# phaistos-networks/Trinity

Hardware: AMD Instinct MI355X
Metric: queries/sec (higher is better)
Workload: dtype u32

## Files before the change

### trinity_amd/csrc/dev_stream.hpp

```cpp
#pragma once
#include "dev_structs.hpp"
#include <hip/hip_runtime.h>

#ifdef TRI_PROF
__device__ unsigned long long g_prof[32];
struct ProfClock {
        long long t;
        unsigned long long acc[16];
        __device__ __forceinline__ void start() {
                for (int i = 0; i < 16; ++i)
                        acc[i] = 0;
                t = clock64();
        }
        __device__ __forceinline__ void lap(const int phase) {
                const long long n = clock64();
                acc[phase] += (unsigned long long)(n - t);
                t = n;
        }
        __device__ __forceinline__ void flush() {
                if (threadIdx.x == 0)
                        for (int i = 0; i < 16; ++i)
                                if (acc[i])
                                        atomicAdd(&g_prof[i], acc[i]);
        }
};
#define PROF_DECL ProfClock prof_
#define PROF_START() prof_.start()
#define PROF_LAP(p) prof_.lap(p)
#define PROF_FLUSH() prof_.flush()
#define PROF_ARG , ProfClock &prof_
#define PROF_PASS , prof_
#ifdef TRI_PROF_COUNTS
#define PROF_COUNT(slot, n) atomicAdd(&g_prof[slot], (unsigned long long)(n))
#else
#define PROF_COUNT(slot, n)
#endif
#else
#define PROF_DECL
#define PROF_START()
#define PROF_LAP(p)
#define PROF_FLUSH()
#define PROF_ARG
#define PROF_PASS
#define PROF_COUNT(slot, n)
#endif

#ifdef TRI_TASKTIMES
static unsigned long long *g_tt_host = nullptr;
static size_t g_tt_cap = 0;
__device__ unsigned long long *g_tt = nullptr;
#define TASKTIME_(i) do { if (threadIdx.x == 0) g_tt[(i)] = wall_clock64(); } while (0)
#if TRI_TASKTIMES == 2
#define TASKTIME(i)
#define TASKTIME_SCORE(i) TASKTIME_(i)
#define TASKTIME_PLANES(i)
#define TASKTIME_DENSE(i)
#define TASKTIME_PHRASE(i)
#elif TRI_TASKTIMES == 3
#define TASKTIME(i)
#define TASKTIME_SCORE(i)
#define TASKTIME_PLANES(i) TASKTIME_(i)
#define TASKTIME_DENSE(i)
#define TASKTIME_PHRASE(i)
#elif TRI_TASKTIMES == 4
#define TASKTIME(i)
#define TASKTIME_SCORE(i)
#define TASKTIME_PLANES(i)
#define TASKTIME_DENSE(i) TASKTIME_(i)
#define TASKTIME_PHRASE(i)
#elif TRI_TASKTIMES == 5
#define TASKTIME(i)
#define TASKTIME_SCORE(i)
#define TASKTIME_PLANES(i)
#define TASKTIME_DENSE(i)
#define TASKTIME_PHRASE(i) TASKTIME_(i)
#else
#define TASKTIME(i) TASKTIME_(i)
#define TASKTIME_SCORE(i)
#define TASKTIME_PLANES(i)
#define TASKTIME_DENSE(i)
#define TASKTIME_PHRASE(i)
#endif
#else
#define TASKTIME(i)
#define TASKTIME_SCORE(i)
#define TASKTIME_PLANES(i)
#define TASKTIME_DENSE(i)
#define TASKTIME_PHRASE(i)
#endif

#ifdef TRI_TRACE
static uint32_t *g_trace_host = nullptr;
__device__ volatile uint32_t *g_trace = nullptr;
#ifndef TRI_TRACE_MASK
#define TRI_TRACE_MASK 0xffffffffu
#endif
#define TRACE(stage, a, b)                                                      \
        do {                                                                    \
                if (((TRI_TRACE_MASK >> (stage)) & 1u) && threadIdx.x == 0 && g_trace) {                              \
                        volatile uint32_t *t_ = g_trace + (blockIdx.x & 63) * 4; \
                        t_[0] = (stage);                                        \
                        t_[1] = (a);                                            \
                        t_[2] = (b);                                            \
                        t_[3] = t_[3] + 1;                                      \
                        __threadfence_system();                                 \
                }                                                               \
        } while (0)
#else
#define TRACE(stage, a, b) \
        do {               \
        } while (0)
#endif

__device__ __forceinline__ uint32_t vb_decode(uint64_t w, uint32_t &len) {
        const uint32_t lo32 = (uint32_t)w;
        const uint32_t b0 = lo32 & 0xffu;
        const uint32_t ones = __clz(~(lo32 << 24));
        const uint32_t n = ones < 4u ? ones : 4u;
        const uint32_t be = __builtin_bswap32(lo32);
        const uint32_t v1 = b0;
        const uint32_t v2 = (be >> 16) & 0x3fffu;
        const uint32_t v3 = ((b0 & 0x1fu) << 16) | ((lo32 >> 8) & 0xffffu);
        const uint32_t v4 = be & 0x0fffffffu;
        const uint32_t v5 = (uint32_t)(w >> 8);
        len = n + 1;
        uint32_t v = v1;
        v = n == 1 ? v2 : v;
        v = n == 2 ? v3 : v;
        v = n == 3 ? v4 : v;
        v = n == 4 ? v5 : v;
        return v;
}

#ifndef TRI_VB_AHEAD
#define TRI_VB_AHEAD 3
#endif
struct VbStream {
        static constexpr int AHEAD = TRI_VB_AHEAD;
        const uint64_t *q;
        uint64_t lo, hi, n[AHEAD];
        int valid;

        __device__ __forceinline__ void init(const uint8_t *p) {
                const uint32_t sk = (uint32_t)((uintptr_t)p & 7u);
                q = (const uint64_t *)(p - sk);
                const uint64_t w0 = q[0], w1 = q[1];
#pragma unroll
                for (int i = 0; i < AHEAD; ++i)
                        n[i] = q[2 + i];
                q += 2 + AHEAD;
                const uint32_t sh = sk * 8;
                lo = sh ? (w0 >> sh) | (w1 << (64 - sh)) : w0;
                hi = sh ? (w1 >> sh) : w1;
                valid = 16 - (int)sk;
        }
        __device__ __forceinline__ void refill() {
                if (valid <= 8) {
                        const uint64_t w = n[0];
#pragma unroll
                        for (int i = 0; i + 1 < AHEAD; ++i)
                                n[i] = n[i + 1];
                        n[AHEAD - 1] = *q++;
                        const uint32_t sh = (uint32_t)valid * 8;
                        if (valid == 8)
                                hi = w;
                        else if (valid == 0) {
                                lo = w;
                                hi = 0;
                        } else {
                                lo |= w << sh;
                                hi = w >> (64 - sh);
                        }
                        valid += 8;
                }
        }
        __device__ __forceinline__ uint32_t next() {
                refill();
                uint32_t len;
                const uint32_t v = vb_decode(lo, len);
                const uint32_t s = len * 8;
                lo = (lo >> s) | (hi << (64 - s));
                hi >>= s;
                valid -= (int)len;
                return v;
        }
        __device__ __forceinline__ const uint8_t *tell() const { return (const uint8_t *)q - 8 * AHEAD - valid; }
        __device__ __forceinline__ uint32_t byte() {
                refill();
                const uint32_t b = (uint32_t)lo & 0xffu;
                lo = (lo >> 8) | (hi << 56);
                hi >>= 8;
                valid -= 1;
                return b;
        }
        __device__ __forceinline__ void skip(uint32_t n) {
                for (; n; --n)
                        (void)byte();
        }
        __device__ __forceinline__ bool small_run(const uint32_t k) const { return (lo & (0x8080808080808080ull >> (8u * (8u - k)))) == 0; }
        __device__ __forceinline__ uint64_t take(const uint32_t k) {
                const uint64_t w = lo;
                if (k == 8) {
                        lo = hi;
                        hi = 0;
                } else {
                        const uint32_t s = k * 8;
                        lo = (lo >> s) | (hi << (64 - s));
                        hi >>= s;
                }
                valid -= (int)k;
                return w;
        }
};
```

### trinity_amd/csrc/dev_structs.hpp

```cpp
#pragma once
#include <cstdint>
#ifdef __HIPCC__
#define TRI_HD __host__ __device__
#else
#define TRI_HD
#endif

struct DevTerm {
        uint32_t documents;
        uint32_t first_block;
        uint32_t nblocks;
        uint32_t last_n;
        uint32_t win_off;
        uint32_t flags;
        uint32_t npfor;
        uint32_t pad;
};
constexpr uint32_t TERM_FULL_BLOCKS = 1u;
constexpr uint32_t TERM_SPARSE = 2u;

#define TRI_BLOCK_N(t, b, index, off) (((t).flags & TERM_FULL_BLOCKS) ? ((b) + 1 == (t).nblocks ? (t).last_n : 32u) : (uint32_t)(index)[(off)-1])
constexpr uint32_t WIN_MIN_BLOCKS = 128;

constexpr uint32_t QT_GROUP = 0x80000000u;
constexpr uint32_t QT_NOT = 0x40000000u;
constexpr uint32_t QT_TERM = 0x3fffffffu;
constexpr uint32_t MAX_QTERMS = 16;
struct DevQuery {
        uint32_t nterms;
        uint32_t term_base;
        uint64_t out_off;
        uint32_t out_cap;
        uint32_t qid;
        uint32_t first_task, ntasks;
        uint32_t score_base, nscore;
        uint32_t phrase_base, nphrases;
        uint32_t fused_idx, form;
};

constexpr uint32_t RESULT_DOCIDS = 0, RESULT_BITMAP = 1;
constexpr uint32_t MAX_PHRASE_TERMS = 16;
struct DevPhrase {
        uint32_t term_base;
        uint32_t nterms;
        double weight;
};

struct DevTask {
        uint32_t slot;
        uint32_t tile_begin;
        uint32_t tile_end;
        uint32_t kind;
        uint64_t out_off;
};
constexpr uint32_t CAND_QUEUES = 8;
constexpr uint32_t CAND_TICKET_STRIDE = 16;
constexpr uint32_t CAND_HEAVY_TILES = 3;
constexpr uint32_t TASK_CAND = 0;
constexpr uint32_t TASK_DENSE = 1;
constexpr uint32_t TASK_FUSED = 2;
constexpr uint32_t TASK_FUSED16 = 3;

constexpr uint32_t TASK_FUSED_GEN = 4;
constexpr uint32_t TASK_PLANES = 5;
constexpr uint32_t TASK_PLANES8 = 6;
constexpr uint32_t TASK_PSET = 7;
constexpr uint32_t TASK_PROBE = 8;
constexpr uint32_t TASK_TREE = 9;
constexpr uint32_t TASK_KINDS = 10;
constexpr uint32_t PSET_INLINE_TERMS = 4;
#ifndef TRI_PSET_TASK_WINDOWS
#define TRI_PSET_TASK_WINDOWS 4
#endif
constexpr uint32_t PSET_TASK_WINDOWS = TRI_PSET_TASK_WINDOWS;
struct DevPsetUnit {
        uint64_t out_off;
        uint32_t w_begin, w_end;
        uint32_t tix;
        uint32_t nterms;
        uint32_t term_base;
        uint32_t first;
        uint32_t tt[PSET_INLINE_TERMS];
        uint32_t row[PSET_INLINE_TERMS];
};
static_assert(sizeof(DevPsetUnit) == 64, "one cache-line half per unit");
constexpr uint32_t PSET_UNIT_FIRST = 1u, PSET_UNIT_BITMAP = 2u;
constexpr uint32_t PSET_UNIT_ROUND_SHIFT = 4, PSET_UNIT_ROUND_MASK = 15u;
constexpr uint32_t PSET_ROUND_DOCS = 16384, PSET_STAGE_DOCS = 1024;
constexpr uint32_t PSET_UNIT_SCATTER = 4u;
constexpr uint32_t TREE_MAX_NODES = 64;
constexpr uint32_t TREE_HDR_WORDS = 8;
constexpr uint32_t TREE_CHUNK_WORDS = 2048;
constexpr uint32_t TREE_ROW_PHRASE = 0x80000000u;
struct DevTreeNode {
        uint8_t op;
        uint8_t parent;
        uint8_t ord;
        uint8_t thr;
        uint32_t arg;
        uint32_t row;
        uint32_t score;
        uint32_t rmask;
        uint8_t kid0, kid1, pad0, pad1;
        uint64_t kids;
};
static_assert(sizeof(DevTreeNode) == 32, "eight words per node");
TRI_HD constexpr bool task_onepass(const uint32_t kind) { return kind >= TASK_FUSED && kind <= TASK_PLANES8; }

constexpr uint32_t PL_W = 32768;
constexpr uint32_t PL_WORDS = PL_W / 32;
constexpr uint32_t PL_NONE = 0xffffffffu;
constexpr uint32_t PL_NESTED = 6;
constexpr uint32_t PL_LEVEL_WORDS = 3;
constexpr uint32_t PL_STORED = 4;
constexpr uint32_t PL_PLANES = PL_STORED + PL_LEVEL_WORDS;
constexpr uint32_t PL_HI = PL_PLANES - 1;
constexpr uint32_t PL_HI_LEVELS = PL_STORED - 1;
constexpr uint32_t PL_RANK_WORDS = 16;
constexpr uint32_t PL_RANK_DOCS = 256;
constexpr uint32_t BLK_HITS_PLAIN = 0x80000000u;
constexpr int TILE_BLOCKS = 256;
constexpr int TILE_CANDS = TILE_BLOCKS * 32;
constexpr uint32_t SPAN_BITS = 1u << 17;
constexpr uint32_t SPAN_WORDS = SPAN_BITS / 32;
constexpr uint32_t CELL_LOG2 = 10;
constexpr uint32_t CELL_DOCS = 1u << CELL_LOG2;
constexpr uint32_t CELLS_PER_SPAN = SPAN_BITS / CELL_DOCS;
#ifndef TRI_FUS_CELLS
#define TRI_FUS_CELLS 14
#endif
constexpr uint32_t FUS_CELLS = TRI_FUS_CELLS;
constexpr uint32_t FUS_W = FUS_CELLS * CELL_DOCS;
constexpr uint32_t PLK_MAX_SPARSE = 6;
constexpr uint32_t PLK_NS_SMALL = 5;
constexpr uint32_t TOPK_MAX = 256;
constexpr uint32_t FUS_MAX_SLOTS = 8;
constexpr uint32_t FUS_MAX_LEAVES = 16;
struct DevFused {
        uint32_t nslots;
        uint32_t fbits;
        uint32_t cap;
        uint32_t nreq;
        uint32_t term[FUS_MAX_SLOTS];
        uint32_t gmask[FUS_MAX_SLOTS];
        uint32_t gslots[FUS_MAX_SLOTS];
        uint32_t nmask;
        uint32_t hw;
        uint32_t mode;
        uint32_t nleaf;
        uint32_t tt[8];
        uint8_t leaf_slot[FUS_MAX_LEAVES];
        uint32_t ctt[FUS_MAX_LEAVES][8];
        uint32_t plane[FUS_MAX_SLOTS];
        uint32_t negslots;
};
constexpr uint32_t FUS_MODE_TT = 1;
constexpr uint32_t FUS_MODE_EMIT = 2;
```

### trinity_amd/csrc/host/plan_host.cpp

```cpp
#include "../planner.hpp"
#include "../lucene_enc_units.hpp"
#include "lucene_encoder.hpp"

#include <cstdlib>
#include <memory>
#include <mutex>

namespace {
        struct HostPlan {
                BatchPlan P;
                uint8_t *block = nullptr;
                ~HostPlan() { free(block); }
        };
        void put_err(char *err, size_t cap, const std::string &s) {
                if (err && cap) {
                        const size_t n = std::min(cap - 1, s.size());
                        memcpy(err, s.data(), n);
                        err[n] = 0;
                }
        }
}

extern "C" {
void *tri_host_index_build(const uint8_t *index, uint64_t len, const uint8_t *hits, uint64_t hits_len, int codec, const uint32_t *terms3, uint64_t nterms,
                           uint32_t docs_cnt, char *err, uint64_t errcap) {
        auto H = std::make_unique<HostIndex>();
        std::string e;
        static_assert(sizeof(tri_term) == 12, "tri_term is three u32");
        if (build_host_index(index, len, hits, hits_len, codec, reinterpret_cast<const tri_term *>(terms3), nterms, docs_cnt, *H, e) != TRI_OK) {
                put_err(err, errcap, e);
                return nullptr;
        }
        return H.release();
}
void tri_host_index_free(void *h) { delete static_cast<HostIndex *>(h); }

void *tri_host_plan(void *hindex, const uint32_t *prog, uint64_t prog_len, const uint32_t *queries2, uint64_t nq, uint32_t flags, uint32_t topk, int similarity,
                    unsigned threads, const char *const *opt_names, const uint64_t *opt_values, unsigned nopt, uint32_t cus, char *err, uint64_t errcap) {
        const HostIndex &H = *static_cast<HostIndex *>(hindex);
        PlanEnv env;
        env.cus = cus ? cus : 256;
        bool use_frag_cache = false;
        for (unsigned i = 0; i < nopt; ++i) {
                const std::string n = opt_names[i];
                if (n == "frag_cache") {
                        use_frag_cache = opt_values[i] != 0;
                        continue;
                }
                tri_options &o = env.opt;
                uint64_t *slot = n == "dense_min_postings" ? &o.dense_min_postings : n == "dense_task_cost" ? &o.dense_task_cost : n == "fused" ? &o.fused
                                 : n == "fused_task_cost" ? &o.fused_task_cost : n == "fused_freq_cap" ? &o.fused_freq_cap : n == "fused_halfwords" ? &o.fused_halfwords
                                 : n == "account_needed_bytes" ? &o.account_needed_bytes : n == "planes" ? &o.planes : n == "planes_split" ? &o.planes_split
                                 : n == "plane_div" ? &o.plane_div : n == "plane_max_bytes" ? &o.plane_max_bytes : n == "probe_max_blocks" ? &o.probe_max_blocks : n == "tree_max_bytes" ? &o.tree_max_bytes : n == "result_bitmaps" ? &o.result_bitmaps : n == "cand_task_cost" ? &o.cand_task_cost : n == "dense_window_cost" ? &o.dense_window_cost
                                 : n == "cand_xcd" ? &o.cand_xcd : n == "planes_order" ? &o.planes_order : n == "pset_order" ? &o.pset_order : n == "scatter_bitmap_slack" ? &o.scatter_bitmap_slack : n == "phrase_task_div" ? &o.phrase_task_div : n == "plane_amortize" ? &o.plane_amortize : nullptr;
                if (!slot) {
                        put_err(err, errcap, "unknown option " + n);
                        return nullptr;
                }
                *slot = opt_values[i];
        }
        PlanInput in;
        in.prog = prog;
        in.prog_len = prog_len;
        static_assert(sizeof(tri_query) == 8, "tri_query is two u32");
        in.queries = reinterpret_cast<const tri_query *>(queries2);
        in.nq = nq;
        in.flags = flags;
        in.topk = topk;
        in.similarity = similarity;
        auto hp = std::make_unique<HostPlan>();
        std::unique_ptr<HostPool> pool;
        if (threads > 1)
                pool = std::make_unique<HostPool>(threads);
        std::string e;
        static trip::FragCache g_frag_cache;
        static std::mutex g_frag_mu;
        std::unique_lock<std::mutex> frag_lock(g_frag_mu, std::defer_lock);
        if (use_frag_cache)
                frag_lock.lock();
        const int rc = plan_batch(
                H, env, in, pool.get(),
                [&](size_t bytes) {
                        hp->block = static_cast<uint8_t *>(aligned_alloc(64, (bytes + 63) & ~(size_t)63));
                        if (hp->block)
                                memset(hp->block, 0, bytes);
                        return hp->block;
                },
                hp->P, e, use_frag_cache ? &g_frag_cache : nullptr);
        if (rc != TRI_OK) {
                put_err(err, errcap, e);
                return nullptr;
        }
        return hp.release();
}
void tri_host_plan_free(void *p) { delete static_cast<HostPlan *>(p); }

void tri_host_plan_summary(void *p, uint64_t *out , double *ms ) {
        const BatchPlan &P = static_cast<HostPlan *>(p)->P;
        const uint64_t v[] = {P.block_bytes,       P.plan.size(),    P.qterms.size(),      P.tasks.size(),  P.fused.size(),       P.qplane.size(),    P.plane_terms.size(), P.sterms.size(),
                              P.sweights.size(),   P.phrases.size(), P.pterms.size(),      P.ptasks.size(), P.plan.off,           P.qterms.off,       P.tasks.off,          P.sched.off,
                              P.fused.off,         P.qplane.off,     P.plane_terms.off,    P.sterms.off,    P.sweights.off,       P.phrases.off,      P.pterms.off,         P.ptasks.off,
                              P.n_dense,           P.n_cand,         P.n_fused,            P.n_fused16,     P.n_fusedgen,         P.n_planes,         P.n_planes8,          P.plw,
                              P.sparse_cap,        P.out_capacity,   P.term_bytes,         P.term_bytes_dense, P.dense_queries,   P.cand_queries,     P.fused_queries,      P.planes_queries,
                              P.unsupported_queries, P.rich_R,       sizeof(DevQuery),     sizeof(DevTask), sizeof(DevFused),     sizeof(DevPhrase),  P.cand_needed_term_bytes, P.plane_decoded_bytes,
                              P.n_pset,            P.pset_queries,   P.n_probe,            P.probe_queries, P.units.size(),       P.units.off,        P.pset_sched.off,     sizeof(DevPsetUnit),
                              P.n_tree,            P.tree_queries,   P.tree.size(),        P.tree.off,      P.tree_terms.size(),  P.tree_terms.off,   P.tree_hidden.size(), P.tree_hidden.off,
                              P.cand_q.off};
        static_assert(sizeof v / sizeof v[0] == 65, "summary layout");
        memcpy(out, v, sizeof v);
        if (ms)
                memcpy(ms, P.plan_ms, sizeof P.plan_ms);
}
const uint8_t *tri_host_plan_block(void *p) { return static_cast<HostPlan *>(p)->P.block; }
void tri_host_plan_query_maps(void *p, uint32_t *slot_of_query, int32_t *qstatus) {
        const BatchPlan &P = static_cast<HostPlan *>(p)->P;
        memcpy(slot_of_query, P.slot_of_query.data(), P.slot_of_query.size() * 4);
        memcpy(qstatus, P.qstatus.data(), P.qstatus.size() * 4);
}
}

extern "C" {
int tri_host_lucene_encode(const uint32_t *docs, const uint32_t *freqs, const uint16_t *pos, const uint64_t *term_first, uint64_t nterms, uint8_t *index_out, uint64_t icap,
                           uint64_t *ilen, uint8_t *hits_out, uint64_t hcap, uint64_t *hlen, uint32_t *terms3) {
        using namespace trinity_amd::Codecs;
        Lucene::IndexSession sess;
        Lucene::Encoder enc(&sess);
        uint64_t h = 0;
        for (uint64_t t = 0; t < nterms; ++t) {
                enc.begin_term();
                for (uint64_t p = term_first[t]; p < term_first[t + 1]; ++p) {
                        enc.begin_document(docs[p]);
                        for (uint32_t i = 0; i < freqs[p]; ++i)
                                enc.new_hit(pos[h++]);
                        enc.end_document();
                }
                trinity_amd::term_index_ctx tctx;
                enc.end_term(&tctx);
                terms3[3 * t] = tctx.documents, terms3[3 * t + 1] = tctx.offset, terms3[3 * t + 2] = tctx.size;
        }
        *ilen = sess.indexOut.size(), *hlen = sess.positionsOut.size();
        if (*ilen > icap || *hlen > hcap)
                return -1;
        if (*ilen)
                memcpy(index_out, sess.indexOut.data(), *ilen);
        if (*hlen)
                memcpy(hits_out, sess.positionsOut.data(), *hlen);
        return 0;
}
int tri_host_lucene_encode_units(const uint32_t *docs, const uint32_t *freqs, const uint16_t *pos, const uint64_t *term_first, uint64_t nterms, uint8_t *index_out, uint64_t icap,
                                 uint64_t *ilen, uint8_t *hits_out, uint64_t hcap, uint64_t *hlen, uint32_t *terms3) {
        const uint64_t np = term_first[nterms];
        std::vector<uint64_t> hit_off(np + 1, 0), dblk_first(nterms + 1, 0), hblk_first(nterms + 1, 0);
        for (uint64_t p = 0; p < np; ++p)
                hit_off[p + 1] = hit_off[p] + freqs[p];
        for (uint64_t t = 0; t < nterms; ++t) {
                dblk_first[t + 1] = dblk_first[t] + (term_first[t + 1] - term_first[t]) / LENC_BLOCK;
                hblk_first[t + 1] = hblk_first[t] + (hit_off[term_first[t + 1]] - hit_off[term_first[t]]) / LENC_BLOCK;
        }
        std::vector<uint32_t> hdelta(hit_off[np] + 1);
        LencArgs a{docs, freqs, pos, hit_off.data(), term_first, hdelta.data(), dblk_first.data(), hblk_first.data(), nterms};
        for (uint64_t p = 0; p < np; ++p)
                lenc_unit_hdelta(a, p, hdelta.data());
        const uint64_t nd = dblk_first[nterms], nh = hblk_first[nterms];
        std::vector<uint64_t> doff(nd + 1, 0), hoff(nh + 1, 0), term_off(nterms + 1, 0), hterm_off(nterms + 1, 0);
        std::vector<uint32_t> tail_d(nterms + 1), tail_h(nterms + 1);
        for (uint64_t g = 0; g < nd; ++g)
                doff[g + 1] = doff[g] + lenc_unit_dblk_size(a, g);
        for (uint64_t h = 0; h < nh; ++h)
                hoff[h + 1] = hoff[h] + lenc_unit_hblk_size(a, h);
        for (uint64_t t = 0; t < nterms; ++t)
                lenc_unit_tail_size(a, t, &tail_d[t], &tail_h[t]);
        LencPlace pl{doff.data(), hoff.data(), term_off.data(), hterm_off.data(), tail_d.data(), tail_h.data()};
        for (uint64_t t = 0; t < nterms; ++t) {
                term_off[t + 1] = term_off[t] + lenc_term_index_size(a, pl, t);
                hterm_off[t + 1] = hterm_off[t] + lenc_term_hits_size(a, pl, t);
        }
        *ilen = term_off[nterms], *hlen = hterm_off[nterms];
        if (*ilen > icap || *hlen > hcap)
                return -1;
        for (uint64_t g = 0; g < nd; ++g)
                lenc_unit_dblk_write(a, pl, g, index_out);
        for (uint64_t h = 0; h < nh; ++h)
                lenc_unit_hblk_write(a, pl, h, hits_out);
        for (uint64_t t = 0; t < nterms; ++t) {
                lenc_unit_term_write(a, pl, t, index_out, hits_out);
                terms3[3 * t] = (uint32_t)(term_first[t + 1] - term_first[t]), terms3[3 * t + 1] = (uint32_t)term_off[t], terms3[3 * t + 2] = lenc_term_index_size(a, pl, t);
        }
        return 0;
}
}

extern "C" {
void tri_host_pfor128_group(const uint32_t *v, uint8_t *a, uint32_t *alen, uint8_t *b, uint32_t *blen) {
        auto get = [&](uint32_t i) { return v[i]; };
        const Pfor128Plan p = pfor128_plan(get);
        uint8_t *e = pfor128_emit(get, p, a);
        *alen = (uint32_t)(e - a);
        if ((uint32_t)(e - a) != p.bytes)
                *alen = 0xffffffffu;
        std::vector<uint8_t> o;
        trinity_amd::Codecs::Lucene::ints_encode(v, o);
        memcpy(b, o.data(), o.size());
        *blen = (uint32_t)o.size();
}
uint32_t tri_host_fastpfor_encode(const uint32_t *v, uint32_t *out) {
        std::vector<uint32_t> w;
        trif::fastpfor_encode(v, w);
        memcpy(out, w.data(), w.size() * 4);
        return (uint32_t)w.size();
}
int tri_host_fastpfor_decode(const uint32_t *w, uint32_t L, uint32_t *v) { return trif::fastpfor_decode(w, L, v) ? 1 : 0; }
uint32_t tri_host_pool_cpus(uint32_t threads, int32_t *out, uint32_t cap) {
        HostPool pool(threads);
        const std::vector<int> &c = pool.pinned_cpus();
        for (size_t i = 0; i < c.size() && i < cap; ++i)
                out[i] = c[i];
        return (uint32_t)c.size();
}

uint32_t tri_host_cpu_budget() { return host_cpu_budget(); }

void tri_host_index_facts(void *h, uint64_t *info6, uint32_t *per_term3) {
        const HostIndex &H = *static_cast<HostIndex *>(h);
        info6[0] = H.info.postings, info6[1] = H.info.blocks, info6[2] = H.info.doc_bytes, info6[3] = H.info.hit_bytes, info6[4] = H.transcoded_groups, info6[5] = H.dev_index.size();
        for (size_t t = 0; t < H.terms.size(); ++t) {
                per_term3[3 * t] = H.terms[t].documents;
                per_term3[3 * t + 1] = H.terms[t].nblocks;
                per_term3[3 * t + 2] = H.terms[t].nblocks ? H.blk_last[H.terms[t].first_block + H.terms[t].nblocks - 1] : 0;
        }
}
}
```

### trinity_amd/csrc/k_match.hpp

```cpp
#pragma once
#include "codec_streams.hpp"

constexpr int AND_WG = 256;
constexpr int DENSE_WG = 512;
static_assert(TILE_BLOCKS == AND_WG, "the candidate kernel maps one 32-candidate row to each of its 256 lanes");

__device__ __forceinline__ uint32_t uni(uint32_t v) { return (uint32_t)__builtin_amdgcn_readfirstlane((int)v); }

__device__ __forceinline__ uint32_t phys(uint32_t j) { return (j & ~31u) | ((j + (j >> 5)) & 31u); }

__device__ __forceinline__ uint32_t wave_excl_scan(uint32_t v, uint32_t &total) {
        uint32_t x = v;
        asm volatile("s_nop 1\n\t"
                     "v_add_u32_dpp %0, %0, %0 row_shr:1 row_mask:0xf bank_mask:0xf bound_ctrl:1\n\t"
                     "s_nop 1\n\t"
                     "v_add_u32_dpp %0, %0, %0 row_shr:2 row_mask:0xf bank_mask:0xf bound_ctrl:1\n\t"
                     "s_nop 1\n\t"
                     "v_add_u32_dpp %0, %0, %0 row_shr:4 row_mask:0xf bank_mask:0xf bound_ctrl:1\n\t"
                     "s_nop 1\n\t"
                     "v_add_u32_dpp %0, %0, %0 row_shr:8 row_mask:0xf bank_mask:0xf bound_ctrl:1\n\t"
                     "s_nop 1\n\t"
                     "v_add_u32_dpp %0, %0, %0 row_bcast:15 row_mask:0xa bank_mask:0xf\n\t"
                     "s_nop 1\n\t"
                     "v_add_u32_dpp %0, %0, %0 row_bcast:31 row_mask:0xc bank_mask:0xf\n\t"
                     "s_nop 1"
                     : "+v"(x));
        total = (uint32_t)__builtin_amdgcn_readlane((int)x, 63);
        return x - v;
}

constexpr uint32_t BM_B_WORDS = SPAN_WORDS + 32;
constexpr uint32_t BM_STRIDE = BM_B_WORDS + BM_B_WORDS / 32;
__device__ __forceinline__ uint32_t bm_pad(const uint32_t w) { return w + (w >> 5); }

__device__ __forceinline__ float sim_score(const int sim, const double weight, const uint32_t freq32) {
        const float f = (float)(uint16_t)freq32;
        if (sim == TRI_SIM_TFIDF)
                return (float)((double)sqrtf(f) * weight);
        if (sim == TRI_SIM_TRIVIAL)
                return f;
        return (float)(weight * (double)f / (double)(f + 1.2f));
}

struct AndShared {
        uint32_t cand[TILE_CANDS];
        uint32_t hit[TILE_BLOCKS];
        uint32_t scan[8];
        uint32_t bcast[4];
        uint32_t lcur[16];
};

struct DenseShared {
        uint32_t bm[2 * BM_STRIDE];
        uint32_t tbase[DENSE_WG];
        uint32_t scan[8];
        uint32_t bcast[4];
        uint32_t lcur[16];
        uint32_t seg_lo[MAX_QTERMS];
        uint32_t seg_cnt[MAX_QTERMS + 1];
        DevTerm seg_term[MAX_QTERMS];
        uint32_t seg_tt[MAX_QTERMS];
        uint32_t seg_wlo[MAX_QTERMS];
        uint32_t seg_whi[MAX_QTERMS];
        uint32_t seg_plane[MAX_QTERMS];
        uint32_t nslow;
};
constexpr uint32_t DENSE_SLOW_CAP = DENSE_WG / 4;

template <int WG = AND_WG>
__device__ uint32_t wg_lower_bound(uint32_t *scan, const uint32_t *__restrict__ a, const uint32_t n, const uint32_t key) {
        const uint32_t tid = threadIdx.x;
        uint32_t lo = 0, hi = n;
        while (hi > lo) {
                const uint32_t len = hi - lo;
                const uint32_t step = (len + WG - 1) / WG;
                const uint32_t pos = lo + (tid + 1) * step - 1;
                const bool ge = pos >= hi ? true : a[pos] >= key;
                const uint64_t m = __ballot(ge);
                scan[tid >> 6] = m ? (tid & ~63u) + (uint32_t)__builtin_ctzll(m) : 0xffffffffu;
                __syncthreads();
                uint32_t first = 0xffffffffu;
#pragma unroll
                for (int wv = 0; wv < WG / 64; ++wv)
                        first = min(first, scan[wv]);
                first = uni(first);
                __syncthreads();
                if (first == 0xffffffffu)
                        return hi;
                const uint32_t nlo = lo + first * step;
                const uint32_t nhi = min(hi, lo + (first + 1) * step - 1);
                lo = nlo;
                hi = step == 1 ? nlo : nhi;
        }
        return lo;
}

typedef uint32_t u32x4_a4 __attribute__((ext_vector_type(4), aligned(4)));
__device__ __forceinline__ void block_bytes32_issue(const uint8_t *__restrict__ p, uint32_t (&r)[9]) {
        const uint8_t *q = p - ((uintptr_t)p & 3u);
        const u32x4_a4 A = *(const u32x4_a4 *)q, B = *(const u32x4_a4 *)(q + 16);
        r[0] = A.x, r[1] = A.y, r[2] = A.z, r[3] = A.w, r[4] = B.x, r[5] = B.y, r[6] = B.z, r[7] = B.w;
        r[8] = *(const uint32_t *)(q + 32);
}
__device__ __forceinline__ bool block_bytes32_finish(const uint8_t *__restrict__ p, const uint32_t (&r)[9], uint32_t (&v)[8]) {
        const uint32_t sk = (uint32_t)((uintptr_t)p & 3u);
#pragma unroll
        for (int i = 0; i < 8; ++i)
                v[i] = __builtin_amdgcn_alignbyte(r[i + 1], r[i], sk);
        return ((v[0] | v[1] | v[2] | v[3] | v[4] | v[5] | v[6] | (v[7] & 0x00ffffffu)) & 0x80808080u) == 0;
}
__device__ __forceinline__ bool load_block_bytes32(const uint8_t *__restrict__ p, uint32_t (&v)[8]) {
        uint32_t r[9];
        block_bytes32_issue(p, r);
        return block_bytes32_finish(p, r, v);
}

__device__ __forceinline__ uint32_t cand_gallop(const AndShared &sh, uint32_t ptr, const uint32_t C, const uint32_t doc) {
        uint32_t step = 1, lo = ptr;
        while (lo + step <= C && sh.cand[phys(lo + step - 1)] < doc) {
                lo += step;
                step <<= 1;
        }
        uint32_t hi = min(lo + step - 1, C);
        while (lo < hi) {
                const uint32_t mid = (lo + hi) >> 1;
                if (sh.cand[phys(mid)] < doc)
                        lo = mid + 1;
                else
                        hi = mid;
        }
        return lo;
}

template <int CODEC, bool PRE>
__device__ __forceinline__ void merge_block(AndShared &sh, const uint8_t *__restrict__ index, const DevTerm &t, const uint32_t b, const uint32_t off,
                                            const uint32_t n, const uint32_t prev, const uint32_t last, uint32_t ptr, uint32_t cv, const uint32_t C,
                                            const uint32_t (&raw)[9]) {
        uint32_t doc = prev;
        uint32_t v[8];
        if (CODEC == CODEC_GOOGLE && n == 32 && (PRE ? block_bytes32_finish(index + off, raw, v) : load_block_bytes32(index + off, v))) {
                uint32_t c[8];
#pragma unroll
                for (int i = 0; i < 8; ++i)
                        c[i] = ptr + i < C ? sh.cand[phys(ptr + i)] : 0xffffffffu;
                if (c[7] > last) {
                        uint32_t at = ptr;
#pragma unroll
                        for (int j = 0; j < 32; ++j) {
                                doc = j < 31 ? doc + ((v[j >> 2] >> ((j & 3) * 8)) & 0xffu) : last;
                                while (c[0] <= doc) {
                                        if (c[0] == doc)
                                                atomicOr(&sh.hit[at >> 5], 1u << (at & 31));
                                        ++at;
#pragma unroll
                                        for (int i = 0; i < 7; ++i)
                                                c[i] = c[i + 1];
                                        c[7] = 0xffffffffu;
                                }
                                if (c[0] > last)
                                        return;
                        }
                        return;
                }
#pragma unroll
                for (int j = 0; j < 32; ++j) {
                        doc = j < 31 ? doc + ((v[j >> 2] >> ((j & 3) * 8)) & 0xffu) : last;
                        if (cv <= doc) {
                                if (cv == doc)
                                        atomicOr(&sh.hit[ptr >> 5], 1u << (ptr & 31));
                                ptr = cand_gallop(sh, ptr + 1, C, doc);
                                cv = ptr < C ? sh.cand[phys(ptr)] : 0xffffffffu;
                                if (cv == doc)
                                        atomicOr(&sh.hit[ptr >> 5], 1u << (ptr & 31));
                                if (cv > last)
                                        return;
                        }
                }
                return;
        }
        DeltaStream<CODEC> s;
        s.init(index, t, b, off);
        for (uint32_t i = 0; i < n; ++i) {
                doc = (i + 1 < n) ? doc + s.next() : last;
                if (cv < doc) {
                        ptr = cand_gallop(sh, ptr + 1, C, doc);
                        cv = ptr < C ? sh.cand[phys(ptr)] : 0xffffffffu;
                }
                if (cv == doc)
                        atomicOr(&sh.hit[ptr >> 5], 1u << (ptr & 31));
                if (cv > last)
                        break;
        }
}

__device__ __forceinline__ uint32_t wave_lower_bound(const uint32_t *__restrict__ a, uint32_t lo, uint32_t hi, const uint32_t key) {
        const uint32_t lane = threadIdx.x & 63u;
        while (hi > lo) {
                const uint32_t len = hi - lo;
                const uint32_t step = (len + 63u) / 64u;
                const uint32_t pos = lo + (lane + 1) * step - 1;
                const bool ge = pos >= hi ? true : a[pos] >= key;
                const uint64_t m = __ballot(ge);
                if (m == 0)
                        return hi;
                const uint32_t first = (uint32_t)__builtin_ctzll(m);
                const uint32_t nlo = lo + first * step;
                const uint32_t nhi = min(hi, lo + (first + 1) * step - 1);
                lo = nlo;
                hi = step == 1 ? nlo : nhi;
        }
        return lo;
}

template <int CODEC>
__device__ void and_filter_tile(AndShared &sh, const uint8_t *__restrict__ index, const uint32_t *__restrict__ blk_last,
                                const uint32_t *__restrict__ blk_off, const uint32_t *__restrict__ win, const DevTerm t, const uint32_t C,
                                const uint32_t lcur_slot, const bool block_driven PROF_ARG) {
        const uint32_t tid = threadIdx.x;
        const uint32_t *bl = blk_last + t.first_block;
        const uint32_t *bo = blk_off + t.first_block;
        const uint32_t cmin = sh.cand[phys(0)], cmax = sh.cand[phys(C - 1)];

        if (block_driven) {
                uint32_t lcur = uni(sh.lcur[lcur_slot]);
                if (lcur == 0xffffffffu)
                        lcur = wg_lower_bound(sh.scan, bl, t.nblocks, cmin);
                for (;;) {
                        const uint32_t b = lcur + tid;
                        const bool below = b < t.nblocks && bl[b] < cmin;
                        const uint64_t m = __ballot(below);
                        const uint32_t lead = m == ~0ull ? 64u : (uint32_t)__builtin_ctzll(~m);
                        sh.scan[tid >> 6] = lead;
                        __syncthreads();
                        uint32_t adv = 0;
                        for (int w = 0; w < AND_WG / 64; ++w) {
                                adv += sh.scan[w];
                                if (sh.scan[w] != 64)
                                        break;
                        }
                        adv = uni(adv);
                        __syncthreads();
                        lcur += adv;
                        if (adv != AND_WG || lcur >= t.nblocks)
                                break;
                }
                sh.lcur[lcur_slot] = lcur;
                PROF_LAP(5);
                TRACE(10, lcur, t.nblocks);
                uint32_t nprev = 0, nlast = 0, noff = 0;
                {
                        const uint32_t b = lcur + tid;
                        if (b < t.nblocks) {
                                nprev = b ? bl[b - 1] : 0;
                                nlast = bl[b];
                                noff = bo[b];
                        }
                }
                for (uint32_t cb = lcur; cb < t.nblocks; cb += AND_WG) {
                        TRACE(11, cb, t.nblocks);
                        const uint32_t b = cb + tid;
                        bool beyond = true;
                        const uint32_t prev = nprev, last = nlast, off = noff;
                        uint32_t raw[9];
                        const bool full = CODEC == CODEC_GOOGLE && b < t.nblocks && prev < cmax && TRI_BLOCK_N(t, b, index, off) == 32;
                        if (full)
                                block_bytes32_issue(index + off, raw);
                        {
                                const uint32_t b2 = b + AND_WG;
                                if (b2 < t.nblocks) {
                                        nprev = bl[b2 - 1];
                                        nlast = bl[b2];
                                        noff = bo[b2];
                                }
                        }
                        if (b < t.nblocks) {
                                beyond = last >= cmax;
                                if (prev < cmax) {
                                        uint32_t lo = 0, hi = C;
                                        while (lo < hi) {
                                                const uint32_t mid = (lo + hi) >> 1;
                                                if (sh.cand[phys(mid)] <= prev)
                                                        lo = mid + 1;
                                                else
                                                        hi = mid;
                                        }
                                        uint32_t ptr = lo;
                                        uint32_t cv = ptr < C ? sh.cand[phys(ptr)] : 0xffffffffu;
                                        PROF_LAP(6);
                                        if (cv <= last) {
                                                if (full)
                                                        merge_block<CODEC, true>(sh, index, t, b, off, 32, prev, last, ptr, cv, C, raw);
                                                else
                                                        merge_block<CODEC, false>(sh, index, t, b, off, TRI_BLOCK_N(t, b, index, off), prev, last, ptr, cv, C, raw);
                                        }
                                        PROF_LAP(7);
                                }
                        }
                        sh.scan[4 + (tid >> 6)] = __ballot(beyond) != 0ull;
                        __syncthreads();
                        const uint32_t any_beyond = uni(sh.scan[4] | sh.scan[5] | sh.scan[6] | sh.scan[7]);
                        __syncthreads();
                        PROF_LAP(8);
                        if (any_beyond)
                                break;
                }
        } else {
                uint32_t carry = 0xffffffffu;
                uint32_t wcur = 0;
                for (uint32_t base = 0; base < C; base += AND_WG) {
                        TRACE(20, base, C);
                        const uint32_t j = base + tid;
                        uint32_t bj = 0xffffffffu;
                        uint32_t cv = 0;
                        const uint32_t wbase = base + (tid & ~63u);
                        uint32_t rlo = 0, rhi = 0;
                        if (t.win_off != 0xffffffffu) {
                                if (j < C) {
                                        const uint32_t c = sh.cand[phys(j)] >> CELL_LOG2;
                                        rlo = win[t.win_off + c];
                                        rhi = win[t.win_off + c + 1];
                                }
                        } else if (wbase < C) {
                                const uint32_t nval = min(64u, C - wbase);
                                const uint32_t klo = sh.cand[phys(wbase)], khi = sh.cand[phys(wbase + nval - 1)];
                                rlo = wave_lower_bound(bl, wcur, t.nblocks, klo);
                                rhi = wave_lower_bound(bl, rlo, t.nblocks, khi);
                                wcur = rlo;
                        }
                        if (j < C) {
                                cv = sh.cand[phys(j)];
                                uint32_t lo = rlo, hi = rhi;
                                while (lo < hi) {
                                        const uint32_t mid = (lo + hi) >> 1;
                                        if (bl[mid] < cv)
                                                lo = mid + 1;
                                        else
                                                hi = mid;
                                }
                                bj = lo;
                        }
                        uint32_t prevb = __shfl_up(bj, 1, 64);
                        if ((tid & 63u) == 0)
                                prevb = carry;
                        carry = __shfl(bj, 63, 64);
                        if (j < C && bj < t.nblocks && bj != prevb) {
                                const uint32_t prev = bj ? bl[bj - 1] : 0;
                                const uint32_t none[9] = {};
                                merge_block<CODEC, false>(sh, index, t, bj, bo[bj], TRI_BLOCK_N(t, bj, index, bo[bj]), prev, bl[bj], j, cv, C, none);
                        }
                }
        }
}

__device__ __forceinline__ void dense_visit(uint32_t *bm, const uint32_t rel) {
        uint32_t w, r, a;
        asm("v_lshrrev_b32 %0, 5, %1" : "=v"(w) : "v"(rel));
        asm("v_lshrrev_b32 %0, 10, %1" : "=v"(r) : "v"(rel));
        asm("v_add_lshl_u32 %0, %1, %2, 2" : "=v"(a) : "v"(w), "v"(r));
        atomicOr((uint32_t *)((uint8_t *)bm + a), 1u << (rel & 31u));
}
__device__ __forceinline__ void dense_visit_clamped(uint32_t *bm, const uint32_t rel, const uint32_t wbase) {
        atomicOr(&bm[bm_pad(min(rel >> 5, SPAN_WORDS) + wbase)], 1u << (rel & 31u));
}

template <int CODEC>
__device__ __forceinline__ void dense_block_stream(const uint8_t *__restrict__ index, const DevTerm &t, const uint32_t b, const uint32_t off,
                                                   const uint32_t n, const uint32_t prev, const uint32_t last, const uint32_t w0, uint32_t *bm,
                                                   const uint32_t wbase) {
        uint32_t rel = prev - w0;
        const uint32_t nd = n - 1;
        if (CODEC != CODEC_GOOGLE) {
                DeltaStream<CODEC> ls;
                ls.init(index, t, b, off);
                for (uint32_t i = 0; i < nd; ++i) {
                        rel += ls.next();
                        dense_visit_clamped(bm, rel, wbase);
                }
                dense_visit_clamped(bm, last - w0, wbase);
                return;
        }
        VbStream s;
        s.init(index + off);
        uint32_t i = 0;
        while (i < nd) {
                s.refill();
                const uint32_t k = min(8u, nd - i);
                if (s.small_run(k)) {
                        uint64_t w = s.take(k);
#pragma unroll
                        for (uint32_t j = 0; j < 8; ++j) {
                                if (j < k) {
                                        rel += (uint32_t)(w & 0xffu);
                                        w >>= 8;
                                        dense_visit_clamped(bm, rel, wbase);
                                }
                        }
                        i += k;
                } else {
                        rel += s.next();
                        dense_visit_clamped(bm, rel, wbase);
                        ++i;
                }
        }
        dense_visit_clamped(bm, last - w0, wbase);
}

__device__ __forceinline__ void dense_block_regs(const uint8_t *__restrict__ index, const uint32_t off, const uint32_t n, const uint32_t prev,
                                                 const uint32_t last, const uint32_t w0, uint32_t *bm, const uint32_t wbase) {
        const uint8_t *p = index + off;
        const uint32_t sk = (uint32_t)((uintptr_t)p & 3u);
        const uint8_t *q = p - sk;
        const u32x4_a4 A = *(const u32x4_a4 *)q, B = *(const u32x4_a4 *)(q + 16), C = *(const u32x4_a4 *)(q + 32), D = *(const u32x4_a4 *)(q + 48);
        const uint32_t raw[16] = {A.x, A.y, A.z, A.w, B.x, B.y, B.z, B.w, C.x, C.y, C.z, C.w, D.x, D.y, D.z, D.w};
        uint64_t win = 0;
        uint32_t have = 0, done = 0, rel = prev - w0;
        const uint32_t nd = n - 1;
#pragma unroll
        for (int d = 0; d < 15; ++d) {
                win |= (uint64_t)__builtin_amdgcn_alignbyte(raw[d + 1], raw[d], sk) << (have * 8);
                have += 4;
                while (done < nd) {
                        uint32_t len;
                        const uint32_t v = vb_decode(win, len);
                        if (len > have)
                                break;
                        win >>= 8 * len;
                        have -= len;
                        rel += v;
                        dense_visit_clamped(bm, rel, wbase);
                        ++done;
                }
        }
        if (done < nd) {
                VbStream st;
                st.init(p + (60 - have));
                for (; done < nd; ++done) {
                        rel += st.next();
                        dense_visit_clamped(bm, rel, wbase);
                }
        }
        dense_visit_clamped(bm, last - w0, wbase);
}

__device__ __forceinline__ void dense_block_coop(const uint8_t *__restrict__ index, const uint32_t off, const uint32_t n, const uint32_t prev,
                                                 const uint32_t last, const uint32_t w0, uint32_t *bm, const uint32_t wbase) {
        const uint32_t lane = threadIdx.x & 63u;
        const uint8_t *p = index + off + lane;
        const uint32_t sk = (uint32_t)((uintptr_t)p & 3u);
        const uint32_t *q = (const uint32_t *)(p - sk);
        const uint32_t d0 = q[0], d1 = q[1], d2 = q[2];
        const uint64_t w = (uint64_t)__builtin_amdgcn_alignbyte(d1, d0, sk) | ((uint64_t)__builtin_amdgcn_alignbyte(d2, d1, sk) << 32);
        uint32_t len;
        const uint32_t v = vb_decode(w, len);
        const uint32_t nd = n - 1;
        uint64_t starts = 0;
        uint32_t s = 0, found = 0;
        for (; found < nd && s < 64; ++found) {
                starts |= 1ull << s;
                s += (uint32_t)__builtin_amdgcn_readlane((int)len, (int)s);
        }
        if (found < nd) {
                if (lane == 0)
                        dense_block_regs(index, off, n, prev, last, w0, bm, wbase);
                return;
        }
        const bool is_start = (starts >> lane) & 1ull;
        uint32_t x = is_start ? v : 0u, wtot;
        x += wave_excl_scan(x, wtot);
        if (is_start)
                dense_visit_clamped(bm, prev - w0 + x, wbase);
        if (lane == 0)
                dense_visit_clamped(bm, last - w0, wbase);
}

template <int WG, int CODEC>
__device__ __forceinline__ void dense_pass(DenseShared &sh, const uint8_t *__restrict__ index, const uint32_t *__restrict__ blk_last,
                                           const uint32_t *__restrict__ blk_off, const uint32_t kbeg, const uint32_t kend, const uint32_t ksplit,
                                           const uint32_t w0, const uint32_t *__restrict__ planes, const uint32_t plw PROF_ARG) {
        const uint32_t tid = threadIdx.x;
        uint32_t total = 0;
        for (uint32_t k = kbeg; k < kend; ++k) {
                total += uni(sh.seg_cnt[k]);
                const uint32_t prow = uni(sh.seg_plane[k]);
                if (prow != PL_NONE) {
                        const uint32_t *pa = planes + (size_t)prow * plw + (w0 >> 5);
                        const uint32_t wbase = k < ksplit ? 0u : BM_B_WORDS;
#pragma unroll
                        for (uint32_t j = 0; j < SPAN_WORDS / WG; ++j) {
                                const uint32_t i = j * WG + tid;
                                const uint32_t v = pa[i];
                                if (v)
                                        atomicOr(&sh.bm[bm_pad(i + wbase)], v);
                        }
                }
        }
        for (uint32_t v0 = 0; v0 < total; v0 += WG) {
                const uint32_t v = v0 + tid;
                if (v < total) {
                        uint32_t k = kbeg, r = v;
                        for (uint32_t c = sh.seg_cnt[k]; r >= c; c = sh.seg_cnt[k]) {
                                r -= c;
                                ++k;
                        }
// ... 263 lines not shown
                                bool here = false;
                                if (uni(sh.seg_plane[k]) != PL_NONE) {
                                        cur = 0;
                                        here = true;
                                } else if (uni(t.win_off) != 0xffffffffu) {
                                        cur = uni(sh.seg_wlo[k]);
                                        here = cur != uni(sh.seg_whi[k]);
                                } else {
                                        cur = uni(sh.lcur[k]);
                                        if (cur < uni(t.nblocks) && bl[cur] < w * SPAN_BITS)
                                                cur = uni(wave_lower_bound(bl, cur, t.nblocks, w * SPAN_BITS));
                                        sh.lcur[k] = cur;
                                }
                                if (here)
                                        wnext = w;
                                else if (cur < uni(t.nblocks)) {
                                        const uint32_t first_possible = cur ? bl[cur - 1] + 1 : 1;
                                        wnext = min(wnext, max(w, first_possible / SPAN_BITS));
                                }
                        }
                        wnext = uni(wnext);
                        __syncthreads();
                        if (wnext == w || wnext >= task.tile_end) {
                                w = wnext;
                                break;
                        }
                        w = wnext;
                }
                if (w >= task.tile_end)
                        break;
                const uint32_t w0 = w * SPAN_BITS;
                const uint32_t wlast = w0 + (SPAN_BITS - 1);
                uint32_t ngroups = 0, g1 = q.nterms, g2 = q.nterms;
                bool galive = false, neg = false;
                for (uint32_t k = 0; k < q.nterms; ++k) {
                        const uint32_t tt = uni(sh.seg_tt[k]);
                        const DevTerm t = sh.seg_term[k];
                        const uint32_t nblocks = uni(t.nblocks);
                        const uint32_t *bl = blk_last + t.first_block;
                        if (tt & QT_GROUP) {
                                if (k && !galive)
                                        done = true;
                                if (ngroups == 1)
                                        g1 = k;
                                else if (ngroups == 2)
                                        g2 = k;
                                ++ngroups;
                                galive = false;
                                neg = tt & QT_NOT;
                        }
                        uint32_t b_lo, b_hi;
                        if (uni(sh.seg_plane[k]) != PL_NONE) {
                                galive = true;
                                sh.seg_lo[k] = 0;
                                sh.seg_cnt[k] = 0;
                                continue;
                        }
                        if (uni(t.win_off) != 0xffffffffu) {
                                b_lo = uni(sh.seg_wlo[k]);
                                b_hi = min(uni(sh.seg_whi[k]), nblocks - 1);
                        } else {
                                b_lo = uni(sh.lcur[k]);
                                if (b_lo < nblocks && bl[b_lo] < w0)
                                        b_lo = uni(wave_lower_bound(bl, b_lo, nblocks, w0));
                                b_hi = b_lo;
                                if (b_lo < nblocks) {
                                        b_hi = uni(wave_lower_bound(bl, b_lo, nblocks, wlast));
                                        if (b_hi >= nblocks)
                                                b_hi = nblocks - 1;
                                }
                        }
                        if (b_lo < nblocks)
                                galive = true;
                        sh.seg_lo[k] = b_lo;
                        sh.seg_cnt[k] = b_lo < nblocks ? b_hi - b_lo + 1 : 0;
                }
                sh.seg_cnt[q.nterms] = 0xffffffffu;
                if (!galive && !neg)
                        done = true;
                if (done)
                        break;
                PROF_LAP(1);
                __syncthreads();
                PROF_LAP(2);
                dense_pass<WG, CODEC>(sh, index, blk_last, blk_off, 0, g2, g1, w0, planes, plw PROF_PASS);
                for (uint32_t kb = g2; kb < q.nterms;) {
                        uint32_t ke = kb + 1;
                        while (ke < q.nterms && !(qterms[q.term_base + ke] & QT_GROUP))
                                ++ke;
                        for (uint32_t i = tid; i < BM_STRIDE; i += WG) {
                                sh.bm[i] &= sh.bm[BM_STRIDE + i];
                                sh.bm[BM_STRIDE + i] = 0;
                        }
                        __syncthreads();
                        dense_pass<WG, CODEC>(sh, index, blk_last, blk_off, kb, ke, kb, w0, planes, plw PROF_PASS);
                        kb = ke;
                }
                if (as_bitmap) {
                        for (; wdone < w; ++wdone)
                                dense_store_zero<WG>(qout + (size_t)(wdone - task.tile_begin) * SPAN_WORDS);
                        produced += dense_store<WG>(sh, w0, ngroups > 1, neg, masked, qout + (size_t)(w - task.tile_begin) * SPAN_WORDS);
                        wdone = w + 1;
                } else
                        produced += dense_expand<WG>(sh, w0, ngroups > 1, neg, masked, qout, produced PROF_PASS);
                ++w;
        }
        if (as_bitmap)
                for (; wdone < task.tile_end; ++wdone)
                        dense_store_zero<WG>(qout + (size_t)(wdone - task.tile_begin) * SPAN_WORDS);
        __syncthreads();
        if (uni(tid >> 6) == 0)
                *count_out = produced;
        PROF_LAP(8);
}

#ifndef TRI_DENSE_WAVES
#define TRI_DENSE_WAVES 8
#endif
template <int CODEC>
__global__ __launch_bounds__(DENSE_WG, TRI_DENSE_WAVES) void k_and_dense(const uint8_t *__restrict__ index, const uint32_t *__restrict__ blk_last,
                                                        const uint32_t *__restrict__ blk_off, const uint32_t *__restrict__ win,
                                                        const DevTerm *__restrict__ terms, const DevQuery *__restrict__ plan,
                                                        const DevTask *__restrict__ tasks, const uint32_t *__restrict__ sched,
                                                        const uint32_t *__restrict__ qterms, const uint32_t ntasks, uint32_t *__restrict__ ticket,
                                                        uint32_t *__restrict__ out, uint32_t *__restrict__ counts,
                                                        const uint32_t *__restrict__ masked, const uint32_t *__restrict__ qplane,
                                                        const uint32_t *__restrict__ planes, const uint32_t plw) {
        __shared__ DenseShared sh;
        const uint32_t wave = uni(threadIdx.x >> 6);
        PROF_DECL;
        PROF_START();
        for (;;) {
                if (wave == 0) {
                        const uint32_t old = atomicAdd(ticket, 1u);
                        sh.bcast[0] = uni(old) >> 6;
                }
                __syncthreads();
                const uint32_t ticket_no = uni(sh.bcast[0]);
                __syncthreads();
                if (ticket_no >= ntasks)
                        break;
                const uint32_t tix = sched[ticket_no];
                const DevTask task = tasks[tix];
                const DevQuery q = plan[task.slot];
                PROF_LAP(0);
                TASKTIME_DENSE(8 * ticket_no);
                dense_task<DENSE_WG, CODEC>(sh, index, blk_last, blk_off, win, terms, qterms, q, task, out, counts + tix, masked, qplane, planes, plw PROF_PASS);
                TASKTIME_DENSE(8 * ticket_no + 1);
        }
        PROF_LAP(9);
        PROF_FLUSH();
}

#ifndef TRI_AND_PROBES
#define TRI_AND_PROBES 8
#endif
constexpr int AND_PROBES = TRI_AND_PROBES;
template <int CODEC>
#ifndef TRI_AND_WAVES
#define TRI_AND_WAVES 4
#endif
__global__ __launch_bounds__(AND_WG, TRI_AND_WAVES) void k_and(const uint8_t *__restrict__ index, const uint32_t *__restrict__ blk_last,
                                                const uint32_t *__restrict__ blk_off, const uint32_t *__restrict__ win,
                                                const DevTerm *__restrict__ terms,
                                                const DevQuery *__restrict__ plan, const DevTask *__restrict__ tasks,
                                                const uint32_t *__restrict__ sched, const uint32_t *__restrict__ qterms,
                                                const uint32_t *__restrict__ cand_q, uint32_t *__restrict__ ticket,
                                                uint32_t *__restrict__ out, uint32_t *__restrict__ counts,
                                                const uint32_t *__restrict__ masked, const uint32_t *__restrict__ qplane,
                                                const uint32_t *__restrict__ planes, const uint32_t plw) {
        __shared__ AndShared sh;
        const uint32_t tid = threadIdx.x;
        const uint32_t wave = uni(tid >> 6);
        const uint32_t home = uni(__builtin_amdgcn_s_getreg(20 | (0 << 6) | (3 << 11))) % CAND_QUEUES;
        uint32_t qdone = 0;
        PROF_DECL;
        PROF_START();
        for (;;) {
                if (wave == 0) {
                        uint32_t got = 0xffffffffu;
                        for (uint32_t t = 0; t < CAND_QUEUES && got == 0xffffffffu; ++t) {
                                const uint32_t x = (home + t) % CAND_QUEUES;
                                if ((qdone >> x) & 1u)
                                        continue;
                                const uint32_t q0 = cand_q[x], qn = cand_q[x + 1] - q0;
                                const uint32_t old = uni(atomicAdd(ticket + x * CAND_TICKET_STRIDE, 1u)) >> 6;
                                if (old < qn)
                                        got = q0 + old;
                                else
                                        qdone |= 1u << x;
                        }
                        sh.bcast[0] = got;
                }
                __syncthreads();
                const uint32_t ticket_no = uni(sh.bcast[0]);
                __syncthreads();
                if (ticket_no == 0xffffffffu)
                        break;
                const uint32_t tix = sched[ticket_no];
                TASKTIME(8 * ticket_no);
                const DevTask task = tasks[tix];
                const uint32_t slot = task.slot;
                const DevQuery q = plan[slot];
                const DevTerm lead = terms[qterms[q.term_base] & QT_TERM];
                TRACE(1, slot, q.nterms);
                uint32_t *qout = out + task.out_off;
                uint32_t produced = 0;
                sh.lcur[tid & 15] = 0xffffffffu;
                const uint32_t tb_end = min(lead.nblocks, task.tile_end * TILE_BLOCKS);
                PROF_LAP(10);

                for (uint32_t tb = task.tile_begin * TILE_BLOCKS; tb < tb_end; tb += TILE_BLOCKS) {
                        const uint32_t nb = min((uint32_t)TILE_BLOCKS, lead.nblocks - tb);
                        uint32_t C = (tb + nb == lead.nblocks) ? (nb - 1) * 32 + lead.last_n : nb * 32;
                        if (tid < nb) {
                                const uint32_t b = tb + tid, gb = lead.first_block + b;
                                const uint32_t off = blk_off[gb];
                                const uint32_t n = TRI_BLOCK_N(lead, b, index, off);
                                const uint32_t last = blk_last[gb];
                                uint32_t doc = b ? blk_last[gb - 1] : 0;
#if defined(TRI_AND_EXP) && TRI_AND_EXP == 2
                                const uint32_t row = tid * 32, step = (last - doc) / 32u + 1u;
                                for (uint32_t i = 0; i + 1 < n; ++i) {
                                        doc += step;
                                        sh.cand[row | ((i + tid) & 31u)] = min(doc, last);
                                }
                                sh.cand[row | ((n - 1 + tid) & 31u)] = last;
                                (void)off;
#else
                                DeltaStream<CODEC> s;
                                s.init(index, lead, b, off);
                                const uint32_t row = tid * 32;
                                for (uint32_t i = 0; i + 1 < n; ++i) {
                                        doc += s.next();
                                        sh.cand[row | ((i + tid) & 31u)] = doc;
                                }
                                sh.cand[row | ((n - 1 + tid) & 31u)] = last;
#endif
                        }
                        __syncthreads();
                        PROF_LAP(11);
                        TASKTIME(8 * ticket_no + 2);
                        TRACE(2, slot, tb);

                        bool gneg = false;
                        for (uint32_t k = 1; k < q.nterms && C; ++k) {
                                const uint32_t tt = qterms[q.term_base + k];
                                const DevTerm t = terms[tt & QT_TERM];
                                if (tt & QT_GROUP) {
                                        sh.hit[tid] = 0;
                                        gneg = tt & QT_NOT;
                                }
                                __syncthreads();
#if defined(TRI_FORCE_CAND)
                                const bool bd = false;
#elif defined(TRI_FORCE_BLOCK)
                                const bool bd = true;
#else
                                const bool bd = t.nblocks <= lead.documents;
#endif
                                TRACE(3, slot, (k << 16) | (bd ? 1 : 0));
                                const uint32_t prow = qplane ? qplane[q.term_base + k] : PL_NONE;
                                if (prow != PL_NONE) {
                                        const uint32_t *pa = planes + (size_t)prow * plw;
                                        for (uint32_t j0 = tid; j0 < C; j0 += AND_WG * AND_PROBES) {
                                                uint32_t doc[AND_PROBES], w[AND_PROBES];
#pragma unroll
                                                for (int u = 0; u < AND_PROBES; ++u) {
                                                        const uint32_t j = j0 + u * AND_WG;
                                                        doc[u] = j < C ? sh.cand[phys(j)] : 0u;
                                                }
#pragma unroll
                                                for (int u = 0; u < AND_PROBES; ++u)
#if defined(TRI_AND_EXP) && TRI_AND_EXP == 1
                                                        w[u] = pa[(doc[u] >> 5) & 0x3ffu];
#else
                                                        w[u] = pa[doc[u] >> 5];
#endif
#pragma unroll
                                                for (int u = 0; u < AND_PROBES; ++u) {
                                                        const uint32_t j = j0 + u * AND_WG;
                                                        if (j < C && ((w[u] >> (doc[u] & 31u)) & 1u))
                                                                atomicOr(&sh.hit[j >> 5], 1u << (j & 31u));
                                                }
                                        }
                                } else
                                and_filter_tile<CODEC>(sh, index, blk_last, blk_off, win, t, C, k - 1, bd PROF_PASS);
                                TRACE(4, slot, C);
                                __syncthreads();
                                TASKTIME(8 * ticket_no + 2 + min(k, 5u));
                                PROF_LAP(bd ? 12 : 13);
                                const bool lastterm = k + 1 == q.nterms;
                                if (!lastterm && !(qterms[q.term_base + k + 1] & QT_GROUP))
                                        continue;
                                uint32_t bits = sh.hit[tid];
                                if (gneg) {
                                        const uint32_t left = C > tid * 32 ? C - tid * 32 : 0u;
                                        bits = ~bits & (left >= 32 ? 0xffffffffu : ((1u << left) - 1u));
                                }
                                if (masked && lastterm)
                                        for (uint32_t m = bits; m;) {
                                                const uint32_t kbit = __builtin_ctz(m);
                                                m &= m - 1;
                                                const uint32_t doc = sh.cand[phys(tid * 32 + kbit)];
                                                if ((masked[doc >> 5] >> (doc & 31u)) & 1u)
                                                        bits &= ~(1u << kbit);
                                        }
                                const uint32_t cnt = __popc(bits);
                                uint32_t wtot;
                                uint32_t ex = wave_excl_scan(cnt, wtot);
                                sh.scan[tid >> 6] = wtot;
                                __syncthreads();
                                uint32_t wbase = 0, total = 0;
                                for (int w = 0; w < AND_WG / 64; ++w) {
                                        if (w < (int)(tid >> 6))
                                                wbase += sh.scan[w];
                                        total += sh.scan[w];
                                }
                                ex += wbase;
                                if (lastterm) {
                                        uint32_t m = bits, o = produced + ex;
                                        while (m) {
                                                const uint32_t kbit = __builtin_ctz(m);
                                                m &= m - 1;
                                                qout[o++] = sh.cand[phys(tid * 32 + kbit)];
                                        }
                                } else {
                                        uint32_t vals[32];
#pragma unroll
                                        for (int kk = 0; kk < 32; ++kk)
                                                vals[kk] = sh.cand[(tid * 32) | ((kk + tid) & 31u)];
                                        __syncthreads();
                                        uint32_t o = ex;
#pragma unroll
                                        for (int kk = 0; kk < 32; ++kk)
                                                if ((bits >> kk) & 1u) {
                                                        sh.cand[phys(o)] = vals[kk];
                                                        ++o;
                                                }
                                }
                                C = uni(total);
                                __syncthreads();
                        }
                        if (q.nterms == 1) {
                                if (!masked) {
                                        for (uint32_t j = tid; j < C; j += AND_WG)
                                                qout[produced + j] = sh.cand[phys(j)];
                                } else {
                                        const uint32_t left = C > tid * 32 ? C - tid * 32 : 0u;
                                        uint32_t bits = left >= 32 ? 0xffffffffu : ((1u << left) - 1u);
                                        for (uint32_t m = bits; m;) {
                                                const uint32_t kbit = __builtin_ctz(m);
                                                m &= m - 1;
                                                const uint32_t doc = sh.cand[phys(tid * 32 + kbit)];
                                                if ((masked[doc >> 5] >> (doc & 31u)) & 1u)
                                                        bits &= ~(1u << kbit);
                                        }
                                        uint32_t wtot;
                                        uint32_t ex = wave_excl_scan(__popc(bits), wtot);
                                        sh.scan[tid >> 6] = wtot;
                                        __syncthreads();
                                        uint32_t wbase = 0, total = 0;
                                        for (int w = 0; w < AND_WG / 64; ++w) {
                                                if (w < (int)(tid >> 6))
                                                        wbase += sh.scan[w];
                                                total += sh.scan[w];
                                        }
                                        uint32_t o = produced + ex + wbase;
                                        for (uint32_t m = bits; m;) {
                                                const uint32_t kbit = __builtin_ctz(m);
                                                m &= m - 1;
                                                qout[o++] = sh.cand[phys(tid * 32 + kbit)];
                                        }
                                        C = uni(total);
                                }
                        }
                        produced += C;
                        __syncthreads();
                        PROF_LAP(14);
                }
                if (wave == 0)
                        counts[tix] = produced;
                TASKTIME(8 * ticket_no + 1);
                TRACE(5, slot, produced);
        }
        PROF_LAP(15);
        PROF_FLUSH();
        TRACE(6, 0, 0);
}
```

### trinity_amd/csrc/planner.hpp

```cpp
#pragma once
#include "planner_lower.hpp"
#include "planner_tasks.hpp"

namespace trip {
        struct RowQ {
                uint8_t n = 0, q[CAND_QUEUES] = {}, sub[CAND_QUEUES] = {};
        };
        struct LapTimer {
                const bool on;
                std::chrono::steady_clock::time_point t0 = std::chrono::steady_clock::now();
                std::string line;
                void lap(const char *what) {
                        if (!on)
                                return;
                        char buf[64];
                        snprintf(buf, sizeof buf, " %s %.3f", what, ms_since(t0));
                        line += buf;
                }
        };

        struct PlanState {
                const HostIndex &ix;
                const PlanEnv &env;
                const tri_options &opt;
                HostPool *pool;
                BatchPlan &P;
                std::string &err;
                Ctx C;
                LapTimer dbg;
                FragCache *cache = nullptr;
                std::vector<Frag> frags;
                SectionCounts n;
                uint64_t cand_queries_all = 0;
                std::vector<uint64_t> benefit, cand_row;
                std::vector<uint32_t> tree_terms;
                std::vector<uint32_t> chosen;
                std::vector<uint32_t> row_of_rank;
                bool cand_rows = false;
                std::vector<RowQ> rowq;
                uint32_t pset_ranges = 0;
                uint32_t cand_first = 0, cand_qat[CAND_QUEUES] = {};
                std::vector<uint32_t> unit_of_task;
                ~PlanState() {
                        if (!cache)
                                return;
                        if (cache->frags.size() < frags.size())
                                cache->frags.resize(frags.size());
                        for (size_t k = 0; k < frags.size(); ++k)
                                cache->frags[k] = std::move(frags[k]);
                }
                template <class Fn>
                void run(Fn &&fn) {
                        if (pool && frags.size() > 1)
                                pool->run((unsigned)frags.size(), fn);
                        else
                                for (unsigned k = 0; k < frags.size(); ++k)
                                        fn(k);
                }
                int first_error() {
                        for (Frag &f : frags)
                                if (f.rc != TRI_OK) {
                                        err = f.err;
                                        return f.rc;
                                }
                        return TRI_OK;
                }
                template <class Fn>
                int run_pass(const char *name, const char *doing, Fn &&fn) {
                        run([&](unsigned k) {
                                Frag &f = frags[k];
                                try {
                                        f.rc = fn(f);
                                } catch (const std::bad_alloc &) {
                                        f.rc = herr(f.err, TRI_ERR_NOMEM, "tri_batch_create: out of host memory while %s", doing);
                                } catch (...) {
                                        f.rc = herr(f.err, TRI_ERR_INVALID, "tri_batch_create: unexpected exception while %s", doing);
                                }
                        });
                        dbg.lap(name);
                        return first_error();
                }
        };

        inline void eligible_planes(PlanState &S) {
                const HostIndex &ix = S.ix;
                const tri_options &opt = S.opt;
                S.P.plw = ((ix.max_doc >> 17) + 2u) * (SPAN_BITS / 32u);
                S.C.plw = S.P.plw;
                if (opt.planes && opt.plane_div && !ix.df_sorted.empty()) {
                        const uint64_t min_df = std::max<uint64_t>(1, ix.info.docs_cnt / opt.plane_div);
                        const size_t n = (size_t)(std::partition_point(ix.df_sorted.begin(), ix.df_sorted.end(), [&](uint32_t d) { return d && d >= min_df; }) - ix.df_sorted.begin());
                        const uint64_t row_bytes = (uint64_t)PL_PLANES * S.P.plw * 4;
                        S.C.n_ok = (uint32_t)std::min<uint64_t>(n, std::max<uint64_t>(1, opt.plane_max_bytes / std::max<uint64_t>(1, row_bytes)));
                }
        }

        inline void take_fragments(PlanState &S, FragCache *cache) {
                const size_t nq = S.C.in.nq;
                const unsigned nthreads = S.pool ? std::min<unsigned>(S.pool->size(), (unsigned)std::max<size_t>(1, nq / 512)) : 1u;
                const size_t nfrag = nthreads <= 1 ? 1 : std::min<size_t>(2 * nthreads, std::max<size_t>(1, nq / 256));
                S.frags.resize(nfrag);
                S.cache = cache;
                for (size_t k = 0; k < nfrag; ++k) {
                        if (cache && k < cache->frags.size()) {
                                S.frags[k] = std::move(cache->frags[k]);
                                S.frags[k].recycle();
                        }
                        S.frags[k].q_lo = nq * k / nfrag;
                        S.frags[k].q_hi = nq * (k + 1) / nfrag;
                }
        }

        inline void settle_batch_knobs(PlanState &S) {
                const tri_options &opt = S.opt;
                const PlanEnv &env = S.env;
                Ctx &C = S.C;
                uint64_t onepass_queries = 0, fused_postings = 0, phrase_queries = 0;
                for (const Frag &f : S.frags) {
                        onepass_queries += f.onepass_queries;
                        fused_postings += f.fused_postings;
                        phrase_queries += f.phrase_queries;
                }
                C.phrase_task_div = opt.phrase_task_div ? opt.phrase_task_div : !phrase_queries ? 1 : phrase_queries <= 8ull * env.cus ? 4 : phrase_queries <= 16ull * env.cus ? 2 : 1;
                C.planes_split = opt.planes_split ? opt.planes_split : (2 * onepass_queries >= 4ull * (uint64_t)env.cus * env.plk_wgs_per_cu ? 2 : 3) ;
                C.fused_task_cost = opt.fused_task_cost;
                if (!C.fused_task_cost) {
                        const uint64_t want_tasks = 2ull * (uint64_t)env.cus * env.fus_wgs_per_cu;
                        C.fused_task_cost = std::min<uint64_t>(8u << 20, std::max<uint64_t>(256u << 10, fused_postings / std::max<uint64_t>(1, want_tasks)));
                }
        }

        inline int place_fragments(PlanState &S) {
                BatchPlan &P = S.P;
                SectionCounts &n = S.n;
                const uint32_t n_ok = S.C.n_ok;
                uint64_t off = 0;
                S.benefit.assign(n_ok, 0), S.cand_row.assign(n_ok, 0);
                for (Frag &f : S.frags) {
                        f.b_plan = n.plan, f.b_qterms = n.qterms, f.b_sterms = n.sterms, f.b_phrases = n.phrases, f.b_pterms = n.pterms, f.b_tasks = n.tasks, f.b_fused = n.fused,
                        f.b_ptasks = n.ptasks, f.b_off = off, f.b_units = n.units, f.b_tree = n.tree, f.b_hidden = n.tree_hidden;
                        n.plan += f.tmp.size(), n.qterms += f.qterms.size(), n.sterms += f.sterms.size(), n.phrases += f.phrases.size(), n.pterms += f.pterms.size(),
                                n.tasks += f.tasks.size(), n.fused += f.fused.size(), n.ptasks += f.ptasks.size(), n.units += f.units.size(), n.tree += f.treepool.size(),
                                n.tree_hidden += f.n_hidden, off += f.off;
                        S.tree_terms.insert(S.tree_terms.end(), f.tree_terms.begin(), f.tree_terms.end());
                        P.merge(f);
                        for (uint32_t r = 0; r < n_ok; ++r)
                                S.benefit[r] += f.benefit[r], S.cand_row[r] += f.cand_row[r];
                        for (const size_t qi : f.left_out) {
                                P.qstatus[qi] = TRI_ERR_UNSUPPORTED;
                                ++P.unsupported_queries;
                        }
                        if (!f.left_out.empty())
                                P.last_unsupported = f.err;
                }
                S.cand_queries_all = P.cand_queries + P.probe_queries;
                if (n.qterms > 0xfffffff0ull || n.sterms > 0xfffffff0ull || n.tasks > 0xfffffff0ull || n.pterms > 0xfffffff0ull)
                        return herr(S.err, TRI_ERR_UNSUPPORTED, "tri_batch_create: the batch exceeds 2^32 terms or tasks: split it");
                P.out_capacity = off;
                std::sort(S.tree_terms.begin(), S.tree_terms.end());
                S.tree_terms.erase(std::unique(S.tree_terms.begin(), S.tree_terms.end()), S.tree_terms.end());
                n.tree_terms = S.tree_terms.size();
                P.tree_scratch_bytes = ((uint64_t)n.tree_terms * PL_PLANES + n.tree_hidden + P.tree_queries) * P.plw * 4;
                if (P.tree_scratch_bytes > S.opt.tree_max_bytes)
                        return herr(S.err, TRI_ERR_NOMEM, "tri_batch_create: the batch's %llu tree queries need %llu bytes of bitmap scratch (%zu distinct term leaves, %zu phrase leaves; option tree_max_bytes = %llu): split the batch",
                                    (unsigned long long)P.tree_queries, (unsigned long long)P.tree_scratch_bytes, n.tree_terms, n.tree_hidden, (unsigned long long)S.opt.tree_max_bytes);
                return TRI_OK;
        }

        inline void choose_planes(PlanState &S) {
                const HostIndex &ix = S.ix;
                const uint32_t n_ok = S.C.n_ok;
                std::vector<uint32_t> rank_term(n_ok, UINT32_MAX);
                std::vector<uint8_t> forced(n_ok, 0);
                for (const Frag &f : S.frags) {
                        for (const QUse &u : f.quses)
                                rank_term[ix.df_rank[u.term]] = u.term;
                        for (const QUse &u : f.suses)
                                rank_term[ix.df_rank[u.term]] = u.term;
                        for (const FUse &u : f.fuses)
                                rank_term[ix.df_rank[u.term]] = u.term, forced[ix.df_rank[u.term]] = 1;
                }
                for (uint32_t r = 0; r < n_ok; ++r)
                        if (rank_term[r] != UINT32_MAX && (forced[r] || S.benefit[r] * std::max<uint64_t>(1, S.opt.plane_amortize) >= ix.terms[rank_term[r]].documents))
                                S.chosen.push_back(rank_term[r]);
                std::sort(S.chosen.begin(), S.chosen.end());
                S.row_of_rank.assign(n_ok, PL_NONE);
                for (const uint32_t term : S.chosen) {
                        S.row_of_rank[ix.df_rank[term]] = ix.df_rank[term];
                        S.P.plane_decoded_bytes += ix.docbytes[term];
                }
                S.P.plane_rows = n_ok;
                S.n.plane_terms = S.chosen.size();
                S.n.qplane = S.chosen.empty() ? 0 : S.n.qterms;
                S.n.splane = (S.chosen.empty() || !S.C.scored) ? 0 : S.n.sterms;
                S.n.sweights = S.C.scored ? S.n.sterms : 0;
        }

        inline void assign_cand_rows(PlanState &S) {
                const BatchPlan &P = S.P;
                const uint32_t n_ok = S.C.n_ok;
                const std::vector<uint64_t> &cand_row = S.cand_row;
                S.pset_ranges = ((S.ix.max_doc >> 17) + 1u + PSET_TASK_WINDOWS - 1) / PSET_TASK_WINDOWS;
                S.cand_rows = S.opt.cand_xcd && !S.chosen.empty() && S.cand_queries_all && P.cand_lead_docs >= CAND_ROWS_MIN_LEAD * S.cand_queries_all && P.cand_terms <= 3 * S.cand_queries_all;
                S.rowq.assign(S.cand_rows ? n_ok : 0, RowQ{});
                if (S.cand_rows) {
                        uint64_t total = 0, load[CAND_QUEUES] = {};
                        uint32_t placed[CAND_QUEUES] = {};
                        std::vector<uint32_t> rows;
                        for (uint32_t r = 0; r < n_ok; ++r)
                                if (cand_row[r] && S.row_of_rank[r] != PL_NONE)
                                        rows.push_back(r), total += cand_row[r];
                        std::sort(rows.begin(), rows.end(), [&](uint32_t a, uint32_t b) { return cand_row[a] != cand_row[b] ? cand_row[a] > cand_row[b] : a < b; });
                        const uint64_t cap = std::max<uint64_t>(1, total / (2 * CAND_QUEUES));
                        for (const uint32_t r : rows) {
                                RowQ &z = S.rowq[r];
                                z.n = (uint8_t)std::min<uint64_t>(CAND_QUEUES, (cand_row[r] + cap - 1) / cap);
                                for (uint32_t k = 0; k < z.n; ++k) {
                                        const uint32_t x = (uint32_t)(std::min_element(load, load + CAND_QUEUES) - load);
                                        load[x] += cand_row[r] / z.n;
                                        z.q[k] = (uint8_t)x;
                                        z.sub[k] = (uint8_t)(CAND_COST_SUBS + placed[x]++ % (CAND_SUBS - CAND_COST_SUBS - 1));
                                }
                        }
                }
                if (S.dbg.on) {
                        char buf[96];
                        snprintf(buf, sizeof buf, " [cand queries %llu lead docs %llu terms %llu rows %d]", (unsigned long long)S.cand_queries_all, (unsigned long long)P.cand_lead_docs, (unsigned long long)P.cand_terms, (int)S.cand_rows);
                        S.dbg.line += buf;
                }
        }

        inline int layout_block(PlanState &S, const std::function<uint8_t *(size_t)> &alloc_block) {
                BatchPlan &P = S.P;
                P.block_bytes = layout_sections(P, S.n);
                S.dbg.lap("sums+planes+layout");
                P.block = alloc_block(P.block_bytes);
                S.dbg.lap("alloc_block");
                if (!P.block)
                        return herr(S.err, TRI_ERR_NOMEM, "tri_batch_create: no host memory for the plan (%zu bytes)", P.block_bytes);
                point_sections(P, S.n);
                std::copy(S.tree_terms.begin(), S.tree_terms.end(), P.tree_terms.p);
                S.unit_of_task.assign(S.n.units ? S.n.tasks : 0, 0u);
                std::copy(S.chosen.begin(), S.chosen.end(), P.plane_terms.p);
                S.dbg.lap("spans");
                return TRI_OK;
        }

        inline int fill_fragment(PlanState &S, Frag &f) {
                const HostIndex &ix = S.ix;
                BatchPlan &P = S.P;
                const std::vector<uint32_t> &row_of_rank = S.row_of_rank;
                for (size_t i = 0; i < f.tmp.size(); ++i) {
                        DevQuery q = f.tmp[i].q;
                        q.term_base += (uint32_t)f.b_qterms;
                        q.score_base += (uint32_t)f.b_sterms;
                        q.phrase_base += (uint32_t)f.b_phrases;
                        q.first_task += (uint32_t)f.b_tasks;
                        q.out_off += f.b_off;
                        if (f.tmp[i].fuse)
                                q.fused_idx += (uint32_t)f.b_fused;
                        if (f.tmp[i].tree)
                                q.fused_idx += (uint32_t)f.b_tree;
                        if (f.tmp[i].hidden) {
                                q.qid = 0xffffffffu;
                                P.tree_hidden[f.b_hidden + f.tmp[i].hidden_ord] = (uint32_t)(f.b_plan + i);
                        } else
                                P.slot_of_query[q.qid] = (uint32_t)(f.b_plan + i);
                        P.plan[f.b_plan + i] = q;
                }
                if (!f.treepool.empty()) {
                        memcpy(&P.tree[f.b_tree], f.treepool.data(), f.treepool.size() * 4);
                        for (size_t i = 0; i < f.tmp.size(); ++i) {
                                if (!f.tmp[i].tree)
                                        continue;
                                uint32_t *rec = &P.tree[f.b_tree + f.tmp[i].q.fused_idx];
                                DevTreeNode *tn = reinterpret_cast<DevTreeNode *>(rec + TREE_HDR_WORDS);
                                for (uint32_t k = 0; k < rec[0]; ++k)
                                        if (tn[k].op == TRI_OP_TERM)
                                                tn[k].row = (uint32_t)(std::lower_bound(P.tree_terms.begin(), P.tree_terms.end(), tn[k].arg) - P.tree_terms.begin());
                                        else if (tn[k].op == TRI_OP_PHRASE) {
                                                tn[k].arg += (uint32_t)f.b_plan;
                                                tn[k].row += (uint32_t)f.b_hidden;
                                        }
                        }
                }
                for (size_t i = 0; i < f.tasks.size(); ++i) {
                        DevTask t = f.tasks[i];
                        t.slot += (uint32_t)f.b_plan;
                        t.out_off += f.b_off;
                        P.tasks[f.b_tasks + i] = t;
                }
                if (!f.qterms.empty())
                        memcpy(&P.qterms[f.b_qterms], f.qterms.data(), f.qterms.size() * 4);
                if (!f.sterms.empty())
                        memcpy(&P.sterms[f.b_sterms], f.sterms.data(), f.sterms.size() * 4);
                if (S.C.scored && !f.sweights.empty())
                        memcpy(&P.sweights[f.b_sterms], f.sweights.data(), f.sweights.size() * 8);
                for (size_t i = 0; i < f.phrases.size(); ++i) {
                        DevPhrase ph = f.phrases[i];
                        ph.term_base += (uint32_t)f.b_pterms;
                        P.phrases[f.b_phrases + i] = ph;
                }
                if (!f.pterms.empty())
                        memcpy(&P.pterms[f.b_pterms], f.pterms.data(), f.pterms.size() * 4);
                for (size_t i = 0; i < f.ptasks.size(); ++i)
                        P.ptasks[f.b_ptasks + i] = f.ptasks[i] + (uint32_t)f.b_tasks;
                for (size_t i = 0; i < f.fused.size(); ++i)
                        P.fused[f.b_fused + i] = f.fused[i];
                for (const FUse &u : f.fuses)
                        P.fused[f.b_fused + u.fidx].plane[u.slot] = row_of_rank[ix.df_rank[u.term]];
                for (size_t i = 0; i < f.units.size(); ++i) {
                        DevPsetUnit u = f.units[i];
                        u.out_off += f.b_off;
                        u.tix += (uint32_t)f.b_tasks;
                        u.term_base += (uint32_t)f.b_qterms;
                        const bool is_probe = f.tasks[f.units[i].tix].kind == TASK_PROBE;
                        bool rows = true;
                        for (uint32_t k = is_probe ? 1u : 0u; k < u.nterms; ++k) {
                                const uint32_t term = (k < PSET_INLINE_TERMS ? u.tt[k] : f.qterms[f.units[i].term_base + k]) & QT_TERM;
                                const uint32_t rank = ix.df_rank[term];
                                const uint32_t row = rank < row_of_rank.size() ? row_of_rank[rank] : PL_NONE;
                                rows &= row != PL_NONE;
                                if (k < PSET_INLINE_TERMS)
                                        u.row[k] = row;
                                if (row == PL_NONE && (u.first & PSET_UNIT_SCATTER) && u.w_begin == 0)
                                        f.pscatter_docs += ix.terms[term].documents;
                        }
                        if (is_probe && !rows) {
                                P.tasks[u.tix].kind = TASK_CAND;
                                if (u.first & PSET_UNIT_FIRST) {
                                        ++f.probe_demoted;
                                        f.probe_demoted_bytes += distinct_docbytes(ix, &f.qterms[f.units[i].term_base], u.nterms, f.S.seen);
                                }
                        }
                        P.units[f.b_units + i] = u;
                        S.unit_of_task[u.tix] = (uint32_t)(f.b_units + i);
                }
                if (S.n.splane) {
                        std::fill(&P.splane.p[f.b_sterms], &P.splane.p[f.b_sterms] + f.sterms.size(), PL_NONE);
                        for (const QUse &u : f.suses)
                                P.splane[f.b_sterms + u.qpos] = row_of_rank[ix.df_rank[u.term]];
                }
                if (S.n.qplane) {
                        std::fill(&P.qplane.p[f.b_qterms], &P.qplane.p[f.b_qterms] + f.qterms.size(), PL_NONE);
                        for (const QUse &u : f.quses)
                                P.qplane[f.b_qterms + u.qpos] = row_of_rank[ix.df_rank[u.term]];
                }
                return TRI_OK;
        }

        inline uint32_t key_planes_order(const PlanState &S, const Frag &f, const size_t i, const DevTask &tk) {
                const DevQuery &q = S.P.plan[tk.slot];
                const DevFused &z = S.P.fused[q.fused_idx];
                uint32_t minrow = PL_NONE;
                for (uint32_t sidx = 0; sidx < z.nslots; ++sidx)
                        minrow = std::min(minrow, z.plane[sidx]);
                const uint32_t ord = (uint32_t)(f.b_tasks + i) - q.first_task, per = SCHED_NB / 4;
                return SCHED_RANK[tk.kind] * SCHED_NB + (S.opt.planes_order == 2 ? std::min(minrow, per - 1) * 4 + std::min(ord, 3u) : std::min(ord, 3u) * per + std::min(minrow, per - 1));
        }
        inline uint32_t key_pset_order(const PlanState &S, const Frag &f, const size_t i) {
                const uint32_t range = (uint32_t)(f.tcost[i] & 0xffffffffull) / PSET_TASK_WINDOWS;
                const uint32_t rb = S.pset_ranges <= PSET_RANGE_BKS ? std::min(range, PSET_RANGE_BKS - 1) : (uint32_t)std::min<uint64_t>((uint64_t)range * PSET_RANGE_BKS / S.pset_ranges, PSET_RANGE_BKS - 1);
                return PSET_KEY0 + rb * PSET_SUBS + pset_sub((uint32_t)(f.tcost[i] >> 32));
        }
        inline uint32_t key_cand_rows(const PlanState &S, const Frag &f, const size_t i, const DevTask &tk) {
                const DevQuery &q = S.P.plan[tk.slot];
                uint32_t row = PL_NONE;
                for (uint32_t k = 1; k < q.nterms && row == PL_NONE; ++k)
                        row = S.P.qplane[q.term_base + k];
                uint32_t queue, sub;
                if (tk.tile_end - tk.tile_begin > CAND_HEAVY_TILES || row == PL_NONE)
                        queue = (uint32_t)(f.b_tasks + i) % CAND_QUEUES, sub = (sched_key(TASK_CAND, f.tcost[i]) % SCHED_NB) / (SCHED_NB / CAND_COST_SUBS);
                else if (row < S.rowq.size() && S.rowq[row].n) {
                        const RowQ &z = S.rowq[row];
                        const uint32_t piece = (uint32_t)(f.b_tasks + i) % z.n;
                        queue = z.q[piece], sub = z.sub[piece];
                } else
                        queue = row % CAND_QUEUES, sub = CAND_SUBS - 1;
                return CAND_KEY0 + queue * CAND_SUBS + sub;
        }
        inline uint32_t schedule_key(const PlanState &S, const Frag &f, const size_t i) {
                const DevTask &tk = S.P.tasks[f.b_tasks + i];
                switch (tk.kind) {
                        case TASK_PLANES:
                        case TASK_PLANES8:
                                if (S.opt.planes_order)
                                        return key_planes_order(S, f, i, tk);
                                break;
                        case TASK_PSET:
                                if (S.opt.pset_order)
                                        return key_pset_order(S, f, i);
                                break;
                        case TASK_CAND:
                                if (S.cand_rows)
                                        return key_cand_rows(S, f, i, tk);
                                break;
                }
                return sched_key(tk.kind, f.tcost[i]);
        }
        inline int key_fragment(const PlanState &S, Frag &f) {
                f.keys.resize(f.tasks.size());
                f.hist.assign(SCHED_KEYS, 0u);
                for (size_t i = 0; i < f.tasks.size(); ++i)
                        ++f.hist[f.keys[i] = schedule_key(S, f, i)];
                return TRI_OK;
        }

        inline void place_schedule(PlanState &S) {
                BatchPlan &P = S.P;
                uint32_t at = 0;
                for (uint32_t r = 0; r < TASK_KINDS; ++r) {
                        const uint32_t before = at;
                        if (r == SCHED_RANK[TASK_CAND])
                                S.cand_first = at;
                        auto place = [&](const uint32_t bk) {
                                for (Frag &f : S.frags) {
                                        const uint32_t c = f.hist[bk];
                                        f.hist[bk] = at;
                                        at += c;
                                }
                        };
                        for (uint32_t bk = r * SCHED_NB; bk < (r + 1) * SCHED_NB; ++bk)
                                place(bk);
                        if (r == SCHED_RANK[TASK_PSET] && S.opt.pset_order)
                                for (uint32_t bk = PSET_KEY0; bk < PSET_KEY0 + std::min(S.pset_ranges, PSET_RANGE_BKS) * PSET_SUBS; ++bk)
                                        place(bk);
                        if (r == SCHED_RANK[TASK_CAND])
                                for (uint32_t bk = CAND_KEY0; bk < PSET_KEY0; ++bk) {
                                        if ((bk - CAND_KEY0) % CAND_SUBS == 0)
                                                S.cand_qat[(bk - CAND_KEY0) / CAND_SUBS] = at;
                                        place(bk);
                                }
                        for (uint32_t k = 0; k < TASK_KINDS; ++k)
                                if (SCHED_RANK[k] == r)
                                        P.*SCHED_COUNT[k] = at - before;
                }
                const uint32_t units_first = sched_first(P, TASK_PSET), n_units_run = P.n_pset + P.n_probe;
                S.run([&](unsigned k) {
                        Frag &f = S.frags[k];
                        for (size_t i = 0; i < f.tasks.size(); ++i) {
                                const uint32_t pos = f.hist[f.keys[i]]++, ti = (uint32_t)(f.b_tasks + i);
                                P.sched[pos] = ti;
                                if (pos >= units_first && pos - units_first < n_units_run)
                                        P.pset_sched[pos - units_first] = S.unit_of_task[ti];
                        }
                });
        }

        inline void deal_cand_queues(PlanState &S) {
                BatchPlan &P = S.P;
                const uint32_t nc = P.n_cand;
                uint32_t *const sc = P.sched.p + S.cand_first;
                if (S.cand_rows) {
                        for (uint32_t x = 0; x <= CAND_QUEUES; ++x)
                                P.cand_q[x] = x < CAND_QUEUES ? S.cand_qat[x] - S.cand_first : nc;
                } else {
                        const std::vector<uint32_t> was(sc, sc + nc);
                        uint32_t pos = 0;
                        for (uint32_t x = 0; x < CAND_QUEUES; ++x) {
                                P.cand_q[x] = pos;
                                for (uint32_t i = x; i < nc; i += CAND_QUEUES)
                                        sc[pos++] = was[i];
                        }
                        P.cand_q[CAND_QUEUES] = pos;
                }
        }

        inline void order_phrase_tasks(BatchPlan &P) {
                if (P.ptasks.size() <= 1)
                        return;
                const size_t np = P.ptasks.size();
                std::vector<uint32_t> key(np), sorted(np);
                uint32_t hist[SCHED_NB + 1] = {};
                for (size_t i = 0; i < np; ++i) {
                        const uint32_t ti = P.ptasks[i];
                        const DevTask &tk = P.tasks[ti];
                        const DevQuery &q = P.plan[tk.slot];
                        const uint64_t end = ti + 1 < q.first_task + q.ntasks ? P.tasks[ti + 1].out_off : q.out_off + q.out_cap;
                        key[i] = SCHED_NB - 1 - cost_bucket(end - tk.out_off);
                        ++hist[key[i] + 1];
                }
                for (uint32_t bk = 0; bk < SCHED_NB; ++bk)
                        hist[bk + 1] += hist[bk];
                for (size_t i = 0; i < np; ++i)
                        sorted[hist[key[i]]++] = P.ptasks[i];
                std::copy(sorted.begin(), sorted.end(), P.ptasks.p);
        }

        inline void account_distinct_bytes(const HostIndex &ix, const Ctx &C, BatchPlan &P) {
                std::vector<uint8_t> seen(ix.terms.size(), 0);
                std::vector<uint8_t> seen_hits(ix.terms.size(), 0);
                for (size_t sidx = 0; sidx < P.plan.size(); ++sidx) {
                        const DevQuery &q = P.plan[sidx];
                        const uint32_t kind = P.tasks[q.first_task].kind;
                        auto touch = [&](uint32_t term) {
                                if (!(seen[term] & 0x80u))
                                        P.distinct_bytes += ix.docbytes[term];
                                if (!(seen[term] & (1u << kind)))
                                        P.distinct_bytes_kind[kind] += ix.docbytes[term];
                                seen[term] |= (uint8_t)(0x80u | (1u << kind));
                        };
                        if (kind == TASK_TREE) {
                                const uint32_t *rec = &P.tree[q.fused_idx];
                                const DevTreeNode *tn = reinterpret_cast<const DevTreeNode *>(rec + TREE_HDR_WORDS);
                                for (uint32_t k = 0; k < rec[0]; ++k)
                                        if (tn[k].op == TRI_OP_TERM)
                                                touch(tn[k].arg);
                        } else if (task_onepass(kind)) {
                                const DevFused &z = P.fused[q.fused_idx];
                                for (uint32_t k = 0; k < z.nslots; ++k)
                                        touch(z.term[k]);
                        } else {
                                for (uint32_t k = 0; k < q.nterms; ++k)
                                        touch(P.qterms[q.term_base + k] & QT_TERM);
                                if (C.mode != TRI_FLAG_DOCUMENTS_ONLY)
                                        for (uint32_t k = 0; k < q.nscore; ++k)
                                                touch(P.sterms[q.score_base + k]);
                        }
                        auto touch_hits = [&](uint32_t term, bool phrase) {
                                if (!(seen_hits[term] & 1u))
                                        P.distinct_bytes += ix.hitbytes[term];
                                if (phrase && !(seen_hits[term] & 2u))
                                        P.distinct_bytes_kind[TASK_KINDS] += ix.hitbytes[term];
                                seen_hits[term] |= (uint8_t)(1u | (phrase ? 2u : 0u));
                        };
                        for (uint32_t ph = 0; ph < q.nphrases; ++ph)
                                for (uint32_t k = 0; k < P.phrases[q.phrase_base + ph].nterms; ++k)
                                        touch_hits(P.pterms[P.phrases[q.phrase_base + ph].term_base + k], true);
                        if (C.rich)
                                for (uint32_t k = 0; k < q.nscore; ++k)
                                        touch_hits(P.sterms[q.score_base + k], false);
                }
        }
}

inline int plan_batch(const HostIndex &ix, const PlanEnv &env, const PlanInput &in, HostPool *pool, const std::function<uint8_t *(size_t)> &alloc_block,
                      BatchPlan &P, std::string &err, trip::FragCache *frag_cache = nullptr) {
        using namespace trip;
        auto t0 = std::chrono::steady_clock::now();
        static const bool dbg_plan = getenv("TRINITY_DEBUG_PLAN") != nullptr;
        const uint32_t mode = in.flags & (TRI_FLAG_DOCUMENTS_ONLY | TRI_FLAG_ACCUMULATED_SCORE | TRI_FLAG_MATCHED_TERMS);
        PlanState S{ix, env, env.opt, pool, P, err, Ctx{ix, env, in, mode == TRI_FLAG_ACCUMULATED_SCORE, mode == TRI_FLAG_MATCHED_TERMS, mode}, LapTimer{dbg_plan}};
        P.slot_of_query.assign(in.nq, UINT32_MAX);
        P.qstatus.assign(in.nq, TRI_OK);
        eligible_planes(S);
        take_fragments(S, frag_cache);
        S.dbg.lap("setup");
        if (const int rc = S.run_pass("LOWER", "lowering the batch", [&](Frag &f) { return lower_range(S.C, f); }))
                return rc;
        settle_batch_knobs(S);
        S.dbg.lap("glue0");
        P.plan_ms[0] = ms_since(t0);
        if (const int rc = S.run_pass("TASKS", "cutting the batch into tasks", [&](Frag &f) { return task_range(S.C, f); }))
                return rc;
        P.plan_ms[1] = ms_since(t0);
        if (const int rc = place_fragments(S))
                return rc;
        choose_planes(S);
        assign_cand_rows(S);
        if (const int rc = layout_block(S, alloc_block))
                return rc;
        if (const int rc = S.run_pass("FILL", "filling the plan", [&](Frag &f) {
                    fill_fragment(S, f);
                    return key_fragment(S, f);
            }))
                return rc;
        for (const Frag &f : S.frags) {
                P.pscatter_docs += f.pscatter_docs;
                P.probe_queries -= f.probe_demoted, P.cand_queries += f.probe_demoted;
                P.term_bytes_probe -= f.probe_demoted_bytes;
        }
        P.plan_ms[2] = ms_since(t0);
        place_schedule(S);
        deal_cand_queues(S);
        order_phrase_tasks(P);
        P.sparse_cap = (P.sparse_cap + 63u) & ~63u;
        S.dbg.lap("sched+rest");
        if (dbg_plan)
                fprintf(stderr, "[tri plan] nq %zu frags %zu:%s\n", in.nq, S.frags.size(), S.dbg.line.c_str());
        P.plan_ms[3] = ms_since(t0);
        if (env.opt.account_needed_bytes && !ix.terms.empty())
                account_distinct_bytes(ix, S.C, P);
        return TRI_OK;
}
```

### trinity_amd/csrc/planner_types.hpp

```cpp
#pragma once
#include "host_pool.hpp"
#include "index_host.hpp"

#include <array>
#include <chrono>
#include <cmath>
#include <memory>
#include <numeric>

struct tri_options {
        uint64_t dense_min_postings = 512 * 1024;
        uint64_t dense_task_cost = 192 * 1024;
        uint64_t dense_window_cost = 16 * 1024;
        uint64_t cand_task_cost = 32 * 1024;
        uint64_t fused = 1;
        uint64_t fused_task_cost = 0;
        uint64_t fused_freq_cap = 0;
        uint64_t account_needed_bytes = 0;
        uint64_t fused_halfwords = 1;
        uint64_t overlap_dense_wgs = 0, overlap_cand_wgs = 0;
        uint64_t overlap = 0;
        uint64_t planes = 7;
        uint64_t planes_split = 0;
        uint64_t plane_div = 1024;
        uint64_t plane_amortize = 1;
        uint64_t plane_max_bytes = 8ull << 30;
        uint64_t planes_rebuild = 0;
        uint64_t phrase_task_div = 0;
        uint64_t planes_order = 1;
        uint64_t scatter_bitmap_slack = 4;
        uint64_t pset_order = 1;
        uint64_t cand_xcd = 1;
        uint64_t plan_threads = 0;
        uint64_t plan_hot_us = 300;
        uint64_t plan_pin = 2;
        uint64_t result_bitmaps = 1;
        uint64_t tree_max_bytes = 16ull << 30;
        uint64_t probe_max_blocks = 0;
};

struct PlanEnv {
        tri_options opt;
        uint32_t cus = 256;
        uint32_t fus_wgs_per_cu = 2;
        uint32_t plk_wgs_per_cu = 2;
};

template <class T>
struct Span {
        T *p = nullptr;
        size_t n = 0;
        size_t off = 0;
        size_t size() const { return n; }
        bool empty() const { return !n; }
        T *data() { return p; }
        const T *data() const { return p; }
        T &operator[](size_t i) { return p[i]; }
        const T &operator[](size_t i) const { return p[i]; }
        T *begin() { return p; }
        T *end() { return p + n; }
        const T *begin() const { return p; }
        const T *end() const { return p + n; }
};

struct PlanInput {
        const uint32_t *prog = nullptr;
        size_t prog_len = 0;
        const tri_query *queries = nullptr;
        size_t nq = 0;
        const double *weights = nullptr;
        uint32_t flags = 0, topk = 0;
        int similarity = TRI_SIM_BM25;
};

namespace trip {
        struct PlanCounters {
                uint64_t term_bytes = 0, term_bytes_dense = 0, term_bytes_fused = 0, term_bytes_planes = 0, term_bytes_phrase_hits = 0, term_bytes_pset = 0, term_bytes_probe = 0,
                         cand_needed_term_bytes = 0;
                uint64_t dense_queries = 0, pset_queries = 0, probe_queries = 0, cand_queries = 0, fused_queries = 0, planes_queries = 0, tree_queries = 0;
                uint64_t bitmap_queries = 0;
                uint64_t pscatter_queries = 0, pscatter_docs = 0;
                uint64_t cand_lead_docs = 0, cand_terms = 0;
                uint64_t probe_demoted = 0, probe_demoted_bytes = 0;
                uint32_t sparse_cap = 0;
                uint32_t rich_R = 0;
                bool rich_allow = false;
                void merge(const PlanCounters &o) {
                        term_bytes += o.term_bytes, term_bytes_dense += o.term_bytes_dense, term_bytes_fused += o.term_bytes_fused, term_bytes_planes += o.term_bytes_planes;
                        term_bytes_phrase_hits += o.term_bytes_phrase_hits, term_bytes_pset += o.term_bytes_pset, term_bytes_probe += o.term_bytes_probe;
                        cand_needed_term_bytes += o.cand_needed_term_bytes;
                        dense_queries += o.dense_queries, pset_queries += o.pset_queries, probe_queries += o.probe_queries, cand_queries += o.cand_queries;
                        fused_queries += o.fused_queries, planes_queries += o.planes_queries, tree_queries += o.tree_queries;
                        bitmap_queries += o.bitmap_queries, pscatter_queries += o.pscatter_queries, pscatter_docs += o.pscatter_docs;
                        cand_lead_docs += o.cand_lead_docs, cand_terms += o.cand_terms;
                        probe_demoted += o.probe_demoted, probe_demoted_bytes += o.probe_demoted_bytes;
                        sparse_cap = std::max(sparse_cap, o.sparse_cap);
                        rich_R = std::max(rich_R, o.rich_R);
                        rich_allow |= o.rich_allow;
                }
        };
}

struct BatchPlan : trip::PlanCounters {
        uint8_t *block = nullptr;
        size_t block_bytes = 0;
        Span<DevQuery> plan;
        Span<uint32_t> qterms;
        Span<DevTask> tasks;
        Span<uint32_t> sched;
        Span<DevFused> fused;
        Span<uint32_t> qplane;
        Span<uint32_t> plane_terms;
        Span<uint32_t> splane;
        Span<uint32_t> sterms;
        Span<double> sweights;
        Span<DevPhrase> phrases;
        Span<uint32_t> pterms, ptasks;
        Span<DevPsetUnit> units;
        Span<uint32_t> pset_sched;
        Span<uint32_t> cand_q;
        Span<uint32_t> tree;
        Span<uint32_t> tree_terms;
        Span<uint32_t> tree_hidden;
        uint32_t n_tree = 0;
        uint64_t tree_scratch_bytes = 0;
        std::vector<uint32_t> slot_of_query;
        std::vector<int32_t> qstatus;
        uint32_t n_dense = 0, n_pset = 0, n_probe = 0, n_cand = 0, n_fused = 0, n_fused16 = 0, n_fusedgen = 0, n_planes = 0, n_planes8 = 0;
        uint32_t plw = 0;
        uint32_t plane_rows = 0;
        uint64_t out_capacity = 0;
        uint64_t plane_decoded_bytes = 0, unsupported_queries = 0;
        uint64_t distinct_bytes = 0, distinct_bytes_kind[TASK_KINDS + 1] = {};
        std::string last_unsupported;
        double plan_ms[4] = {0, 0, 0, 0};
};

namespace trip {
        constexpr size_t SECTION_ALIGN = 64;
        struct SectionCounts {
                size_t plan = 0, qterms = 0, tasks = 0, fused = 0, qplane = 0, plane_terms = 0, splane = 0, sterms = 0, sweights = 0, phrases = 0, pterms = 0, ptasks = 0, units = 0,
                       tree = 0, tree_terms = 0, tree_hidden = 0;
        };
        template <class Plan, class Fn>
        inline void for_each_section(Plan &P, const SectionCounts &n, Fn &&fn) {
                fn(P.plan, n.plan);
                fn(P.qterms, n.qterms);
                fn(P.tasks, n.tasks);
                fn(P.sched, n.tasks);
                fn(P.fused, n.fused);
                fn(P.qplane, n.qplane);
                fn(P.plane_terms, n.plane_terms);
                fn(P.splane, n.splane);
                fn(P.sterms, n.sterms);
                fn(P.sweights, n.sweights);
                fn(P.phrases, n.phrases);
                fn(P.pterms, n.pterms);
                fn(P.ptasks, n.ptasks);
                fn(P.units, n.units);
                fn(P.pset_sched, n.units);
                fn(P.cand_q, (size_t)CAND_QUEUES + 1);
                fn(P.tree, n.tree);
                fn(P.tree_terms, n.tree_terms);
                fn(P.tree_hidden, n.tree_hidden);
        }
        inline size_t layout_sections(BatchPlan &P, const SectionCounts &n) {
                size_t bytes = 0;
                for_each_section(P, n, [&](auto &s, const size_t count) {
                        s.off = bytes;
                        s.n = count;
                        bytes += (count * sizeof(*s.p) + SECTION_ALIGN + SECTION_ALIGN - 1) & ~(SECTION_ALIGN - 1);
                });
                return bytes;
        }
        inline void point_sections(BatchPlan &P, const SectionCounts &n) {
                for_each_section(P, n, [&](auto &s, size_t) { s.p = reinterpret_cast<std::remove_reference_t<decltype(*s.p)> *>(P.block + s.off); });
        }

        constexpr uint32_t SCHED_NB = 64 * 4;
        constexpr uint32_t CAND_SUBS = 128, CAND_COST_SUBS = 16;
        constexpr uint32_t PSET_RANGE_BKS = 64, PSET_SUBS = 64;
        constexpr uint32_t CAND_KEY0 = TASK_KINDS * SCHED_NB, PSET_KEY0 = CAND_KEY0 + CAND_QUEUES * CAND_SUBS, SCHED_KEYS = PSET_KEY0 + PSET_RANGE_BKS * PSET_SUBS;
        inline uint32_t pset_sub(const uint32_t rank) { return rank < PSET_SUBS / 2 ? rank : std::min(PSET_SUBS / 2 + (rank - PSET_SUBS / 2) / 8, PSET_SUBS - 1); }
        constexpr uint64_t CAND_ROWS_MIN_LEAD = 1024;
        constexpr uint32_t SCHED_RANK[TASK_KINDS] = {3, 0, 4, 5, 6, 7, 8, 1, 2, 9};
        constexpr uint32_t BatchPlan::*const SCHED_COUNT[TASK_KINDS] = {&BatchPlan::n_cand, &BatchPlan::n_dense, &BatchPlan::n_fused, &BatchPlan::n_fused16, &BatchPlan::n_fusedgen,
                                                                        &BatchPlan::n_planes, &BatchPlan::n_planes8, &BatchPlan::n_pset, &BatchPlan::n_probe, &BatchPlan::n_tree};
        inline uint32_t sched_first(const BatchPlan &P, const uint32_t kind) {
                uint32_t at = 0;
                for (uint32_t k = 0; k < TASK_KINDS; ++k)
                        if (SCHED_RANK[k] < SCHED_RANK[kind])
                                at += P.*SCHED_COUNT[k];
                return at;
        }
        inline uint32_t cost_bucket(const uint64_t cost) {
                const uint64_t c = std::max<uint64_t>(1, cost);
                const uint32_t lg = 63u - (uint32_t)__builtin_clzll(c);
                const uint32_t frac = lg >= 2 ? (uint32_t)((c >> (lg - 2)) & 3u) : (uint32_t)((c << (2 - lg)) & 3u);
                return lg * 4 + frac;
        }
        inline uint32_t sched_key(const uint32_t kind, const uint64_t cost) {
                if (kind == TASK_PSET)
                        return SCHED_RANK[TASK_PSET] * SCHED_NB + (uint32_t)std::min<uint64_t>((cost & 0xffffffffull) / PSET_TASK_WINDOWS, SCHED_NB - 1);
                return SCHED_RANK[kind] * SCHED_NB + (SCHED_NB - 1 - cost_bucket(cost));
        }

        struct PNode {
                uint32_t op = 0, term = 0;
                uint32_t tok = 0;
                uint32_t kid_off = 0, kid_n = 0;
                uint64_t cost = 0;
                bool empty = false;
        };

        struct Scratch {
                std::vector<PNode> nodes;
                std::vector<int> kidpool, st, tmpk;
                std::vector<uint64_t> cs;
                std::vector<uint32_t> gt, gs;
                std::vector<uint32_t> gorder, leaves, leaf_tok, negs, opts, opt_tok, ts, ts_tok, u, uniq, rt, seen, phterms, slots;
                struct PhraseTmp {
                        uint32_t t0, n;
                        double weight;
                };
                std::vector<PhraseTmp> qphrases;
                std::vector<std::pair<uint32_t, double>> sc;
                const int *kids(const PNode &x) const { return kidpool.data() + x.kid_off; }
        };

        struct Tmp {
                DevQuery q;
                uint64_t cost;
                uint32_t nlead;
                int32_t fz;
                bool truth;
                bool tree;
                bool hidden;
                uint64_t tree_ub;
                uint32_t hidden_ord;
                uint64_t sumdf, lead_docs;
                uint32_t last_doc;
                bool dense, fuse;
        };

        struct QUse {
                uint32_t qpos, term;
        };
        struct FUse {
                uint32_t fidx, slot, term;
        };

        struct Frag : PlanCounters {
                size_t q_lo = 0, q_hi = 0;
                Scratch S;
                std::vector<Tmp> tmp;
                std::vector<uint32_t> qterms, pterms, sterms;
                std::vector<double> sweights;
                std::vector<DevPhrase> phrases;
                std::vector<DevFused> fz;
                std::vector<size_t> left_out;
                uint64_t onepass_queries = 0, fused_postings = 0, phrase_queries = 0;
                std::vector<DevTask> tasks;
                std::vector<uint64_t> tcost;
                std::vector<DevFused> fused;
                std::vector<uint32_t> ptasks;
                std::vector<DevPsetUnit> units;
                std::vector<QUse> quses, suses;
                std::vector<FUse> fuses;
                std::vector<uint64_t> benefit;
                std::vector<uint64_t> cand_row;
                std::vector<uint32_t> keys, hist;
                std::vector<uint32_t> treepool;
                std::vector<uint32_t> tree_terms;
                uint32_t n_hidden = 0;
                uint64_t off = 0;
                size_t b_plan = 0, b_qterms = 0, b_sterms = 0, b_phrases = 0, b_pterms = 0, b_tasks = 0, b_fused = 0, b_ptasks = 0, b_units = 0, b_tree = 0, b_hidden = 0;
                uint64_t b_off = 0;
                int rc = TRI_OK;
                std::string err;
                void recycle() {
                        Frag fresh;
                        auto keep = [](auto &dst, auto &src) {
                                src.clear();
                                dst = std::move(src);
                        };
                        keep(fresh.S.nodes, S.nodes), keep(fresh.S.kidpool, S.kidpool), keep(fresh.S.st, S.st), keep(fresh.S.tmpk, S.tmpk), keep(fresh.S.cs, S.cs);
                        keep(fresh.S.gt, S.gt), keep(fresh.S.gs, S.gs), keep(fresh.S.gorder, S.gorder), keep(fresh.S.leaves, S.leaves), keep(fresh.S.leaf_tok, S.leaf_tok);
                        keep(fresh.S.negs, S.negs), keep(fresh.S.opts, S.opts), keep(fresh.S.opt_tok, S.opt_tok), keep(fresh.S.ts, S.ts), keep(fresh.S.ts_tok, S.ts_tok);
                        keep(fresh.S.u, S.u), keep(fresh.S.uniq, S.uniq), keep(fresh.S.rt, S.rt), keep(fresh.S.seen, S.seen), keep(fresh.S.phterms, S.phterms);
                        keep(fresh.S.slots, S.slots), keep(fresh.S.qphrases, S.qphrases), keep(fresh.S.sc, S.sc);
                        keep(fresh.tmp, tmp), keep(fresh.qterms, qterms), keep(fresh.pterms, pterms), keep(fresh.sterms, sterms), keep(fresh.sweights, sweights);
                        keep(fresh.phrases, phrases), keep(fresh.fz, fz), keep(fresh.left_out, left_out), keep(fresh.tasks, tasks), keep(fresh.tcost, tcost);
                        keep(fresh.fused, fused), keep(fresh.ptasks, ptasks), keep(fresh.units, units), keep(fresh.quses, quses), keep(fresh.suses, suses);
                        keep(fresh.fuses, fuses), keep(fresh.benefit, benefit), keep(fresh.cand_row, cand_row), keep(fresh.keys, keys), keep(fresh.hist, hist), keep(fresh.treepool, treepool);
                        keep(fresh.tree_terms, tree_terms);
                        *this = std::move(fresh);
                }
        };
        struct FragCache {
                std::vector<Frag> frags;
        };

        struct Ctx {
                const HostIndex &ix;
                const PlanEnv &env;
                const PlanInput &in;
                bool scored, rich;
                uint32_t mode;
                uint32_t n_ok = 0;
                bool plane_ok(uint32_t term) const { return ix.df_rank[term] < n_ok; }
                uint64_t planes_split = 2, fused_task_cost = 0, phrase_task_div = 1;
                uint32_t plw = 0;
                double term_weight(const uint32_t df) const {
                        if (in.similarity == TRI_SIM_TFIDF)
                                return std::log((double)((uint64_t)ix.info.docs_cnt + 1) / (double)(df + 1)) + 1.0;
                        if (in.similarity == TRI_SIM_TRIVIAL)
                                return 0.0;
                        const float num = (float)((uint64_t)ix.info.docs_cnt - (uint64_t)df) + 0.5f;
                        const float den = (float)df + 0.5f;
                        return (double)std::log(1 + num / den);
                }
                uint32_t first_block_ge(const DevTerm &t, const uint64_t key) const {
                        if (t.win_off != 0xffffffffu && !ix.win.empty() && !(key & (CELL_DOCS - 1)) && (key >> CELL_LOG2) < ix.nwin)
                                return ix.win[t.win_off + (key >> CELL_LOG2)];
                        const uint32_t *lb = &ix.blk_last[t.first_block];
                        return (uint32_t)(std::lower_bound(lb, lb + t.nblocks, (uint32_t)std::min<uint64_t>(key, 0xffffffffull)) - lb);
                }
        };

        inline uint64_t distinct_docbytes(const HostIndex &ix, const uint32_t *terms, const size_t n, std::vector<uint32_t> &seen) {
                uint64_t bytes = 0;
                seen.clear();
                for (size_t k = 0; k < n; ++k) {
// ... 46 lines not shown
```

### trinity_amd/csrc/trinity_hip.hip

```cpp
#include "../../include/trinity_hip.h"
#include <chrono>
#include <hip/hip_runtime.h>

#include <algorithm>
#include <array>
#include <cmath>
#include <cstdarg>
#include <cstdio>
#include <cstring>
#include <ctime>
#include <unistd.h>
#include <dlfcn.h>
#include <memory>
#include <mutex>
#include <numeric>
#include <string>
#include <thread>
#include <unordered_map>
#include <functional>
#include <vector>

static thread_local char g_err[512] = "";
static int fail(int code, const char *fmt, ...) {
        va_list ap;
// ... 934 lines not shown
                HIP_TRY(pool_alloc(dev, (void **)&b->d_part_docs, (nt * topk + 1) * 4));
                HIP_TRY(pool_alloc(dev, (void **)&b->d_part_scores, (nt * topk + 1) * 8));
        }
        if (b->n_tree) {
                const size_t plw = b->plw, nterms = b->tree_terms.size(), nhid = b->tree_hidden.size(), nchunks = (plw + TREE_CHUNK_WORDS - 1) / TREE_CHUNK_WORDS;
                const size_t w_rows = nterms * PL_PLANES * plw, w_prows = nhid * plw, w_qbits = (size_t)b->n_tree * plw, w_cc = (size_t)b->n_tree * nchunks + 64;
                HIP_TRY(pool_alloc(dev, (void **)&b->d_tree_scratch, (w_rows + w_prows + w_qbits + w_cc + 2 * nterms + 64) * 4));
                b->d_tree_rows = b->d_tree_scratch;
                b->d_tree_prows = b->d_tree_rows + w_rows;
                b->d_tree_qbits = b->d_tree_prows + w_prows;
                b->d_tree_cc = b->d_tree_qbits + w_qbits;
                b->d_tree_build = b->d_tree_cc + w_cc;
                std::vector<uint32_t> build(2 * nterms);
                for (size_t i = 0; i < nterms; ++i)
                        build[2 * i] = b->tree_terms[i], build[2 * i + 1] = (uint32_t)i;
                if (nterms)
                        HIP_TRY(hipMemcpyAsync(b->d_tree_build, build.data(), build.size() * 4, hipMemcpyHostToDevice, dev->stream_up));
                if (scored && topk)
                        HIP_TRY(pool_alloc(dev, (void **)&b->d_tree_scores, (off + 64) * 8));
        }
        HIP_TRY(hipEventRecord(b->ev[EV_UP], dev->stream_up));
        b->info.nqueries = nq;
        b->info.tree_queries = b->tree_queries;
        b->info.bitmap_queries = b->bitmap_queries;
        b->info.tree_scratch_bytes = b->tree_scratch_bytes;
        b->info.out_capacity = off;
        b->info.dense_queries = b->dense_queries;
        b->info.cand_queries = b->cand_queries;
        b->info.fused_queries = b->fused_queries;
        b->info.planes_queries = b->planes_queries;
        b->info.unsupported_queries = b->unsupported_queries;
        b->info.plane_terms = b->plane_terms.size();
        b->info.plane_bytes = (uint64_t)b->plane_terms.size() * (b->planes_hi ? PL_PLANES : 1u) * b->plw * 4;
        b->info.launches = (!b->plane_terms.empty()) + (!b->ptasks.empty()) + (rich ? 2 : 0) + ((scored && trip::sched_first(*b, TASK_FUSED)) ? 1 : 0) + ((scored && topk) ? 1 : 0);
        for (uint32_t kind = 0; kind < TASK_KINDS; ++kind)
                b->info.launches += kind != TASK_TREE && b.get()->*trip::SCHED_COUNT[kind];
        b->info.create_plan_ms = (float)(b->plan_ms[0] + b->plan_ms[1] + b->plan_ms[2] + b->plan_ms[3]);
        b->info.create_ms = (float)std::chrono::duration<double, std::milli>(std::chrono::steady_clock::now() - t_create).count();
        if (dbg_create)
                fprintf(stderr, "[tri create] nq %zu: plan %.3f  arena+copy %.3f  planes/sparse %.3f  out(%.1f MB) %.3f  rest %.3f  total %.3f ms\n", nq, dbg_t[0], dbg_t[1] - dbg_t[0],
                        dbg_t[2] - dbg_t[1], (double)off * 4 / 1e6, dbg_t[3] - dbg_t[2], b->info.create_ms - dbg_t[3], b->info.create_ms);
        *out = b.release();
        return TRI_OK;
}

extern "C" void tri_batch_destroy(tri_batch *b) {
        delete b;
}


static int run_plane_rows(tri_batch *b) {
        tri_dev *dev = b->dev;
        tri_index *ix = b->ix;
        b->info.term_planes_decoded_bytes = 0;
        if (!b->plane_terms.empty()) {
                std::vector<uint32_t> build;
                const uint8_t needs = b->planes_hi ? 3u : 1u;
                for (const uint32_t term : b->plane_terms) {
                        const uint32_t row = ix->df_rank[term];
                        if (row < ix->pc_cap && ((ix->pc_built[row] & needs) != needs || dev->opt.planes_rebuild)) {
                                build.push_back(term);
                                build.push_back(row);
                                b->info.term_planes_decoded_bytes += ix->docbytes[term];
                        }
                }
                if (!build.empty()) {
                        HIP_TRY(hipMemcpyAsync(b->d_build, build.data(), build.size() * 4, hipMemcpyHostToDevice, dev->stream));
                        const uint32_t nrows = (uint32_t)(build.size() / 2), nwin = b->plw / PL_WORDS;
                        for (uint32_t y0 = 0; y0 < nrows; y0 += 65535u) {
                                const uint32_t ny = std::min(65535u, nrows - y0);
                                if (b->planes_hi)
                                        TRI_LAUNCH(k_term_planes, ix->codec, dim3(nwin, ny), dim3(AND_WG), dev->stream, ix->d_index, ix->d_blk_last, ix->d_blk_off, ix->d_blk_rec,
                                                   ix->d_blk_doff, ix->d_win, ix->d_terms, (const uint32_t *)b->d_build + 2 * (size_t)y0, ix->d_pcache, (size_t)b->plw, ix->d_pcache_hi,
                                                   (size_t)PL_HI * b->plw, b->plw, (uint32_t *)nullptr);
                                else
                                        TRI_LAUNCH(k_term_plane0, ix->codec, dim3((nwin + P0_GROUP - 1) / P0_GROUP, ny), dim3(AND_WG), dev->stream, ix->d_index, ix->d_blk_last, ix->d_blk_off,
                                                   ix->d_blk_rec, ix->d_blk_doff, ix->d_win, ix->d_terms, (const uint32_t *)b->d_build + 2 * (size_t)y0, ix->d_pcache, b->plw, (uint32_t *)nullptr);
                                HIP_TRY(hipGetLastError());
                        }
                        for (size_t i = 1; i < build.size(); i += 2)
                                ix->pc_built[build[i]] |= needs;
                }
        }
        HIP_TRY(hipEventRecord(b->ev[EV_PLANE_ROWS], dev->stream));
        return TRI_OK;
}

static int run_matching(tri_batch *b) {
        tri_dev *dev = b->dev;
        tri_index *ix = b->ix;
        const uint8_t *match_bytes = ix->codec == TRI_CODEC_GOOGLE ? ix->d_dstream : ix->d_index;
        const uint32_t *match_off = ix->codec == TRI_CODEC_GOOGLE ? ix->d_blk_doff : ix->d_blk_off;
        uint32_t dense_wgs = TRI_DENSE_WAVES * 256 / DENSE_WG, cand_wgs = 4;
        bool overlap = false;
        if (dev->opt.overlap_dense_wgs && dev->opt.overlap_cand_wgs && (b->n_dense || b->n_pset) && b->n_cand) {
                overlap = true;
                dense_wgs = (uint32_t)dev->opt.overlap_dense_wgs;
                cand_wgs = (uint32_t)dev->opt.overlap_cand_wgs;
        } else if (dev->opt.overlap && b->n_cand && trip::sched_first(*b, TASK_CAND))
                overlap = true;
        hipStream_t cand_stream = dev->stream;
        if (overlap) {
                HIP_TRY(hipEventRecord(dev->ev_fork, dev->stream));
                HIP_TRY(hipStreamWaitEvent(dev->stream2, dev->ev_fork, 0));
                cand_stream = dev->stream2;
        }
        const DevPsetUnit *units = b->dev_at(b->units);
        const uint32_t *pset_sched = b->dev_at(b->pset_sched);
        const bool prep = b->n_pset && b->pscatter_queries, prep_forked = prep && !overlap && b->n_dense;
        if (prep) {
                if (prep_forked) {
                        HIP_TRY(hipEventRecord(dev->ev_fork, dev->stream));
                        HIP_TRY(hipStreamWaitEvent(dev->stream2, dev->ev_fork, 0));
                }
                hipStream_t prep_stream = prep_forked ? dev->stream2 : dev->stream;
                const uint32_t nunits = b->n_pset + b->n_probe, nscat = (uint32_t)b->pscatter_queries;
                hipLaunchKernelGGL(k_psets_prep_list, dim3((nunits + 255) / 256), dim3(256), 0, prep_stream, units, nunits, b->d_ticket + TICKET_SCAT_WORD + 1, b->d_scat_list, nscat);
                HIP_TRY(hipGetLastError());
                TRI_LAUNCH(k_psets_prep, ix->codec, dim3(nscat), dim3(PSCAT_WG), prep_stream, units, (const uint32_t *)b->d_scat_list, (const uint32_t *)(b->d_ticket + TICKET_SCAT_WORD + 1),
                           b->dev_at(b->plan), b->dev_at(b->tasks), (const uint32_t *)b->dev_at(b->qterms), (const uint32_t *)b->dev_opt(b->qplane), ix->d_masked, ix->d_index, ix->d_blk_last, ix->d_blk_off, ix->d_blk_rec,
                           ix->d_blk_doff, ix->d_terms, b->d_ticket + TICKET_SCAT_WORD, b->d_scat_off, b->d_scat_cnt, b->d_scat_docs, b->scat_cap);
                HIP_TRY(hipGetLastError());
                if (prep_forked)
                        HIP_TRY(hipEventRecord(dev->ev_join, dev->stream2));
        }
        if (b->n_dense) {
                TRI_LAUNCH(k_and_dense, ix->codec, dim3(std::min<uint32_t>(b->n_dense, (uint32_t)dev->cus * dense_wgs)), dim3(DENSE_WG), dev->stream, match_bytes, ix->d_blk_last,
                           match_off, ix->d_win, ix->d_terms, b->dev_at(b->plan), b->dev_at(b->tasks), b->dev_at(b->sched) + trip::sched_first(*b, TASK_DENSE), b->dev_at(b->qterms), b->n_dense,
                           b->d_ticket + TICKET_DENSE_WORD, b->d_out, b->d_counts, ix->d_masked, (const uint32_t *)b->dev_opt(b->qplane), (const uint32_t *)ix->d_pcache, b->plw);
                HIP_TRY(hipGetLastError());
        }
        HIP_TRY(hipEventRecord(b->ev[EV_DENSE], dev->stream));
        if (prep_forked)
                HIP_TRY(hipStreamWaitEvent(dev->stream, dev->ev_join, 0));
        if (b->n_pset) {
                const uint32_t pset_wgs = TRI_PSET_WAVES * 256 / PSET_WG;
                TRI_LAUNCH(k_psets, ix->codec, dim3(std::min<uint32_t>(b->n_pset, (uint32_t)dev->cus * (overlap && dev->opt.overlap_dense_wgs ? std::min<uint32_t>(dense_wgs, pset_wgs) : pset_wgs))),
                           dim3(PSET_WG), dev->stream, units, pset_sched, b->n_pset, b->d_ticket + TICKET_PSET_WORD, (const uint32_t *)b->dev_at(b->qterms), (const uint32_t *)b->dev_opt(b->qplane), b->d_out,
                           b->d_counts, ix->d_masked, (const uint32_t *)ix->d_pcache, b->plw, (const uint32_t *)b->d_scat_off, (const uint32_t *)b->d_scat_cnt,
                           (const uint32_t *)b->d_scat_docs);
                HIP_TRY(hipGetLastError());
        }
        HIP_TRY(hipEventRecord(b->ev[EV_PSET], dev->stream));
        if (b->n_probe) {
                TRI_LAUNCH(k_probe, ix->codec, dim3(std::min<uint32_t>((b->n_probe + PROBE_WG / 64 - 1) / (PROBE_WG / 64), (uint32_t)dev->cus * (TRI_PROBE_WAVES * 256 / PROBE_WG))),
                           dim3(PROBE_WG), dev->stream, match_bytes, ix->d_blk_last, match_off, ix->d_terms, units, pset_sched + b->n_pset, b->n_probe, b->d_ticket + TICKET_PROBE_WORD,
                           (const uint32_t *)b->dev_at(b->qterms), (const uint32_t *)b->dev_opt(b->qplane), b->d_out, b->d_counts, ix->d_masked, (const uint32_t *)ix->d_pcache, b->plw);
                HIP_TRY(hipGetLastError());
        }
        HIP_TRY(hipEventRecord(b->ev[EV_PROBE], dev->stream));
        if (b->n_cand)
                TRI_LAUNCH(k_and, ix->codec, dim3(std::min<uint32_t>(b->n_cand, (uint32_t)dev->cus * cand_wgs)), dim3(AND_WG), cand_stream, match_bytes, ix->d_blk_last, match_off,
                           ix->d_win, ix->d_terms, b->dev_at(b->plan), b->dev_at(b->tasks), b->dev_at(b->sched) + trip::sched_first(*b, TASK_CAND), b->dev_at(b->qterms), b->dev_at(b->cand_q),
                           b->d_ticket + TICKET_CAND_WORD, b->d_out, b->d_counts, ix->d_masked, (const uint32_t *)b->dev_opt(b->qplane), (const uint32_t *)ix->d_pcache, b->plw);
        HIP_TRY(hipGetLastError());
        if (overlap) {
                HIP_TRY(hipEventRecord(dev->ev_join, dev->stream2));
                HIP_TRY(hipStreamWaitEvent(dev->stream, dev->ev_join, 0));
        }
        HIP_TRY(hipEventRecord(b->ev[EV_CAND], dev->stream));
        return TRI_OK;
}

static int run_fused(tri_batch *b) {
        tri_dev *dev = b->dev;
        tri_index *ix = b->ix;
        for (uint32_t kind = TASK_FUSED; kind <= TASK_FUSED_GEN; ++kind) {
                const uint32_t nf = b->*trip::SCHED_COUNT[kind], variant = kind - TASK_FUSED;
                if (!nf)
                        continue;
                tri_launch(ix->codec, [&](auto c) { return std::array{k_fused<c.value, 0, 0>, k_fused<c.value, 1, 0>, k_fused<c.value, 0, 1>}[variant]; },
                           dim3(std::min<uint32_t>(nf, (uint32_t)dev->cus * FUS_WGS_PER_CU)), dim3(FUS_WG), dev->stream, ix->d_index, ix->d_blk_last, ix->d_blk_off, ix->d_blk_rec,
                           ix->d_blk_doff, ix->d_win, ix->d_terms, b->dev_at(b->plan), b->dev_at(b->fused), b->dev_at(b->tasks), (const uint32_t *)b->dev_at(b->sched) + trip::sched_first(*b, kind), b->dev_at(b->sterms),
                           b->dev_at(b->sweights), nf, b->d_ticket + TICKET_FUSED_WORD + 2 * variant, b->d_counts, b->topk, b->d_part_docs, b->d_part_scores, b->d_part_counts, ix->d_masked,
                           b->similarity, b->d_out, b->d_all_scores, b->d_rich_allow);
                HIP_TRY(hipGetLastError());
        }
        HIP_TRY(hipEventRecord(b->ev[EV_FUSED], dev->stream));
        return TRI_OK;
}

static int run_planes(tri_batch *b) {
        tri_dev *dev = b->dev;
        tri_index *ix = b->ix;
        if (b->d_qthr)
                HIP_TRY(hipMemsetAsync(b->d_qthr, 0, (b->plan.size() + 1) * 8, dev->stream));
        for (uint32_t kind = TASK_PLANES; kind <= TASK_PLANES8; ++kind) {
                const uint32_t np = b->*trip::SCHED_COUNT[kind], wide = kind - TASK_PLANES;
                if (!np)
                        continue;
                tri_launch(ix->codec, [&](auto c) { return wide ? k_planes<c.value, FUS_MAX_SLOTS> : k_planes<c.value, PLK_NS_SMALL>; },
                           dim3(std::min<uint32_t>(np, (uint32_t)dev->cus * PLK_WGS_PER_CU)), dim3(PLK_WG), dev->stream, ix->d_index, ix->d_blk_last, ix->d_blk_off, ix->d_blk_rec,
                           ix->d_blk_doff, ix->d_win, ix->d_terms, b->dev_at(b->plan), b->dev_at(b->fused), b->dev_at(b->tasks), (const uint32_t *)b->dev_at(b->sched) + trip::sched_first(*b, kind), b->dev_at(b->sterms),
                           b->dev_at(b->sweights), np, b->d_ticket + TICKET_PLANES_WORD + 2 * wide, b->d_counts, b->topk, b->d_part_docs, b->d_part_scores, b->d_part_counts, ix->d_masked,
                           b->similarity, (const uint32_t *)ix->d_pcache, (const uint32_t *)ix->d_pcache_hi, b->plw, ix->pc_cap, b->d_sparse, b->sparse_cap, b->d_qthr);
                HIP_TRY(hipGetLastError());
        }
        HIP_TRY(hipEventRecord(b->ev[EV_PLANES], dev->stream));
        return TRI_OK;
}

static int run_phrases(tri_batch *b) {
        tri_dev *dev = b->dev;
        tri_index *ix = b->ix;
        if (!b->ptasks.empty() && ix->codec == TRI_CODEC_GOOGLE && ix->d_prank && ix->pc_cap) {
                std::vector<uint32_t> hits_build, hits_only;
                uint32_t max_blocks = 0;
                for (size_t i = 0; i < b->pterms.size(); ++i) {
                        const uint32_t term = b->pterms[i], r = ix->df_rank[term];
                        if (r >= ix->pc_cap || ix->ph_built[r])
                                continue;
                        const DevTerm &t = ix->terms[term];
                        if (!(t.flags & TERM_FULL_BLOCKS) || !t.documents)
                                continue;
                        ix->ph_built[r] = 1;
                        max_blocks = std::max(max_blocks, t.nblocks);
                        std::vector<uint32_t> &dst = (ix->pc_built[r] & 4u) ? hits_only : hits_build;
                        ix->pc_built[r] |= 5u;
                        dst.push_back(term);
                        dst.push_back(r);
                }
                const uint32_t nrows_build = (uint32_t)(hits_build.size() / 2);
                hits_build.insert(hits_build.end(), hits_only.begin(), hits_only.end());
                if (!hits_build.empty()) {
                        uint32_t *d_pairs = ix->d_ph_pairs + 2 * ix->ph_pairs_n;
                        HIP_TRY(hipMemcpyAsync(d_pairs, hits_build.data(), hits_build.size() * 4, hipMemcpyHostToDevice, dev->stream));
                        ix->ph_pairs_n += hits_build.size() / 2;
                        for (uint32_t y0 = 0; y0 < nrows_build; y0 += 65535u) {
                                const dim3 grid((b->plw / PL_WORDS + P0_GROUP - 1) / P0_GROUP, std::min(65535u, nrows_build - y0));
                                TRI_LAUNCH(k_term_plane0, ix->codec, grid, dim3(AND_WG), dev->stream, ix->d_index, ix->d_blk_last, ix->d_blk_off, ix->d_blk_rec, ix->d_blk_doff, ix->d_win,
                                           ix->d_terms, (const uint32_t *)d_pairs + 2 * (size_t)y0, ix->d_pcache, b->plw, ix->d_prank);
                                HIP_TRY(hipGetLastError());
                        }
                        const uint32_t npairs = (uint32_t)(hits_build.size() / 2);
                        for (uint32_t y0 = 0; y0 < npairs; y0 += 65535u) {
                                hipLaunchKernelGGL(k_term_hits, dim3((max_blocks + 255) / 256, std::min(65535u, npairs - y0)), dim3(256), 0, dev->stream, ix->d_index, ix->d_blk_off,
                                                   ix->d_blk_hits, ix->d_terms, (const uint32_t *)d_pairs + 2 * (size_t)y0, (const uint64_t *)ix->d_hs_off, ix->d_phs, ix->d_term_row);
                                HIP_TRY(hipGetLastError());
                        }
                }
        }
        if (!b->ptasks.empty()) {
                const uint32_t np = (uint32_t)b->ptasks.size();
                TRI_LAUNCH(k_phrase, ix->codec, dim3(std::min<uint32_t>(np, (uint32_t)dev->cus * PHRASE_WGS_PER_CU)), dim3(AND_WG), dev->stream, ix->d_index, ix->d_hits,
                           ix->d_blk_hits, ix->d_hdir, ix->d_blk_last, ix->d_blk_off, ix->d_win, ix->d_terms, b->dev_at(b->plan), b->dev_at(b->tasks), b->dev_at(b->ptasks), np, b->dev_at(b->phrases), b->dev_at(b->pterms),
                           b->d_ticket + TICKET_PHRASE_WORD, b->d_out, b->d_counts, b->d_pscore,
                           (b->flags & TRI_FLAG_ACCUMULATED_SCORE) ? 65535u : 1u,
                           b->similarity, (const uint32_t *)ix->d_pcache, ix->pc_plw, (const uint32_t *)ix->d_prank, (const unsigned long long *)ix->d_phs,
                           (const uint64_t *)ix->d_hs_off, (const uint32_t *)(ix->codec == TRI_CODEC_GOOGLE ? ix->d_term_row : nullptr));
                HIP_TRY(hipGetLastError());
        }
        HIP_TRY(hipEventRecord(b->ev[EV_PHRASE], dev->stream));
        return TRI_OK;
}

static int run_trees(tri_batch *b) {
        tri_dev *dev = b->dev;
        tri_index *ix = b->ix;
        if (b->n_tree) {
                const uint32_t plw = b->plw, nterms = (uint32_t)b->tree_terms.size(), nhid = (uint32_t)b->tree_hidden.size();
                const uint32_t nchunks = (plw + TREE_CHUNK_WORDS - 1) / TREE_CHUNK_WORDS;
                const uint32_t *tsched = b->dev_at(b->sched) + trip::sched_first(*b, TASK_TREE);
                const uint32_t *d_tree = b->dev_at(b->tree);
                for (uint32_t y0 = 0; y0 < nterms; y0 += 65535u) {
                        const dim3 grid(plw / PL_WORDS, std::min(65535u, nterms - y0));
                        TRI_LAUNCH(k_term_planes, ix->codec, grid, dim3(AND_WG), dev->stream, ix->d_index, ix->d_blk_last, ix->d_blk_off, ix->d_blk_rec, ix->d_blk_doff, ix->d_win,
                                   ix->d_terms, (const uint32_t *)b->d_tree_build + 2 * (size_t)y0, b->d_tree_rows, (size_t)PL_PLANES * plw, b->d_tree_rows + plw,
                                   (size_t)PL_PLANES * plw, plw, (uint32_t *)nullptr);
                        HIP_TRY(hipGetLastError());
                }
                if (nhid) {
                        HIP_TRY(hipMemsetAsync(b->d_tree_prows, 0, (size_t)nhid * plw * 4, dev->stream));
                        hipLaunchKernelGGL(k_tree_gather, dim3(nhid), dim3(TREE_WG), 0, dev->stream, b->dev_at(b->plan), b->dev_at(b->tasks), b->dev_at(b->tree_hidden), b->d_out,
                                           b->d_counts, b->d_pscore, b->d_tree_prows, plw);
                        HIP_TRY(hipGetLastError());
                }
                const bool scored_run = b->flags & TRI_FLAG_ACCUMULATED_SCORE, rich_run = b->flags & TRI_FLAG_MATCHED_TERMS;
                double *tscores = scored_run ? (b->topk ? b->d_tree_scores : b->d_all_scores) : nullptr;
                for (uint32_t y0 = 0; y0 < b->n_tree; y0 += 65535u) {
                        const dim3 grid(nchunks, std::min(65535u, b->n_tree - y0));
                        uint32_t *qbits = b->d_tree_qbits + (size_t)y0 * plw, *cc = b->d_tree_cc + (size_t)y0 * nchunks;
                        hipLaunchKernelGGL(k_tree_eval, grid, dim3(TREE_WG), 0, dev->stream, b->dev_at(b->plan), b->dev_at(b->tasks), tsched + y0, d_tree, (const uint32_t *)b->d_tree_rows,
                                           (const uint32_t *)b->d_tree_prows, (const uint32_t *)ix->d_masked, qbits, cc, plw);
                        hipLaunchKernelGGL(k_tree_expand, grid, dim3(TREE_WG), 0, dev->stream, b->dev_at(b->plan), b->dev_at(b->tasks), tsched + y0, (const uint32_t *)qbits, (const uint32_t *)cc,
                                           b->d_out, b->d_counts, plw);
                        if (scored_run || rich_run)
                                TRI_LAUNCH(k_tree_leaves, ix->codec, grid, dim3(TREE_WG), dev->stream, ix->d_index, ix->d_blk_last, ix->d_blk_off, ix->d_terms, b->dev_at(b->plan), b->dev_at(b->tasks),
                                           tsched + y0, d_tree, (const uint32_t *)b->d_tree_rows, (const uint32_t *)b->d_tree_prows, (const uint32_t *)cc, (const uint32_t *)b->d_out,
                                           (const uint32_t *)b->d_counts, (const double *)b->dev_at(b->sweights), (const double *)b->d_pscore, tscores, rich_run ? b->d_rich_allow : nullptr,
                                           plw, b->similarity);
                        HIP_TRY(hipGetLastError());
                }
                if (scored_run && b->topk) {
                        hipLaunchKernelGGL(k_tree_topk, dim3(b->n_tree), dim3(AND_WG), 0, dev->stream, tsched, b->dev_at(b->tasks), (const uint32_t *)b->d_out, (const uint32_t *)b->d_counts,
                                           (const double *)tscores, b->topk, b->d_part_docs, b->d_part_scores, b->d_part_counts);
                        HIP_TRY(hipGetLastError());
                }
        }
        HIP_TRY(hipEventRecord(b->ev[EV_TREE], dev->stream));
        return TRI_OK;
}

template <bool WRITE>
static int launch_rich(tri_batch *b) {
        tri_dev *dev = b->dev;
        tri_index *ix = b->ix;
        const uint32_t n = (uint32_t)b->tasks.size();
// ... 64 lines not shown
                HIP_TRY(hipMemcpyToSymbol(HIP_SYMBOL(g_trace), &dptr, sizeof dptr));
        }
        memset(g_trace_host, 0, 64 * 16);
#endif
        b->ran = true;
#ifdef TRI_TASKTIMES
        if (b->tasks.size()) {
                if (g_tt_cap < 8 * (size_t)b->tasks.size()) {
                        if (g_tt_host)
                                hipHostFree(g_tt_host);
                        g_tt_cap = 8 * (size_t)b->tasks.size() + 1024;
                        HIP_TRY(hipHostMalloc((void **)&g_tt_host, g_tt_cap * 8, hipHostMallocMapped | hipHostMallocCoherent));
                        unsigned long long *dptr = nullptr;
                        HIP_TRY(hipHostGetDevicePointer((void **)&dptr, g_tt_host, 0));
                        HIP_TRY(hipMemcpyToSymbol(HIP_SYMBOL(g_tt), &dptr, sizeof dptr));
                }
                memset(g_tt_host, 0, g_tt_cap * 8);
        }
#endif
        HIP_TRY(hipStreamWaitEvent(dev->stream, b->ev[EV_UP], 0));
        if (b->ix->ev_pc_ready)
                HIP_TRY(hipStreamWaitEvent(dev->stream, b->ix->ev_pc_ready, 0));
        HIP_TRY(hipEventRecord(b->ev[EV_START], dev->stream));
        if (b->tasks.empty()) {
                for (int e = EV_PLANE_ROWS; e <= EV_TREE; ++e)
                        HIP_TRY(hipEventRecord(b->ev[e], dev->stream));
        } else {
                HIP_TRY(hipMemsetAsync(b->d_ticket, 0, TICKET_BYTES, dev->stream));
                for (int (*stage)(tri_batch *) : {run_plane_rows, run_matching, run_fused, run_planes, run_phrases, run_trees, run_rich_count, run_scores})
                        if (const int rc = stage(b))
                                return rc;
        }
        if (const int rc = run_query_counts(b))
                return rc;
        HIP_TRY(hipEventRecord(b->ev[EV_END], dev->stream));
        return TRI_OK;
}

#ifdef TRI_TASKTIMES
static void report_tasktimes(tri_batch *b) {
        const tri_dev *dev = b->dev;
        if (!b->tasks.size() || !getenv("TRINITY_TASKTIMES"))
                return;
#if TRI_TASKTIMES == 2
        const uint32_t nc = trip::sched_first(*b, TASK_FUSED), first = 0;
#elif TRI_TASKTIMES == 5
        const uint32_t nc = (uint32_t)b->ptasks.size(), first = 0;
#elif TRI_TASKTIMES == 4
        const uint32_t nc = b->n_dense, first = trip::sched_first(*b, TASK_DENSE);
#elif TRI_TASKTIMES == 3
        const uint32_t nc = b->n_planes, first = trip::sched_first(*b, TASK_PLANES);
#else
        const uint32_t nc = b->n_cand, first = trip::sched_first(*b, TASK_CAND);
#endif
        unsigned long long t0 = ~0ull, t1 = 0, busy = 0;
        std::vector<std::pair<unsigned long long, uint32_t>> by;
        for (uint32_t i = 0; i < nc; ++i) {
                const unsigned long long s = g_tt_host[8 * i], e = g_tt_host[8 * i + 1];
                if (!s || !e)
                        continue;
                t0 = std::min(t0, s), t1 = std::max(t1, e);
                busy += e - s;
                by.emplace_back(e - s, i);
        }
        std::sort(by.rbegin(), by.rend());
        const double span_us = (double)(t1 - t0) / 100.0;
        const unsigned wgs = std::min<uint32_t>(nc, (uint32_t)dev->cus * (TRI_TASKTIMES == 3 ? PLK_WGS_PER_CU : TRI_TASKTIMES == 2 ? SCORE_WGS_PER_CU : TRI_TASKTIMES == 5 ? PHRASE_WGS_PER_CU : 4));
        fprintf(stderr, "[tri tasktimes] k_and: %u tasks, span %.1f us, busy %.1f %% of %u workgroups; mean task %.2f us\n", nc, span_us,
                100.0 * (double)busy / ((double)(t1 - t0) * wgs), wgs, (double)busy / 100.0 / std::max<size_t>(1, by.size()));
        if (!by.empty()) {
                auto at = [&](double f) { return (double)by[std::min(by.size() - 1, (size_t)(f * by.size()))].first / 100.0; };
                unsigned long long top1 = 0, top5 = 0, top20 = 0;
                for (size_t i = 0; i < by.size(); ++i) {
                        if (i < by.size() / 100)
                                top1 += by[i].first;
                        if (i < by.size() / 20)
                                top5 += by[i].first;
                        if (i < by.size() / 5)
                                top20 += by[i].first;
                }
                fprintf(stderr, "   task us: max %.1f  p99 %.1f  p90 %.1f  p50 %.1f  p10 %.1f; the longest 1 %% / 5 %% / 20 %% of the tasks take %.1f / %.1f / %.1f %% of the time\n", at(0), at(0.01), at(0.1),
                        at(0.5), at(0.9), 100.0 * top1 / busy, 100.0 * top5 / busy, 100.0 * top20 / busy);
        }
        for (const double f : {0.25, 0.5, 0.75, 0.9}) {
                const unsigned long long at = t0 + (unsigned long long)((double)(t1 - t0) * f);
                unsigned running = 0;
                for (uint32_t i = 0; i < nc; ++i)
                        running += g_tt_host[8 * i] <= at && g_tt_host[8 * i + 1] > at;
                fprintf(stderr, "   at %2.0f %% of the span: %u tasks running\n", f * 100, running);
        }
#if TRI_TASKTIMES == 3
        {
                const char *nm[8] = {"", "", "setup+lists", "phase A", "prune+tables", "sweep", "drain", "end"};
                double sum[8] = {0};
                std::vector<double> span[8];
                for (uint32_t i = 0; i < nc; ++i) {
                        unsigned long long prev = g_tt_host[8 * i];
                        for (int j = 2; j <= 7; ++j) {
                                const unsigned long long at = j == 7 ? g_tt_host[8 * i + 1] : g_tt_host[8 * i + j];
                                if (!at || !prev)
                                        continue;
                                const double d = (double)(at - prev) / 100.0;
                                sum[j] += d;
                                span[j].push_back(d);
                                prev = at;
                        }
                }
                fprintf(stderr, "   phases (us per task: mean / median / p90):");
                for (int j = 2; j <= 7; ++j)
                        if (!span[j].empty()) {
                                std::sort(span[j].begin(), span[j].end());
                                fprintf(stderr, "  %s %.1f / %.1f / %.1f", nm[j], sum[j] / span[j].size(), span[j][span[j].size() / 2], span[j][span[j].size() * 9 / 10]);
                        }
                fprintf(stderr, "\n");
                double tsum[9][2] = {}, ssum[9][2] = {}, asum[9][2] = {};
                unsigned tcnt[9][2] = {};
                for (uint32_t i = 0; i < nc; ++i) {
                        const unsigned long long s0 = g_tt_host[8 * i], e0 = g_tt_host[8 * i + 1];
                        if (!s0 || !e0)
                                continue;
                        const DevTask &tk = b->tasks[b->sched[first + i]];
                        const DevFused &z = b->fused[b->plan[tk.slot].fused_idx];
                        uint32_t nd = 0;
                        for (uint32_t k = 0; k < z.nslots; ++k)
                                nd += z.plane[k] != PL_NONE;
                        const int sp = nd < z.nslots;
                        nd = std::min(nd, 8u);
                        tsum[nd][sp] += (double)(e0 - s0) / 100.0;
                        if (g_tt_host[8 * i + 5] > g_tt_host[8 * i + 4] && g_tt_host[8 * i + 4])
                                ssum[nd][sp] += (double)(g_tt_host[8 * i + 5] - g_tt_host[8 * i + 4]) / 100.0;
                        if (g_tt_host[8 * i + 3] > g_tt_host[8 * i + 2] && g_tt_host[8 * i + 2])
                                asum[nd][sp] += (double)(g_tt_host[8 * i + 3] - g_tt_host[8 * i + 2]) / 100.0;
                        ++tcnt[nd][sp];
                }
                for (uint32_t nd = 0; nd <= 8; ++nd)
                        for (int sp = 0; sp < 2; ++sp)
                                if (tcnt[nd][sp])
                                        fprintf(stderr, "   %u dense slots%s: %u tasks, %.1f %% of the time; per task %.1f us (sweep %.1f, phase A %.1f)\n", nd, sp ? " + sparse" : "          ",
                                                tcnt[nd][sp], 100.0 * tsum[nd][sp] * 100.0 / (double)busy, tsum[nd][sp] / tcnt[nd][sp], ssum[nd][sp] / tcnt[nd][sp], asum[nd][sp] / tcnt[nd][sp]);
        }
#endif
#if TRI_TASKTIMES == 1
        {
                double sum[8] = {0}, cnt[8] = {0};
                for (uint32_t i = 0; i < nc; ++i)
                        for (int j = 1; j < 8; ++j)
                                if (g_tt_host[8 * i + j] && g_tt_host[8 * i])
                                        sum[j] += (double)(g_tt_host[8 * i + j] - g_tt_host[8 * i]) / 100.0, cnt[j] += 1;
                fprintf(stderr, "   means over the tasks (us after the task's start): end %.1f  last tile's lead decoded %.1f", sum[1] / std::max(1.0, cnt[1]), sum[2] / std::max(1.0, cnt[2]));
                for (int j = 3; j < 8; ++j)
                        if (cnt[j])
                                fprintf(stderr, "  term %d %.1f (%.0f tasks)", j - 2, sum[j] / cnt[j], cnt[j]);
                fprintf(stderr, "\n");
        }
#endif
        for (size_t k = 0; k < std::min<size_t>(12, by.size()); ++k) {
#if TRI_TASKTIMES == 5
                const uint32_t ti = b->ptasks[by[k].second];
#else
                const uint32_t ti = b->sched[first + by[k].second];
#endif
                const DevTask &tk = b->tasks[ti];
                const DevQuery &q = b->plan[tk.slot];
                std::string tt;
                char buf[96];
                if (task_onepass(tk.kind)) {
                        const DevFused &z = b->fused[q.fused_idx];
                        for (uint32_t j = 0; j < z.nslots; ++j) {
                                snprintf(buf, sizeof buf, " %u(df %u%s)", z.term[j], b->ix->terms[z.term[j]].documents, z.plane[j] != PL_NONE ? " plane" : "");
                                tt += buf;
                        }
                        snprintf(buf, sizeof buf, " nreq %u", z.nreq);
                        tt += buf;
                } else
                for (uint32_t j = 0; j < q.nterms; ++j) {
                        const uint32_t term = b->qterms[q.term_base + j] & QT_TERM;
                        snprintf(buf, sizeof buf, " %s%u(df %u%s)", (b->qterms[q.term_base + j] & QT_GROUP) ? "|" : "", term, b->ix->terms[term].documents,
                                 (!b->qplane.empty() && b->qplane[q.term_base + j] != PL_NONE) ? " plane" : "");
                        tt += buf;
                }
                snprintf(buf, sizeof buf, "  matches %u phrases %u", b->h_counts.empty() ? 0u : b->h_counts[ti], q.nphrases);
                tt += buf;
                fprintf(stderr, "   %.1f us (started %.1f us in)  ticket %u  tiles [%u, %u)  query %u:%s\n", (double)by[k].first / 100.0,
                        (double)(g_tt_host[8 * by[k].second] - t0) / 100.0, by[k].second, tk.tile_begin, tk.tile_end, q.qid, tt.c_str());
                fprintf(stderr, "        last tile: lead decoded +%.1f us", ((double)g_tt_host[8 * by[k].second + 2] - (double)g_tt_host[8 * by[k].second]) / 100.0);
                for (int j = 3; j < 8; ++j)
                        if (g_tt_host[8 * by[k].second + j])
                                fprintf(stderr, "  term %d +%.1f", j - 2, ((double)g_tt_host[8 * by[k].second + j] - (double)g_tt_host[8 * by[k].second]) / 100.0);
                fprintf(stderr, "\n");
        }
}
#endif

static void read_stage_times(tri_batch *b) {
        static const struct { BatchEvent from; float tri_batch_info::*ms; } STAGES[] = {
                {EV_START, &tri_batch_info::term_planes_ms}, {EV_PLANE_ROWS, &tri_batch_info::dense_ms}, {EV_DENSE, &tri_batch_info::pset_ms}, {EV_PSET, &tri_batch_info::probe_ms},
                {EV_PROBE, &tri_batch_info::cand_ms}, {EV_CAND, &tri_batch_info::fused_ms}, {EV_FUSED, &tri_batch_info::planes_ms}, {EV_PLANES, &tri_batch_info::phrase_ms},
                {EV_PHRASE, &tri_batch_info::tree_ms}, {EV_TREE, &tri_batch_info::rest_ms}};
        float ms = 0;
        if (hipEventElapsedTime(&ms, b->ev[EV_START], b->ev[EV_END]) == hipSuccess)
                b->info.last_run_ms = ms;
        for (const auto &s : STAGES) {
                b->info.*s.ms = 0;
                if (!b->tasks.empty() && hipEventElapsedTime(&ms, b->ev[s.from], b->ev[s.from + 1]) == hipSuccess)
                        b->info.*s.ms = ms;
        }
}

static int account_matches(tri_batch *b) {
        b->h_counts.resize(b->tasks.size());
        if (!b->tasks.empty())
                HIP_TRY(hipMemcpy(b->h_counts.data(), b->d_counts, b->tasks.size() * 4, hipMemcpyDeviceToHost));
        const bool sc = b->flags & TRI_FLAG_ACCUMULATED_SCORE;
        uint64_t m = 0, m_kind[TASK_KINDS] = {}, out_kind[TASK_KINDS] = {};
        b->h_query_counts.assign(b->plan.size(), 0);
        for (size_t sidx = 0; sidx < b->plan.size(); ++sidx) {
                const DevQuery &q = b->plan[sidx];
                for (uint32_t t = 0; t < q.ntasks; ++t)
                        b->h_query_counts[sidx] += b->h_counts[q.first_task + t];
                if (q.qid == 0xffffffffu)
                        continue;
                const uint64_t c = b->h_query_counts[sidx];
                m += c;
                if (!q.ntasks)
                        continue;
                const uint32_t kind = b->tasks[q.first_task].kind;
                m_kind[kind] += c;
                if (task_onepass(kind))
                        out_kind[kind] += q.out_cap ? 4 * c : 8 * std::min<uint64_t>(c, b->topk);
                else if (kind != TASK_TREE)
                        out_kind[kind] += sc && b->topk ? 8 * std::min<uint64_t>(c, b->topk) : (kind == TASK_DENSE || kind == TASK_PSET) && q.form == RESULT_BITMAP ? 4ull * q.out_cap : 4 * c;
        }
        const uint64_t out_fused = out_kind[TASK_FUSED] + out_kind[TASK_FUSED16] + out_kind[TASK_FUSED_GEN], out_planes = out_kind[TASK_PLANES] + out_kind[TASK_PLANES8];
        b->info.dense_algorithmic_bytes = b->term_bytes_dense + 4 * m_kind[TASK_DENSE];
        b->info.pset_algorithmic_bytes = b->term_bytes_pset + 4 * m_kind[TASK_PSET];
        b->info.pset_queries = b->pset_queries;
        b->info.probe_algorithmic_bytes = b->term_bytes_probe + 4 * m_kind[TASK_PROBE];
        b->info.probe_queries = b->probe_queries;
        b->info.cand_algorithmic_bytes = (b->term_bytes - b->term_bytes_dense - b->term_bytes_pset - b->term_bytes_probe - b->term_bytes_fused - b->term_bytes_planes - b->term_bytes_phrase_hits) + 4 * m_kind[TASK_CAND];
        b->info.planes_algorithmic_bytes = b->term_bytes_planes + out_planes;
        b->info.phrase_algorithmic_bytes = b->term_bytes_phrase_hits;
        b->info.phrase_queries = 0;
        for (const DevQuery &q : b->plan)
                b->info.phrase_queries += q.nphrases != 0;
        b->info.cand_needed_bytes = b->cand_needed_term_bytes ? b->cand_needed_term_bytes + 4 * (m_kind[TASK_CAND] + m_kind[TASK_PROBE]) : 0;
        b->info.fused_algorithmic_bytes = b->term_bytes_fused + out_fused;
        b->info.matches = m;
        if (b->distinct_bytes) {
                b->info.pset_bound_bytes = b->distinct_bytes_kind[TASK_PSET] + out_kind[TASK_PSET];
                b->info.probe_bound_bytes = b->distinct_bytes_kind[TASK_PROBE] + out_kind[TASK_PROBE];
                b->info.dense_bound_bytes = b->distinct_bytes_kind[TASK_DENSE] + out_kind[TASK_DENSE];
                b->info.cand_bound_bytes = b->distinct_bytes_kind[TASK_CAND] + out_kind[TASK_CAND];
                b->info.fused_bound_bytes = b->distinct_bytes_kind[TASK_FUSED] + b->distinct_bytes_kind[TASK_FUSED16] + b->distinct_bytes_kind[TASK_FUSED_GEN] + out_fused;
                b->info.planes_bound_bytes = b->distinct_bytes_kind[TASK_PLANES] + b->distinct_bytes_kind[TASK_PLANES8] + out_planes;
                b->info.phrase_bound_bytes = b->distinct_bytes_kind[TASK_KINDS];
                b->info.bound_bytes = b->distinct_bytes;
                for (const uint64_t o : out_kind)
                        b->info.bound_bytes += o;
        }
        if (sc) {
                uint64_t outb = 0;
                for (uint64_t c : b->h_query_counts)
                        outb += 8 * std::min<uint64_t>(c, b->topk);
                b->info.algorithmic_bytes = b->term_bytes + outb;
        } else
                b->info.algorithmic_bytes = b->term_bytes + 4 * m;
        return TRI_OK;
}

static int rich_write_pass(tri_batch *b) {
        if (!(b->flags & TRI_FLAG_MATCHED_TERMS) || b->tasks.empty())
                return TRI_OK;
        tri_dev *dev = b->dev;
        const size_t nt = b->tasks.size();
        std::vector<uint32_t> th(nt);
        HIP_TRY(hipMemcpy(th.data(), b->d_task_hits, nt * 4, hipMemcpyDeviceToHost));
        b->h_task_pos_base.assign(nt + 1, 0);
        for (size_t i = 0; i < nt; ++i)
                b->h_task_pos_base[i + 1] = b->h_task_pos_base[i] + th[i];
        const size_t total = b->h_task_pos_base[nt];
        if (total + 64 > b->rich_pool_cap) {
                hipFree(b->d_rich_pool);
                b->d_rich_pool = nullptr;
                b->rich_pool_cap = total + total / 8 + 64;
                HIP_TRY(hipMalloc((void **)&b->d_rich_pool, b->rich_pool_cap * 2));
                if (b->flags & TRI_FLAG_HIT_PAYLOADS) {
                        hipFree(b->d_rich_plen);
                        hipFree(b->d_rich_payload);
                        b->d_rich_plen = nullptr;
                        b->d_rich_payload = nullptr;
                        HIP_TRY(hipMalloc((void **)&b->d_rich_plen, b->rich_pool_cap));
                        HIP_TRY(hipMalloc((void **)&b->d_rich_payload, b->rich_pool_cap * 8));
                }
        }
        HIP_TRY(hipMemcpy(b->d_task_pos_base, b->h_task_pos_base.data(), (nt + 1) * 8, hipMemcpyHostToDevice));
        HIP_TRY(hipMemsetAsync(b->d_ticket + TICKET_RICH_WRITE_WORD, 0, 4, dev->stream));
        if (const int rc = launch_rich<true>(b))
                return rc;
        HIP_TRY(hipStreamSynchronize(dev->stream));
        b->info.algorithmic_bytes += 2 * total + 4 * b->info.matches;
        return TRI_OK;
}

extern "C" int tri_batch_sync(tri_batch *b) {
        if (!b)
                return fail(TRI_ERR_INVALID, "null batch");
// ... 684 lines not shown
```

### trinity_amd/hostplan.py

```python
import ctypes as C

import numpy as np

from .engine import TrinityError, flatten, host_lib

_SUMMARY = ["block_bytes", "n_plan", "n_qterms", "n_tasks", "n_fused_maps", "n_qplane", "n_plane_terms", "n_sterms", "n_sweights", "n_phrases", "n_pterms", "n_ptasks",
            "off_plan", "off_qterms", "off_tasks", "off_sched", "off_fused", "off_qplane", "off_plane_terms", "off_sterms", "off_sweights", "off_phrases", "off_pterms", "off_ptasks",
            "n_dense", "n_cand", "n_fused", "n_fused16", "n_fusedgen", "n_planes", "n_planes8", "plw", "sparse_cap", "out_capacity", "term_bytes", "term_bytes_dense",
            "dense_queries", "cand_queries", "fused_queries", "planes_queries", "unsupported_queries", "rich_R", "sizeof_query", "sizeof_task", "sizeof_fused", "sizeof_phrase",
            "cand_needed_term_bytes", "plane_decoded_bytes", "n_pset", "pset_queries", "n_probe", "probe_queries", "n_units", "off_units", "off_unit_sched", "sizeof_unit",
            "n_tree", "tree_queries", "n_tree_words", "off_tree", "n_tree_terms", "off_tree_terms", "n_tree_hidden", "off_tree_hidden", "off_cand_q"]

DEV_QUERY = np.dtype([("nterms", "<u4"), ("term_base", "<u4"), ("out_off", "<u8"), ("out_cap", "<u4"), ("qid", "<u4"), ("first_task", "<u4"), ("ntasks", "<u4"),
                      ("score_base", "<u4"), ("nscore", "<u4"), ("phrase_base", "<u4"), ("nphrases", "<u4"), ("fused_idx", "<u4"), ("form", "<u4")])
DEV_TASK = np.dtype([("slot", "<u4"), ("begin", "<u4"), ("end", "<u4"), ("kind", "<u4"), ("out_off", "<u8")])
TASK_CAND, TASK_DENSE, TASK_FUSED, TASK_FUSED16, TASK_FUSED_GEN, TASK_PLANES, TASK_PLANES8, TASK_PSET, TASK_PROBE, TASK_TREE = range(10)
DEV_TREE_NODE = np.dtype([("op", "u1"), ("parent", "u1"), ("ord", "u1"), ("thr", "u1"), ("arg", "<u4"), ("row", "<u4"), ("score", "<u4"), ("rmask", "<u4"),
                          ("kid0", "u1"), ("kid1", "u1"), ("pad", "u1", 2), ("kids", "<u8")])
TREE_HDR_WORDS = 8
DEV_UNIT = np.dtype([("out_off", "<u8"), ("begin", "<u4"), ("end", "<u4"), ("tix", "<u4"), ("nterms", "<u4"), ("term_base", "<u4"), ("first", "<u4"), ("tt", "<u4", 4), ("row", "<u4", 4)])
SCHED_ORDER = [TASK_DENSE, TASK_PSET, TASK_PROBE, TASK_CAND, TASK_FUSED, TASK_FUSED16, TASK_FUSED_GEN, TASK_PLANES, TASK_PLANES8, TASK_TREE]


def _lib():
    L = host_lib()
    if not hasattr(L, "_plan_ready"):
        vp = C.c_void_p
        L.tri_host_index_build.restype = vp
        L.tri_host_index_build.argtypes = [vp, C.c_uint64, vp, C.c_uint64, C.c_int, vp, C.c_uint64, C.c_uint32, C.c_char_p, C.c_uint64]
        L.tri_host_index_free.argtypes = [vp]
        L.tri_host_plan.restype = vp
        L.tri_host_plan.argtypes = [vp, vp, C.c_uint64, vp, C.c_uint64, C.c_uint32, C.c_uint32, C.c_int, C.c_uint, vp, vp, C.c_uint, C.c_uint32, C.c_char_p, C.c_uint64]
        L.tri_host_plan_free.argtypes = [vp]
        L.tri_host_plan_summary.argtypes = [vp, vp, vp]
        L.tri_host_plan_block.restype = C.POINTER(C.c_uint8)
        L.tri_host_plan_block.argtypes = [vp]
        L.tri_host_plan_query_maps.argtypes = [vp, vp, vp]
        L.tri_host_pfor128_group.argtypes = [vp, vp, C.POINTER(C.c_uint32), vp, C.POINTER(C.c_uint32)]
        L.tri_host_pfor128_group.restype = None
        for f in (L.tri_host_lucene_encode, L.tri_host_lucene_encode_units):
            f.argtypes = [vp, vp, vp, vp, C.c_uint64, vp, C.c_uint64, C.POINTER(C.c_uint64), vp, C.c_uint64, C.POINTER(C.c_uint64), vp]
        L._plan_ready = True
    return L


class HostIndex:
    def __init__(self, index_bytes, terms, docs_cnt, codec=1, hits=None):
        b = np.ascontiguousarray(index_bytes, dtype=np.uint8)
        t = np.ascontiguousarray(terms, dtype=np.uint32).reshape(-1, 3)
        h = np.ascontiguousarray(hits, dtype=np.uint8) if hits is not None and len(hits) else None
        err = C.create_string_buffer(600)
        self.h = _lib().tri_host_index_build(b.ctypes.data, b.size, h.ctypes.data if h is not None else None, h.size if h is not None else 0, codec, t.ctypes.data, t.shape[0],
                                             docs_cnt, err, 600)
        if not self.h:
            raise TrinityError(err.value.decode())

    @classmethod
    def from_segment(cls, seg):
        return cls(seg.index, seg.terms, seg.docs_cnt, codec=seg.codec, hits=seg.hits)

    def close(self):
        if self.h:
            _lib().tri_host_index_free(self.h)
            self.h = None

    def __del__(self):
        self.close()


class HostPlan:

    def __init__(self, hindex, programs, flags, topk=0, similarity=0, threads=1, options=None, cus=256, flat=None):
        self.nq = len(programs) if flat is None else flat[1].shape[0]
        prog, q = flatten(programs) if flat is None else flat
        options = options or {}
        names = (C.c_char_p * max(1, len(options)))(*[k.encode() for k in options])
        values = np.array(list(options.values()) or [0], dtype=np.uint64)
        err = C.create_string_buffer(600)
        self.h = _lib().tri_host_plan(hindex.h, prog.ctypes.data, prog.size, q.ctypes.data, self.nq, flags, topk, similarity, threads, names, values.ctypes.data, len(options), cus,
                                      err, 600)
        if not self.h:
            raise TrinityError(err.value.decode())
        out = np.zeros(len(_SUMMARY), dtype=np.uint64)
        ms = np.zeros(4, dtype=np.float64)
        _lib().tri_host_plan_summary(self.h, out.ctypes.data, ms.ctypes.data)
        self.s = {k: int(v) for k, v in zip(_SUMMARY, out)}
        self.ms = ms
        assert self.s["sizeof_query"] == DEV_QUERY.itemsize and self.s["sizeof_task"] == DEV_TASK.itemsize
        p = _lib().tri_host_plan_block(self.h)
        self.block = np.ctypeslib.as_array(p, shape=(max(1, self.s["block_bytes"]),)).copy()
        self.slot_of_query = np.zeros(max(1, self.nq), dtype=np.uint32)
        self.qstatus = np.zeros(max(1, self.nq), dtype=np.int32)
        _lib().tri_host_plan_query_maps(self.h, self.slot_of_query.ctypes.data, self.qstatus.ctypes.data)

    def _view(self, off, n, dtype):
        dt = np.dtype(dtype)
        return self.block[self.s[off] : self.s[off] + n * dt.itemsize].view(dt)

    @property
    def plan(self):
        return self._view("off_plan", self.s["n_plan"], DEV_QUERY)

    @property
    def tasks(self):
        return self._view("off_tasks", self.s["n_tasks"], DEV_TASK)

    @property
    def sched(self):
        return self._view("off_sched", self.s["n_tasks"], "<u4")

    @property
    def units(self):
        return self._view("off_units", self.s["n_units"], DEV_UNIT)

    @property
    def unit_sched(self):
        return self._view("off_unit_sched", self.s["n_pset"] + self.s["n_probe"], "<u4")

    @property
    def cand_q(self):
        return self._view("off_cand_q", 9, "<u4")

    @property
    def qterms(self):
        return self._view("off_qterms", self.s["n_qterms"], "<u4")

    @property
    def qplane(self):
        return self._view("off_qplane", self.s["n_qplane"], "<u4")

    @property
    def plane_terms(self):
        return self._view("off_plane_terms", self.s["n_plane_terms"], "<u4")

    @property
    def tree_terms(self):
        return self._view("off_tree_terms", self.s["n_tree_terms"], "<u4")

    @property
    def tree_hidden(self):
        return self._view("off_tree_hidden", self.s["n_tree_hidden"], "<u4")

    def tree_nodes(self, slot):
        words = self._view("off_tree", self.s["n_tree_words"], "<u4")
        at = int(self.plan[slot]["fused_idx"])
        n = int(words[at])
        return words[at + TREE_HDR_WORDS : at + TREE_HDR_WORDS + 8 * n].view(DEV_TREE_NODE)

    def close(self):
        if self.h:
            self.block = None
            _lib().tri_host_plan_free(self.h)
            self.h = None

    def __del__(self):
        self.close()


def pfor128_group_pair(v):
    v = np.ascontiguousarray(v, dtype=np.uint32)
    assert v.size == 128
    a, b = np.zeros(700, dtype=np.uint8), np.zeros(700, dtype=np.uint8)
    al, bl = C.c_uint32(), C.c_uint32()
    _lib().tri_host_pfor128_group(v.ctypes.data, a.ctypes.data, C.byref(al), b.ctypes.data, C.byref(bl))
    return a[: al.value] if al.value != 0xFFFFFFFF else None, b[: bl.value]


def lucene_encode(docs, freqs, positions, term_first, units=False):
    d = np.ascontiguousarray(docs, dtype=np.uint32)
    f = np.ascontiguousarray(freqs, dtype=np.uint32)
    p = np.ascontiguousarray(positions, dtype=np.uint16)
    tf = np.ascontiguousarray(term_first, dtype=np.uint64)
    n = tf.size - 1
    icap, hcap = 128 + 16 * n + 12 * d.size, 128 + 6 * p.size + 8 * n
    io, ho, t3 = np.zeros(icap, dtype=np.uint8), np.zeros(hcap, dtype=np.uint8), np.zeros((max(n, 1), 3), dtype=np.uint32)
    il, hl = C.c_uint64(), C.c_uint64()
    fn = _lib().tri_host_lucene_encode_units if units else _lib().tri_host_lucene_encode
    if fn(d.ctypes.data, f.ctypes.data, p.ctypes.data, tf.ctypes.data, n, io.ctypes.data, icap, C.byref(il), ho.ctypes.data, hcap, C.byref(hl), t3.ctypes.data):
        raise TrinityError("lucene_encode: buffer too small")
    return io[: il.value], ho[: hl.value], t3[:n]


def cpu_budget():
    L = host_lib()
    L.tri_host_cpu_budget.restype = C.c_uint32
    return int(L.tri_host_cpu_budget())


def pool_cpus(threads=16):
    L = host_lib()
    L.tri_host_pool_cpus.restype = C.c_uint32
    L.tri_host_pool_cpus.argtypes = [C.c_uint32, C.c_void_p, C.c_uint32]
    out = np.zeros(256, dtype=np.int32)
    n = L.tri_host_pool_cpus(threads, out.ctypes.data, out.size)
    return out[:n].tolist()
```

Before: 14.53 million.

## Run small candidate AND tasks per wave instead of per workgroup

Adds a wave-granular path for candidate AND tasks whose lead term has at most 64 blocks. Each wave decodes its own quarter-tile of candidates into a private LDS slice and filters it with wave-local barriers, so one workgroup can run four such tasks at once. The planner puts these tasks into a dedicated last bucket per queue and passes per-queue wave-task counts to the kernel. The aim is to stop paying full workgroup barriers and idle lanes on tiny tasks, at the cost of extra scheduling complexity and possible imbalance among waves.

```diff
diff --git a/trinity_amd/csrc/dev_stream.hpp b/trinity_amd/csrc/dev_stream.hpp
--- a/trinity_amd/csrc/dev_stream.hpp
+++ b/trinity_amd/csrc/dev_stream.hpp
@@ -87,6 +87,12 @@
 #define TASKTIME_PLANES(i)
 #define TASKTIME_DENSE(i)
 #define TASKTIME_PHRASE(i)
+#endif
+
+#if defined(TRI_TASKTIMES) && TRI_TASKTIMES == 1
+#define TASKTIME_WAVE(i) do { if ((threadIdx.x & 63u) == 0) g_tt[(i)] = wall_clock64(); } while (0)
+#else
+#define TASKTIME_WAVE(i)
 #endif
 
 #ifdef TRI_TRACE
diff --git a/trinity_amd/csrc/dev_structs.hpp b/trinity_amd/csrc/dev_structs.hpp
--- a/trinity_amd/csrc/dev_structs.hpp
+++ b/trinity_amd/csrc/dev_structs.hpp
@@ -56,6 +56,7 @@
 constexpr uint32_t CAND_QUEUES = 8;
 constexpr uint32_t CAND_TICKET_STRIDE = 16;
 constexpr uint32_t CAND_HEAVY_TILES = 3;
+constexpr uint32_t CAND_WAVE_BLOCKS = 64;
 constexpr uint32_t TASK_CAND = 0;
 constexpr uint32_t TASK_DENSE = 1;
 constexpr uint32_t TASK_FUSED = 2;
diff --git a/trinity_amd/csrc/host/plan_host.cpp b/trinity_amd/csrc/host/plan_host.cpp
--- a/trinity_amd/csrc/host/plan_host.cpp
+++ b/trinity_amd/csrc/host/plan_host.cpp
@@ -105,8 +105,8 @@
                               P.unsupported_queries, P.rich_R,       sizeof(DevQuery),     sizeof(DevTask), sizeof(DevFused),     sizeof(DevPhrase),  P.cand_needed_term_bytes, P.plane_decoded_bytes,
                               P.n_pset,            P.pset_queries,   P.n_probe,            P.probe_queries, P.units.size(),       P.units.off,        P.pset_sched.off,     sizeof(DevPsetUnit),
                               P.n_tree,            P.tree_queries,   P.tree.size(),        P.tree.off,      P.tree_terms.size(),  P.tree_terms.off,   P.tree_hidden.size(), P.tree_hidden.off,
-                              P.cand_q.off};
-        static_assert(sizeof v / sizeof v[0] == 65, "summary layout");
+                              P.cand_q.off,        P.cand_w.off};
+        static_assert(sizeof v / sizeof v[0] == 66, "summary layout");
         memcpy(out, v, sizeof v);
         if (ms)
                 memcpy(ms, P.plan_ms, sizeof P.plan_ms);
diff --git a/trinity_amd/csrc/k_match.hpp b/trinity_amd/csrc/k_match.hpp
--- a/trinity_amd/csrc/k_match.hpp
+++ b/trinity_amd/csrc/k_match.hpp
@@ -115,7 +115,12 @@
         return block_bytes32_finish(p, r, v);
 }
 
-__device__ __forceinline__ uint32_t cand_gallop(const AndShared &sh, uint32_t ptr, const uint32_t C, const uint32_t doc) {
+struct CandView {
+        uint32_t *cand;
+        uint32_t *hit;
+};
+
+__device__ __forceinline__ uint32_t cand_gallop(const CandView &sh, uint32_t ptr, const uint32_t C, const uint32_t doc) {
         uint32_t step = 1, lo = ptr;
         while (lo + step <= C && sh.cand[phys(lo + step - 1)] < doc) {
                 lo += step;
@@ -133,7 +138,7 @@
 }
 
 template <int CODEC, bool PRE>
-__device__ __forceinline__ void merge_block(AndShared &sh, const uint8_t *__restrict__ index, const DevTerm &t, const uint32_t b, const uint32_t off,
+__device__ __forceinline__ void merge_block(const CandView &sh, const uint8_t *__restrict__ index, const DevTerm &t, const uint32_t b, const uint32_t off,
                                             const uint32_t n, const uint32_t prev, const uint32_t last, uint32_t ptr, uint32_t cv, const uint32_t C,
                                             const uint32_t (&raw)[9]) {
         uint32_t doc = prev;
@@ -213,6 +218,89 @@
 }
 
 template <int CODEC>
+__device__ __forceinline__ void and_filter_cand_driven(const CandView &sh, const uint8_t *__restrict__ index, const uint32_t *__restrict__ bl,
+                                                       const uint32_t *__restrict__ bo, const uint32_t *__restrict__ win, const DevTerm &t, const uint32_t C,
+                                                       const uint32_t idx, const uint32_t stride) {
+        uint32_t carry = 0xffffffffu;
+        uint32_t wcur = 0;
+        for (uint32_t base = 0; base < C; base += stride) {
+                TRACE(20, base, C);
+                const uint32_t j = base + idx;
+                uint32_t bj = 0xffffffffu;
+                uint32_t cv = 0;
+                const uint32_t wbase = base + (idx & ~63u);
+                uint32_t rlo = 0, rhi = 0;
+                if (t.win_off != 0xffffffffu) {
+                        if (j < C) {
+                                const uint32_t c = sh.cand[phys(j)] >> CELL_LOG2;
+                                rlo = win[t.win_off + c];
+                                rhi = win[t.win_off + c + 1];
+                        }
+                } else if (wbase < C) {
+                        const uint32_t nval = min(64u, C - wbase);
+                        const uint32_t klo = sh.cand[phys(wbase)], khi = sh.cand[phys(wbase + nval - 1)];
+                        rlo = wave_lower_bound(bl, wcur, t.nblocks, klo);
+                        rhi = wave_lower_bound(bl, rlo, t.nblocks, khi);
+                        wcur = rlo;
+                }
+                if (j < C) {
+                        cv = sh.cand[phys(j)];
+                        uint32_t lo = rlo, hi = rhi;
+                        while (lo < hi) {
+                                const uint32_t mid = (lo + hi) >> 1;
+                                if (bl[mid] < cv)
+                                        lo = mid + 1;
+                                else
+                                        hi = mid;
+                        }
+                        bj = lo;
+                }
+                uint32_t prevb = __shfl_up(bj, 1, 64);
+                if ((idx & 63u) == 0)
+                        prevb = carry;
+                carry = __shfl(bj, 63, 64);
+                if (j < C && bj < t.nblocks && bj != prevb) {
+                        const uint32_t prev = bj ? bl[bj - 1] : 0;
+                        const uint32_t none[9] = {};
+                        merge_block<CODEC, false>(sh, index, t, bj, bo[bj], TRI_BLOCK_N(t, bj, index, bo[bj]), prev, bl[bj], j, cv, C, none);
+                }
+        }
+}
+
+template <int CODEC>
+__device__ __forceinline__ void filter_block(const CandView &sh, const uint8_t *__restrict__ index, const DevTerm &t, const uint32_t b, const uint32_t off,
+                                             const uint32_t prev, const uint32_t last, const uint32_t C, const bool full, const uint32_t (&raw)[9] PROF_ARG) {
+        uint32_t lo = 0, hi = C;
+        while (lo < hi) {
+                const uint32_t mid = (lo + hi) >> 1;
+                if (sh.cand[phys(mid)] <= prev)
+                        lo = mid + 1;
+                else
+                        hi = mid;
+        }
+        const uint32_t ptr = lo;
+        const uint32_t cv = ptr < C ? sh.cand[phys(ptr)] : 0xffffffffu;
+        PROF_LAP(6);
+        if (cv <= last) {
+                if (full)
+                        merge_block<CODEC, true>(sh, index, t, b, off, 32, prev, last, ptr, cv, C, raw);
+                else
+                        merge_block<CODEC, false>(sh, index, t, b, off, TRI_BLOCK_N(t, b, index, off), prev, last, ptr, cv, C, raw);
+        }
+        PROF_LAP(7);
+}
+
+__device__ __forceinline__ bool and_block_driven(const DevTerm &t, const DevTerm &lead) {
+#if defined(TRI_FORCE_CAND)
+        return false;
+#elif defined(TRI_FORCE_BLOCK)
+        return true;
+#else
+        return t.nblocks <= lead.documents;
+#endif
+}
+
+template <int CODEC>
 __device__ void and_filter_tile(AndShared &sh, const uint8_t *__restrict__ index, const uint32_t *__restrict__ blk_last,
                                 const uint32_t *__restrict__ blk_off, const uint32_t *__restrict__ win, const DevTerm t, const uint32_t C,
                                 const uint32_t lcur_slot, const bool block_driven PROF_ARG) {
@@ -220,6 +308,7 @@
         const uint32_t *bl = blk_last + t.first_block;
         const uint32_t *bo = blk_off + t.first_block;
         const uint32_t cmin = sh.cand[phys(0)], cmax = sh.cand[phys(C - 1)];
+        const CandView view{sh.cand, sh.hit};
 
         if (block_driven) {
                 uint32_t lcur = uni(sh.lcur[lcur_slot]);
@@ -275,26 +364,8 @@
                         }
                         if (b < t.nblocks) {
                                 beyond = last >= cmax;
-                                if (prev < cmax) {
-                                        uint32_t lo = 0, hi = C;
-                                        while (lo < hi) {
-                                                const uint32_t mid = (lo + hi) >> 1;
-                                                if (sh.cand[phys(mid)] <= prev)
-                                                        lo = mid + 1;
-                                                else
-                                                        hi = mid;
-                                        }
-                                        uint32_t ptr = lo;
-                                        uint32_t cv = ptr < C ? sh.cand[phys(ptr)] : 0xffffffffu;
-                                        PROF_LAP(6);
-                                        if (cv <= last) {
-                                                if (full)
-                                                        merge_block<CODEC, true>(sh, index, t, b, off, 32, prev, last, ptr, cv, C, raw);
-                                                else
-                                                        merge_block<CODEC, false>(sh, index, t, b, off, TRI_BLOCK_N(t, b, index, off), prev, last, ptr, cv, C, raw);
-                                        }
-                                        PROF_LAP(7);
-                                }
+                                if (prev < cmax)
+                                        filter_block<CODEC>(view, index, t, b, off, prev, last, C, full, raw PROF_PASS);
                         }
                         sh.scan[4 + (tid >> 6)] = __ballot(beyond) != 0ull;
                         __syncthreads();
@@ -305,50 +376,7 @@
                                 break;
                 }
         } else {
-                uint32_t carry = 0xffffffffu;
-                uint32_t wcur = 0;
-                for (uint32_t base = 0; base < C; base += AND_WG) {
-                        TRACE(20, base, C);
-                        const uint32_t j = base + tid;
-                        uint32_t bj = 0xffffffffu;
-                        uint32_t cv = 0;
-                        const uint32_t wbase = base + (tid & ~63u);
-                        uint32_t rlo = 0, rhi = 0;
-                        if (t.win_off != 0xffffffffu) {
-                                if (j < C) {
-                                        const uint32_t c = sh.cand[phys(j)] >> CELL_LOG2;
-                                        rlo = win[t.win_off + c];
-                                        rhi = win[t.win_off + c + 1];
-                                }
-                        } else if (wbase < C) {
-                                const uint32_t nval = min(64u, C - wbase);
-                                const uint32_t klo = sh.cand[phys(wbase)], khi = sh.cand[phys(wbase + nval - 1)];
-                                rlo = wave_lower_bound(bl, wcur, t.nblocks, klo);
-                                rhi = wave_lower_bound(bl, rlo, t.nblocks, khi);
-                                wcur = rlo;
-                        }
-                        if (j < C) {
-                                cv = sh.cand[phys(j)];
-                                uint32_t lo = rlo, hi = rhi;
-                                while (lo < hi) {
-                                        const uint32_t mid = (lo + hi) >> 1;
-                                        if (bl[mid] < cv)
-                                                lo = mid + 1;
-                                        else
-                                                hi = mid;
-                                }
-                                bj = lo;
-                        }
-                        uint32_t prevb = __shfl_up(bj, 1, 64);
-                        if ((tid & 63u) == 0)
-                                prevb = carry;
-                        carry = __shfl(bj, 63, 64);
-                        if (j < C && bj < t.nblocks && bj != prevb) {
-                                const uint32_t prev = bj ? bl[bj - 1] : 0;
-                                const uint32_t none[9] = {};
-                                merge_block<CODEC, false>(sh, index, t, bj, bo[bj], TRI_BLOCK_N(t, bj, index, bo[bj]), prev, bl[bj], j, cv, C, none);
-                        }
-                }
+                and_filter_cand_driven<CODEC>(view, index, bl, bo, win, t, C, tid, AND_WG);
         }
 }
 
@@ -918,6 +946,106 @@
         PROF_FLUSH();
 }
 
+__device__ __forceinline__ void wave_lds_sync() {
+        __builtin_amdgcn_fence(__ATOMIC_RELEASE, "workgroup");
+        __builtin_amdgcn_wave_barrier();
+        __builtin_amdgcn_fence(__ATOMIC_ACQUIRE, "workgroup");
+}
+typedef __attribute__((address_space(3))) uint32_t lds_u32_t;
+template <class T>
+__device__ __forceinline__ T *uniptr(T *p) {
+        const uint64_t v = (uint64_t)(uintptr_t)p;
+        return (T *)(uintptr_t)((uint64_t)uni((uint32_t)v) | ((uint64_t)uni((uint32_t)(v >> 32)) << 32));
+}
+#ifndef TRI_AND_WAVE_FN
+#define TRI_AND_WAVE_FN __forceinline__
+#endif
+template <int CODEC>
+__device__ TRI_AND_WAVE_FN void and_wave_task(AndShared &sh, const uint8_t *__restrict__ index_, const uint32_t *__restrict__ blk_last_, const uint32_t *__restrict__ blk_off_,
+                                              const uint32_t *__restrict__ win_, const DevTerm *__restrict__ terms_, const DevQuery *__restrict__ plan_,
+                                              const DevTask *__restrict__ tasks_, const uint32_t *__restrict__ qterms_, uint32_t *__restrict__ out_,
+                                              uint32_t *__restrict__ counts_, const uint32_t *__restrict__ masked_, const uint32_t tix_ PROF_ARG) {
+        const uint8_t *__restrict__ index = uniptr(index_);
+        const uint32_t *__restrict__ blk_last = uniptr(blk_last_), *__restrict__ blk_off = uniptr(blk_off_), *__restrict__ win = uniptr(win_), *__restrict__ qterms = uniptr(qterms_),
+                                    *__restrict__ masked = uniptr(masked_);
+        const DevTerm *__restrict__ terms = uniptr(terms_);
+        const DevQuery *__restrict__ plan = uniptr(plan_);
+        const DevTask *__restrict__ tasks = uniptr(tasks_);
+        uint32_t *__restrict__ out = uniptr(out_), *__restrict__ counts = uniptr(counts_);
+        const uint32_t tix = uni(tix_);
+        const uint32_t lane = threadIdx.x & 63u, wave = uni(threadIdx.x >> 6);
+        const CandView view{(uint32_t *)((lds_u32_t *)sh.cand + wave * (TILE_CANDS / (AND_WG / 64))), (uint32_t *)((lds_u32_t *)sh.hit + wave * 64)};
+        static_assert(CAND_WAVE_BLOCKS * 32 == TILE_CANDS / (AND_WG / 64) && CAND_WAVE_BLOCKS == 64, "a wave task's candidates: a row per lane, a quarter of the tile");
+        const DevTask task = tasks[tix];
+        const DevQuery q = plan[task.slot];
+        const DevTerm lead = terms[qterms[q.term_base] & QT_TERM];
+        const uint32_t nb = min(lead.nblocks, CAND_WAVE_BLOCKS);
+        const uint32_t C = (nb - 1) * 32 + lead.last_n;
+        wave_lds_sync();
+        if (lane < nb) {
+                const uint32_t gb = lead.first_block + lane;
+                const uint32_t off = blk_off[gb];
+                const uint32_t n = TRI_BLOCK_N(lead, lane, index, off);
+                const uint32_t last = blk_last[gb];
+                uint32_t doc = lane ? blk_last[gb - 1] : 0;
+                DeltaStream<CODEC> s;
+                s.init(index, lead, lane, off);
+                const uint32_t row = lane * 32;
+                for (uint32_t i = 0; i + 1 < n; ++i) {
+                        doc += s.next();
+                        view.cand[row | ((i + lane) & 31u)] = doc;
+                }
+                view.cand[row | ((n - 1 + lane) & 31u)] = last;
+        }
+        wave_lds_sync();
+        const uint32_t left = C > lane * 32 ? C - lane * 32 : 0u;
+        uint32_t alive = left >= 32 ? 0xffffffffu : ((1u << left) - 1u);
+        const uint32_t cmin = view.cand[phys(0)], cmax = view.cand[phys(C - 1)];
+        for (uint32_t k = 1; k < q.nterms && __ballot(alive != 0u) != 0ull; ++k) {
+                const DevTerm t = terms[qterms[q.term_base + k] & QT_TERM];
+                const uint32_t *bl = blk_last + t.first_block;
+                const uint32_t *bo = blk_off + t.first_block;
+                view.hit[lane] = 0;
+                wave_lds_sync();
+                if (and_block_driven(t, lead)) {
+                        for (uint32_t cb = wave_lower_bound(bl, 0, t.nblocks, cmin); cb < t.nblocks; cb += 64) {
+                                const uint32_t b = cb + lane;
+                                bool beyond = true;
+                                if (b < t.nblocks) {
+                                        const uint32_t prev = b ? bl[b - 1] : 0, last = bl[b], off = bo[b];
+                                        beyond = last >= cmax;
+                                        if (prev < cmax) {
+                                                const uint32_t none[9] = {};
+                                                filter_block<CODEC>(view, index, t, b, off, prev, last, C, false, none PROF_PASS);
+                                        }
+                                }
+                                if (__ballot(beyond) != 0ull)
+                                        break;
+                        }
+                } else
+                        and_filter_cand_driven<CODEC>(view, index, bl, bo, win, t, C, lane, 64u);
+                wave_lds_sync();
+                alive &= view.hit[lane];
+        }
+        if (masked)
+                for (uint32_t m = alive; m;) {
+                        const uint32_t kbit = __builtin_ctz(m);
+                        m &= m - 1;
+                        const uint32_t doc = view.cand[phys(lane * 32 + kbit)];
+                        if ((masked[doc >> 5] >> (doc & 31u)) & 1u)
+                                alive &= ~(1u << kbit);
+                }
+        uint32_t total;
+        uint32_t o = wave_excl_scan(__popc(alive), total);
+        uint32_t *qout = out + task.out_off;
+        for (uint32_t m = alive; m;) {
+                const uint32_t kbit = __builtin_ctz(m);
+                m &= m - 1;
+                qout[o++] = view.cand[phys(lane * 32 + kbit)];
+        }
+        counts[tix] = total;
+}
+
 #ifndef TRI_AND_PROBES
 #define TRI_AND_PROBES 8
 #endif
@@ -931,7 +1059,7 @@
                                                 const DevTerm *__restrict__ terms,
                                                 const DevQuery *__restrict__ plan, const DevTask *__restrict__ tasks,
                                                 const uint32_t *__restrict__ sched, const uint32_t *__restrict__ qterms,
-                                                const uint32_t *__restrict__ cand_q, uint32_t *__restrict__ ticket,
+                                                const uint32_t *__restrict__ cand_q, const uint32_t *__restrict__ cand_w, uint32_t *__restrict__ ticket,
                                                 uint32_t *__restrict__ out, uint32_t *__restrict__ counts,
                                                 const uint32_t *__restrict__ masked, const uint32_t *__restrict__ qplane,
                                                 const uint32_t *__restrict__ planes, const uint32_t plw) {
@@ -949,7 +1077,7 @@
                                 const uint32_t x = (home + t) % CAND_QUEUES;
                                 if ((qdone >> x) & 1u)
                                         continue;
-                                const uint32_t q0 = cand_q[x], qn = cand_q[x + 1] - q0;
+                                const uint32_t q0 = cand_q[x], qn = cand_q[x + 1] - q0 - cand_w[x];
                                 const uint32_t old = uni(atomicAdd(ticket + x * CAND_TICKET_STRIDE, 1u)) >> 6;
                                 if (old < qn)
                                         got = q0 + old;
@@ -1018,13 +1146,7 @@
                                         gneg = tt & QT_NOT;
                                 }
                                 __syncthreads();
-#if defined(TRI_FORCE_CAND)
-                                const bool bd = false;
-#elif defined(TRI_FORCE_BLOCK)
-                                const bool bd = true;
-#else
-                                const bool bd = t.nblocks <= lead.documents;
-#endif
+                                const bool bd = and_block_driven(t, lead);
                                 TRACE(3, slot, (k << 16) | (bd ? 1 : 0));
                                 const uint32_t prow = qplane ? qplane[q.term_base + k] : PL_NONE;
                                 if (prow != PL_NONE) {
@@ -1151,6 +1273,27 @@
                 TRACE(5, slot, produced);
         }
         PROF_LAP(15);
+        __syncthreads();
+        for (uint32_t wdone = 0;;) {
+                uint32_t got = 0xffffffffu;
+                for (uint32_t t = 0; t < CAND_QUEUES && got == 0xffffffffu; ++t) {
+                        const uint32_t x = (home + t) % CAND_QUEUES;
+                        if ((wdone >> x) & 1u)
+                                continue;
+                        const uint32_t wn = cand_w[x];
+                        const uint32_t old = wn ? uni(atomicAdd(ticket + x * CAND_TICKET_STRIDE + 1, 1u)) >> 6 : 0u;
+                        if (old < wn)
+                                got = cand_q[x + 1] - wn + old;
+                        else
+                                wdone |= 1u << x;
+                }
+                if (got == 0xffffffffu)
+                        break;
+                TASKTIME_WAVE(8 * got);
+                and_wave_task<CODEC>(sh, index, blk_last, blk_off, win, terms, plan, tasks, qterms, out, counts, masked, sched[got] PROF_PASS);
+                TASKTIME_WAVE(8 * got + 1);
+        }
+        PROF_LAP(9);
         PROF_FLUSH();
         TRACE(6, 0, 0);
 }
diff --git a/trinity_amd/csrc/planner.hpp b/trinity_amd/csrc/planner.hpp
--- a/trinity_amd/csrc/planner.hpp
+++ b/trinity_amd/csrc/planner.hpp
@@ -40,6 +40,7 @@
                 std::vector<RowQ> rowq;
                 uint32_t pset_ranges = 0;
                 uint32_t cand_first = 0, cand_qat[CAND_QUEUES] = {};
+                uint32_t cand_wn[CAND_QUEUES] = {};
                 std::vector<uint32_t> unit_of_task;
                 ~PlanState() {
                         if (!cache)
@@ -219,7 +220,7 @@
                                         const uint32_t x = (uint32_t)(std::min_element(load, load + CAND_QUEUES) - load);
                                         load[x] += cand_row[r] / z.n;
                                         z.q[k] = (uint8_t)x;
-                                        z.sub[k] = (uint8_t)(CAND_COST_SUBS + placed[x]++ % (CAND_SUBS - CAND_COST_SUBS - 1));
+                                        z.sub[k] = (uint8_t)(CAND_COST_SUBS + placed[x]++ % CAND_ROW_SUBS);
                                 }
                         }
                 }
@@ -363,7 +364,23 @@
                 const uint32_t rb = S.pset_ranges <= PSET_RANGE_BKS ? std::min(range, PSET_RANGE_BKS - 1) : (uint32_t)std::min<uint64_t>((uint64_t)range * PSET_RANGE_BKS / S.pset_ranges, PSET_RANGE_BKS - 1);
                 return PSET_KEY0 + rb * PSET_SUBS + pset_sub((uint32_t)(f.tcost[i] >> 32));
         }
+        inline bool cand_wave_task(const HostIndex &ix, const BatchPlan &P, const DevTask &tk) {
+                const DevQuery &q = P.plan[tk.slot];
+                if (tk.kind != TASK_CAND || q.ntasks != 1 || tk.tile_begin != 0 || tk.tile_end != 1 || q.nterms < 2)
+                        return false;
+                const uint32_t lead_blocks = ix.terms[P.qterms[q.term_base] & QT_TERM].nblocks;
+                if (lead_blocks == 0 || lead_blocks > CAND_WAVE_BLOCKS)
+                        return false;
+                for (uint32_t k = 1; k < q.nterms; ++k) {
+                        const uint32_t tt = P.qterms[q.term_base + k];
+                        if (!(tt & QT_GROUP) || (tt & QT_NOT) || (!P.qplane.empty() && P.qplane[q.term_base + k] != PL_NONE))
+                                return false;
+                }
+                return true;
+        }
         inline uint32_t key_cand_rows(const PlanState &S, const Frag &f, const size_t i, const DevTask &tk) {
+                if (cand_wave_task(S.ix, S.P, tk))
+                        return CAND_KEY0 + (uint32_t)(f.b_tasks + i) % CAND_QUEUES * CAND_SUBS + CAND_WAVE_SUB;
                 const DevQuery &q = S.P.plan[tk.slot];
                 uint32_t row = PL_NONE;
                 for (uint32_t k = 1; k < q.nterms && row == PL_NONE; ++k)
@@ -376,7 +393,7 @@
                         const uint32_t piece = (uint32_t)(f.b_tasks + i) % z.n;
                         queue = z.q[piece], sub = z.sub[piece];
                 } else
-                        queue = row % CAND_QUEUES, sub = CAND_SUBS - 1;
+                        queue = row % CAND_QUEUES, sub = CAND_STRAGGLER_SUB;
                 return CAND_KEY0 + queue * CAND_SUBS + sub;
         }
         inline uint32_t schedule_key(const PlanState &S, const Frag &f, const size_t i) {
@@ -429,7 +446,10 @@
                                 for (uint32_t bk = CAND_KEY0; bk < PSET_KEY0; ++bk) {
                                         if ((bk - CAND_KEY0) % CAND_SUBS == 0)
                                                 S.cand_qat[(bk - CAND_KEY0) / CAND_SUBS] = at;
+                                        const uint32_t bucket_first = at;
                                         place(bk);
+                                        if ((bk - CAND_KEY0) % CAND_SUBS == CAND_WAVE_SUB)
+                                                S.cand_wn[(bk - CAND_KEY0) / CAND_SUBS] = at - bucket_first;
                                 }
                         for (uint32_t k = 0; k < TASK_KINDS; ++k)
                                 if (SCHED_RANK[k] == r)
@@ -454,13 +474,20 @@
                 if (S.cand_rows) {
                         for (uint32_t x = 0; x <= CAND_QUEUES; ++x)
                                 P.cand_q[x] = x < CAND_QUEUES ? S.cand_qat[x] - S.cand_first : nc;
+                        for (uint32_t x = 0; x < CAND_QUEUES; ++x)
+                                P.cand_w[x] = S.cand_wn[x];
                 } else {
-                        const std::vector<uint32_t> was(sc, sc + nc);
+                        std::vector<uint32_t> was(sc, sc + nc);
+                        const uint32_t nwg = (uint32_t)(std::stable_partition(was.begin(), was.end(), [&](const uint32_t ti) { return !cand_wave_task(S.ix, P, P.tasks[ti]); }) - was.begin());
                         uint32_t pos = 0;
                         for (uint32_t x = 0; x < CAND_QUEUES; ++x) {
                                 P.cand_q[x] = pos;
-                                for (uint32_t i = x; i < nc; i += CAND_QUEUES)
+                                uint32_t nw = 0;
+                                for (uint32_t i = x; i < nc; i += CAND_QUEUES) {
                                         sc[pos++] = was[i];
+                                        nw += i >= nwg;
+                                }
+                                P.cand_w[x] = nw;
                         }
                         P.cand_q[CAND_QUEUES] = pos;
                 }
diff --git a/trinity_amd/csrc/planner_types.hpp b/trinity_amd/csrc/planner_types.hpp
--- a/trinity_amd/csrc/planner_types.hpp
+++ b/trinity_amd/csrc/planner_types.hpp
@@ -122,6 +122,7 @@
         Span<uint32_t> tree;
         Span<uint32_t> tree_terms;
         Span<uint32_t> tree_hidden;
+        Span<uint32_t> cand_w;
         uint32_t n_tree = 0;
         uint64_t tree_scratch_bytes = 0;
         std::vector<uint32_t> slot_of_query;
@@ -163,6 +164,7 @@
                 fn(P.tree, n.tree);
                 fn(P.tree_terms, n.tree_terms);
                 fn(P.tree_hidden, n.tree_hidden);
+                fn(P.cand_w, (size_t)CAND_QUEUES);
         }
         inline size_t layout_sections(BatchPlan &P, const SectionCounts &n) {
                 size_t bytes = 0;
@@ -178,7 +180,9 @@
         }
 
         constexpr uint32_t SCHED_NB = 64 * 4;
-        constexpr uint32_t CAND_SUBS = 128, CAND_COST_SUBS = 16;
+        constexpr uint32_t CAND_SUBS = 129, CAND_COST_SUBS = 16, CAND_ROW_SUBS = 111;
+        constexpr uint32_t CAND_STRAGGLER_SUB = CAND_COST_SUBS + CAND_ROW_SUBS, CAND_WAVE_SUB = CAND_STRAGGLER_SUB + 1;
+        static_assert(CAND_WAVE_SUB + 1 == CAND_SUBS, "the wave tasks' bucket is a queue's last");
         constexpr uint32_t PSET_RANGE_BKS = 64, PSET_SUBS = 64;
         constexpr uint32_t CAND_KEY0 = TASK_KINDS * SCHED_NB, PSET_KEY0 = CAND_KEY0 + CAND_QUEUES * CAND_SUBS, SCHED_KEYS = PSET_KEY0 + PSET_RANGE_BKS * PSET_SUBS;
         inline uint32_t pset_sub(const uint32_t rank) { return rank < PSET_SUBS / 2 ? rank : std::min(PSET_SUBS / 2 + (rank - PSET_SUBS / 2) / 8, PSET_SUBS - 1); }
diff --git a/trinity_amd/csrc/trinity_hip.hip b/trinity_amd/csrc/trinity_hip.hip
--- a/trinity_amd/csrc/trinity_hip.hip
+++ b/trinity_amd/csrc/trinity_hip.hip
@@ -1110,7 +1110,7 @@
         if (b->n_cand)
                 TRI_LAUNCH(k_and, ix->codec, dim3(std::min<uint32_t>(b->n_cand, (uint32_t)dev->cus * cand_wgs)), dim3(AND_WG), cand_stream, match_bytes, ix->d_blk_last, match_off,
                            ix->d_win, ix->d_terms, b->dev_at(b->plan), b->dev_at(b->tasks), b->dev_at(b->sched) + trip::sched_first(*b, TASK_CAND), b->dev_at(b->qterms), b->dev_at(b->cand_q),
-                           b->d_ticket + TICKET_CAND_WORD, b->d_out, b->d_counts, ix->d_masked, (const uint32_t *)b->dev_opt(b->qplane), (const uint32_t *)ix->d_pcache, b->plw);
+                           b->dev_at(b->cand_w), b->d_ticket + TICKET_CAND_WORD, b->d_out, b->d_counts, ix->d_masked, (const uint32_t *)b->dev_opt(b->qplane), (const uint32_t *)ix->d_pcache, b->plw);
         HIP_TRY(hipGetLastError());
         if (overlap) {
                 HIP_TRY(hipEventRecord(dev->ev_join, dev->stream2));
@@ -1481,6 +1481,13 @@
                         if (cnt[j])
                                 fprintf(stderr, "  term %d %.1f (%.0f tasks)", j - 2, sum[j] / cnt[j], cnt[j]);
                 fprintf(stderr, "\n");
+                unsigned long long wsum = 0;
+                uint32_t wn = 0;
+                for (uint32_t i = 0; i < nc; ++i)
+                        if (g_tt_host[8 * i] && g_tt_host[8 * i + 1] && trip::cand_wave_task(*b->ix, *b, b->tasks[b->sched[first + i]]))
+                                wsum += g_tt_host[8 * i + 1] - g_tt_host[8 * i], ++wn;
+                fprintf(stderr, "   wave tasks: %u of %u, summed span %.1f us = %.1f %% of the tasks' summed span (%.1f us); kernel span x %u workgroups = %.1f us\n", wn, nc, (double)wsum / 100.0,
+                        100.0 * (double)wsum / (double)std::max(1ull, busy), (double)busy / 100.0, wgs, span_us * wgs);
         }
 #endif
         for (size_t k = 0; k < std::min<size_t>(12, by.size()); ++k) {
diff --git a/trinity_amd/hostplan.py b/trinity_amd/hostplan.py
--- a/trinity_amd/hostplan.py
+++ b/trinity_amd/hostplan.py
@@ -9,7 +9,7 @@
             "n_dense", "n_cand", "n_fused", "n_fused16", "n_fusedgen", "n_planes", "n_planes8", "plw", "sparse_cap", "out_capacity", "term_bytes", "term_bytes_dense",
             "dense_queries", "cand_queries", "fused_queries", "planes_queries", "unsupported_queries", "rich_R", "sizeof_query", "sizeof_task", "sizeof_fused", "sizeof_phrase",
             "cand_needed_term_bytes", "plane_decoded_bytes", "n_pset", "pset_queries", "n_probe", "probe_queries", "n_units", "off_units", "off_unit_sched", "sizeof_unit",
-            "n_tree", "tree_queries", "n_tree_words", "off_tree", "n_tree_terms", "off_tree_terms", "n_tree_hidden", "off_tree_hidden", "off_cand_q"]
+            "n_tree", "tree_queries", "n_tree_words", "off_tree", "n_tree_terms", "off_tree_terms", "n_tree_hidden", "off_tree_hidden", "off_cand_q", "off_cand_w"]
 
 DEV_QUERY = np.dtype([("nterms", "<u4"), ("term_base", "<u4"), ("out_off", "<u8"), ("out_cap", "<u4"), ("qid", "<u4"), ("first_task", "<u4"), ("ntasks", "<u4"),
                       ("score_base", "<u4"), ("nscore", "<u4"), ("phrase_base", "<u4"), ("nphrases", "<u4"), ("fused_idx", "<u4"), ("form", "<u4")])
@@ -122,6 +122,10 @@
         return self._view("off_cand_q", 9, "<u4")
 
     @property
+    def cand_w(self):
+        return self._view("off_cand_w", 8, "<u4")
+
+    @property
     def qterms(self):
         return self._view("off_qterms", self.s["n_qterms"], "<u4")
 
```

New measurement: 11.92 million. 18.0% lower.
